# ihsanhadi57/Face-Detection-With-YOLOv11-SAHI-and-Real-ESRGAN

Measured on AMD Instinct MI355X. Metric: end-to-end 4K frames/sec (SAHI+YOLOv11s+ESRGAN×4), higher is better.
Workload: dtype f32x3(detect)+f16(sr)

## Files before the change

### face-detection-with-yolov11-sahi-and-real-esrgan_amd/_lib.py

```python
from __future__ import annotations

import ctypes as C
import os
import sys
from typing import List, Optional, Sequence, Tuple

import numpy as np

from . import weights_io

_HERE = os.path.dirname(os.path.abspath(__file__))
LIB_PATH = os.environ.get("FFP_LIB") or os.path.join(_HERE, "libffp.so")

PREC_F32, PREC_F16, PREC_F32X3 = 0, 1, 2
SR_ALPHA_REALESRGAN, SR_ALPHA_LINEAR = 0, 1
CHAN_AS_BGR, CHAN_AS_RGB = 0, 1
IQA_F32_CHW, IQA_U8_HWC = 0, 1
NIQE_FEATURES = 36
PP_NMS, PP_GREEDYNMM = 0, 1
METRIC_IOU, METRIC_IOS = 0, 1
PP_TYPES = {"NMS": PP_NMS, "GREEDYNMM": PP_GREEDYNMM}
METRICS = {"IOU": METRIC_IOU, "IOS": METRIC_IOS}

_lib = None


class FfpError(RuntimeError):
    def __init__(self, code: int, msg: str):
        super().__init__(f"libffp error {code}: {msg}")
        self.code = code


def _p(t):
    return C.POINTER(t)


_SIGS = {
    "ffp_last_error": (C.c_char_p, []),
    "ffp_version": (C.c_int, []),
    "ffp_device_count": (C.c_int, [_p(C.c_int)]),
    "ffp_slice_bboxes": (C.c_int, [C.c_int, C.c_int, C.c_int, C.c_int, C.c_float, C.c_float, _p(C.c_int32), C.c_int, _p(C.c_int32)]),
    "ffp_tile_chunks": (C.c_int, [C.c_int, C.c_int, _p(C.c_int32), C.c_int, _p(C.c_int32)]),
    "ffp_letterbox_geometry": (C.c_int, [C.c_int, C.c_int, C.c_int, _p(C.c_int32)]),
    "ffp_det_create": (C.c_int, [C.c_void_p, C.c_size_t, C.c_int, C.c_int, C.c_int, C.c_int, C.c_int, _p(C.c_void_p)]),
    "ffp_det_destroy": (None, [C.c_void_p]),
    "ffp_det_infer_tiles": (C.c_int, [C.c_void_p, C.c_void_p, C.c_int, C.c_int, C.c_int, _p(C.c_int32), C.c_int, C.c_int, C.c_float,
                                      C.c_float, C.c_int, C.c_int, _p(C.c_float), _p(C.c_int32)]),
    "ffp_det_infer_tiles_dev": (C.c_int, [C.c_void_p, C.c_void_p, C.c_int, C.c_int, C.c_int, _p(C.c_int32), C.c_int, C.c_int, C.c_float,
                                          C.c_float, C.c_int, C.c_int, C.c_void_p, C.c_void_p]),
    "ffp_det_truncate_shift_dev": (C.c_int, [C.c_void_p, C.c_void_p, C.c_void_p, C.c_int, C.c_int, C.c_int, C.c_int]),
    "ffp_det_forward_raw": (C.c_int, [C.c_void_p, C.c_void_p, C.c_int, C.c_int, C.c_int, _p(C.c_int32), C.c_int, C.c_int, _p(C.c_float),
                                      C.c_size_t, _p(C.c_int32)]),
    "ffp_merge": (C.c_int, [C.c_int, _p(C.c_float), C.c_int, C.c_int, C.c_int, C.c_int, C.c_double, C.c_int, _p(C.c_float), _p(C.c_int32),
                            _p(C.c_int32)]),
    "ffp_merge_dev": (C.c_int, [C.c_void_p, C.c_void_p, C.c_void_p, C.c_int, C.c_int, C.c_int, C.c_int, C.c_double, C.c_int, C.c_void_p,
                                C.c_int, C.c_void_p]),
    "ffp_sliced_predict": (C.c_int, [C.c_void_p, C.c_void_p, C.c_int, C.c_int, C.c_int, C.c_int, C.c_int, C.c_float, C.c_float, C.c_int,
                                     C.c_int, C.c_float, C.c_float, C.c_int, C.c_int, C.c_int, C.c_int, C.c_double, C.c_int, _p(C.c_float),
                                     C.c_int, _p(C.c_int32)]),
    "ffp_det_stage_dev": (C.c_int, [C.c_void_p, C.c_void_p, C.c_int, C.c_int, C.c_int, C.c_int, C.c_int, C.c_float, C.c_float, C.c_int,
                                    C.c_int, C.c_float, C.c_float, C.c_int, C.c_int, C.c_int, C.c_int, C.c_void_p, C.c_void_p,
                                    _p(C.c_int32), _p(C.c_int32)]),
    "ffp_det_last_ms": (C.c_int, [C.c_void_p, C.c_int, _p(C.c_float)]),
    "ffp_det_last_conv_stats": (C.c_int, [C.c_void_p, _p(C.c_double), _p(C.c_float), _p(C.c_int32)]),
    "ffp_det_set_profile": (C.c_int, [C.c_void_p, C.c_int]),
    "ffp_det_profile_count": (C.c_int, [C.c_void_p, _p(C.c_int32)]),
    "ffp_det_profile_get": (C.c_int, [C.c_void_p, C.c_int, C.c_char_p, C.c_int, _p(C.c_double), _p(C.c_float), _p(C.c_int32)]),
    "ffp_det_profile_detail": (C.c_int, [C.c_void_p, C.c_int, C.c_char_p, C.c_int, _p(C.c_double), _p(C.c_float)]),
    "ffp_sr_profile_detail": (C.c_int, [C.c_void_p, C.c_int, C.c_char_p, C.c_int, _p(C.c_double), _p(C.c_float)]),
    "ffp_sr_create": (C.c_int, [C.c_void_p, C.c_size_t, C.c_int, C.c_int, C.c_int, C.c_int, _p(C.c_void_p)]),
    "ffp_sr_destroy": (None, [C.c_void_p]),
    "ffp_sr_enhance": (C.c_int, [C.c_void_p, C.c_void_p, C.c_int, C.c_int, C.c_int, C.c_int, C.c_int, C.c_void_p]),
    "ffp_sr_enhance_ex": (C.c_int, [C.c_void_p, C.c_void_p, C.c_int, C.c_int, C.c_int, C.c_int, C.c_int, C.c_int, C.c_int, C.c_int, C.c_int,
                                    C.c_int, C.c_int, C.c_void_p]),
    "ffp_sr_enhance_dev": (C.c_int, [C.c_void_p, C.c_void_p, C.c_int, C.c_int, C.c_int, C.c_int, C.c_int, C.c_void_p]),
    "ffp_sr_enhance_batch": (C.c_int, [C.c_void_p, C.c_int, _p(C.c_void_p), _p(C.c_int32), _p(C.c_int32), C.c_int, C.c_int, C.c_int,
                                       _p(C.c_void_p)]),
    "ffp_sr_enhance_crops_dev": (C.c_int, [C.c_void_p, C.c_void_p, C.c_int, C.c_int, _p(C.c_int32), C.c_int, C.c_int, C.c_int, C.c_void_p,
                                           C.c_size_t, _p(C.c_int64)]),
    "ffp_sr_enhance_crops_dev_async": (C.c_int, [C.c_void_p, C.c_void_p, C.c_int, C.c_int, _p(C.c_int32), C.c_int, C.c_int, C.c_int,
                                                 C.c_void_p, C.c_size_t, _p(C.c_int64)]),
    "ffp_sr_wait": (C.c_int, [C.c_void_p]),
    "ffp_sr_enhance_crops_multi_dev_async": (C.c_int, [C.c_void_p, C.c_int, _p(C.c_void_p), _p(C.c_int32), C.c_int, C.c_int, _p(C.c_int32),
                                                       C.c_int, C.c_int, C.c_int, C.c_void_p, C.c_size_t, _p(C.c_int64)]),
    "ffp_sr_plan_state": (C.c_int, [C.c_void_p, _p(C.c_int32), _p(C.c_int32)]),
    "ffp_det_graph_status": (C.c_int, [C.c_void_p, _p(C.c_int32)]),
    "ffp_sr_set_fused_body": (C.c_int, [C.c_void_p, C.c_int]),
    "ffp_det_drop_plans": (C.c_int, [C.c_void_p]),
    "ffp_sr_drop_plans": (C.c_int, [C.c_void_p]),
    "ffp_det_profile_bytes": (C.c_int, [C.c_void_p, C.c_int, _p(C.c_double)]),
    "ffp_sr_profile_bytes": (C.c_int, [C.c_void_p, C.c_int, _p(C.c_double)]),
    "ffp_conv_totals_enable": (C.c_int, [C.c_int]),
    "ffp_conv_totals_count": (C.c_int, [_p(C.c_int32)]),
    "ffp_conv_totals_get": (C.c_int, [C.c_int, C.c_char_p, C.c_int, _p(C.c_double), _p(C.c_double), _p(C.c_int64)]),
    "ffp_sr_mem_bytes": (C.c_int, [C.c_void_p, _p(C.c_uint64), _p(C.c_uint64), _p(C.c_int32)]),
    "ffp_det_mem_bytes": (C.c_int, [C.c_void_p, _p(C.c_uint64), _p(C.c_uint64), _p(C.c_int32)]),
    "ffp_det_set_lanes": (C.c_int, [C.c_void_p, C.c_int]),
    "ffp_det_set_buffer_reuse": (C.c_int, [C.c_void_p, C.c_int]),
    "ffp_det_set_gate": (C.c_int, [C.c_void_p, C.c_int]),
    "ffp_det_last_active": (C.c_int, [C.c_void_p, C.POINTER(C.c_int32), C.POINTER(C.c_int32)]),
    "ffp_det_mem_detail": (C.c_int, [C.c_void_p, _p(C.c_uint64), _p(C.c_uint64), _p(C.c_uint64)]),
    "ffp_det_fill_steps": (C.c_int, [C.c_void_p, _p(C.c_int32), _p(C.c_int32)]),
    "ffp_det_stream_wait_event": (C.c_int, [C.c_void_p, C.c_void_p]),
    "ffp_sr_last_ms": (C.c_int, [C.c_void_p, _p(C.c_float)]),
    "ffp_sr_last_conv_stats": (C.c_int, [C.c_void_p, _p(C.c_double), _p(C.c_float), _p(C.c_int32)]),
    "ffp_sr_set_profile": (C.c_int, [C.c_void_p, C.c_int]),
    "ffp_sr_profile_count": (C.c_int, [C.c_void_p, _p(C.c_int32)]),
    "ffp_sr_profile_get": (C.c_int, [C.c_void_p, C.c_int, C.c_char_p, C.c_int, _p(C.c_double), _p(C.c_float), _p(C.c_int32)]),
    "ffp_eval_wider_pr": (C.c_int, [C.c_int, _p(C.c_double), _p(C.c_int64), _p(C.c_double), _p(C.c_int64), _p(C.c_uint8), C.c_int, C.c_double, C.c_int,
                                    _p(C.c_int64)]),
    "ffp_eval_dual_match": (C.c_int, [C.c_int, _p(C.c_double), _p(C.c_int64), _p(C.c_double), _p(C.c_int64), _p(C.c_uint8), C.c_int, C.c_double, _p(C.c_int32)]),
    "ffp_eval_coco_bbox": (C.c_int, [C.c_int, C.c_int, C.c_int, _p(C.c_double), _p(C.c_int64), _p(C.c_double), _p(C.c_int64), _p(C.c_double), C.c_int,
                                     _p(C.c_double), C.c_int, _p(C.c_double), C.c_int, _p(C.c_int32), C.c_int, _p(C.c_double), _p(C.c_double),
                                     _p(C.c_double), _p(C.c_double), _p(C.c_uint8), _p(C.c_double), _p(C.c_uint8)]),
    "ffp_jpeg_encode": (C.c_int, [C.c_int, _p(C.c_uint8), C.c_int, C.c_int, C.c_int, C.c_int, _p(C.c_uint8), C.c_int64, _p(C.c_int64)]),
    "ffp_jpeg_encode_dev": (C.c_int, [C.c_int, C.c_void_p, C.c_int, C.c_int, C.c_int64, C.c_int, C.c_int, _p(C.c_uint8), C.c_int64, _p(C.c_int64)]),
    "ffp_jpeg_encode_batch_dev": (C.c_int, [C.c_int, C.c_void_p, C.c_int, _p(C.c_int64), _p(C.c_int32), _p(C.c_int32), _p(C.c_int64), C.c_int, C.c_int, _p(C.c_uint8),
                                            C.c_int64, _p(C.c_int64)]),
    "ffp_png_bound": (C.c_int64, [C.c_int, C.c_int, C.c_int, C.c_int]),
    "ffp_png_segment_bytes": (C.c_int, []),
    "ffp_png_encode": (C.c_int, [C.c_int, C.c_void_p, C.c_int, C.c_int, C.c_int, C.c_int, C.c_int, C.c_int, _p(C.c_uint8), C.c_int64, _p(C.c_int64)]),
    "ffp_png_encode_dev": (C.c_int, [C.c_int, C.c_void_p, C.c_int, C.c_int, C.c_int, C.c_int, C.c_int64, C.c_int, C.c_int, _p(C.c_uint8), C.c_int64, _p(C.c_int64)]),
    "ffp_png_encode_batch_dev": (C.c_int, [C.c_int, C.c_void_p, C.c_int, _p(C.c_int64), _p(C.c_int32), _p(C.c_int32), _p(C.c_int64), C.c_int, C.c_int, C.c_int, C.c_int,
                                           _p(C.c_uint8), C.c_int64, _p(C.c_int64)]),
    "ffp_jpeg_info": (C.c_int, [_p(C.c_uint8), C.c_int64, _p(C.c_int32), _p(C.c_int32), _p(C.c_int32)]),
    "ffp_jpeg_decode": (C.c_int, [C.c_int, _p(C.c_uint8), C.c_int64, C.c_int, _p(C.c_uint8), C.c_int64]),
    "ffp_jpeg_decode_dev": (C.c_int, [C.c_int, _p(C.c_uint8), C.c_int64, C.c_int, C.c_void_p, C.c_int64, C.c_int64]),
    "ffp_jpeg_decode_stats": (C.c_int, [_p(C.c_int64), _p(C.c_int64), _p(C.c_int64)]),
    "ffp_op_conv2d_shape": (C.c_int, [C.c_int]),
    "ffp_op_conv2d_shape_name": (C.c_int, [C.c_int, C.c_char_p, C.c_int]),
    "ffp_op_conv2d_last_variant": (C.c_int, [C.c_char_p, C.c_int]),
    "ffp_op_conv2d_act_post": (C.c_int, [C.c_int]),
    "ffp_op_conv1x1_up2": (C.c_int, [C.c_int, C.c_int, _p(C.c_float), _p(C.c_float), C.c_int, C.c_int, C.c_int, C.c_int, C.c_int, _p(C.c_float),
                                     _p(C.c_float), C.c_int, C.c_int, _p(C.c_float)]),
    "ffp_op_conv2d_time": (C.c_int, [C.c_int, C.c_int, C.c_int, C.c_int, C.c_int, C.c_int, C.c_int, C.c_int, C.c_int, C.c_int, C.c_int, C.c_int,
                                     C.c_int, _p(C.c_float)]),
    "ffp_op_conv2d": (C.c_int, [C.c_int, C.c_int, _p(C.c_float), C.c_int, C.c_int, C.c_int, C.c_int, _p(C.c_float), _p(C.c_float), C.c_int,
                                C.c_int, C.c_int, C.c_int, C.c_int, C.c_int, _p(C.c_float), C.c_float, _p(C.c_float)]),
    "ffp_op_variant": (C.c_int, [C.c_int, C.c_int]),
    "ffp_op_cls_tower_variant": (C.c_int, [C.c_int, C.c_int]),
    "ffp_op_sppf_pool": (C.c_int, [C.c_int, C.c_int, C.c_int, _p(C.c_int32), _p(C.c_int32), C.c_int, C.c_int, _p(C.c_float), C.c_int, C.c_int,
                                   _p(C.c_float), C.c_int, C.c_int, C.c_int, C.c_int]),
    "ffp_op_upsample2x": (C.c_int, [C.c_int, C.c_int, C.c_int, _p(C.c_int32), _p(C.c_int32), C.c_int, C.c_int, _p(C.c_float), C.c_int, C.c_int,
                                    _p(C.c_float), C.c_int, C.c_int]),
    "ffp_op_psa_attention": (C.c_int, [C.c_int, C.c_int, C.c_int, _p(C.c_int32), _p(C.c_int32), C.c_int, C.c_int, _p(C.c_float), C.c_int, C.c_int,
                                       _p(C.c_float), C.c_int, C.c_int]),
    "ffp_op_dwconv3x3": (C.c_int, [C.c_int, C.c_int, C.c_int, _p(C.c_int32), _p(C.c_int32), C.c_int, C.c_int, _p(C.c_float), C.c_int, C.c_int,
                                   C.c_int, C.c_int, C.c_int, _p(C.c_float), _p(C.c_float), C.c_int, _p(C.c_float), C.c_int, C.c_int,
                                   _p(C.c_float), C.c_int, C.c_int]),
    "ffp_op_cls_tower": (C.c_int, [C.c_int, C.c_int, _p(C.c_int32), _p(C.c_int32), C.c_int, C.c_int, C.c_int] + [_p(C.c_float)] * 13 + [C.c_int, C.c_int, _p(C.c_int64)]),
    "ffp_op_conv2d_views": (C.c_int, [C.c_int, C.c_int, C.c_int, _p(C.c_int32), _p(C.c_int32), C.c_int, _p(C.c_float), C.c_int, C.c_int, C.c_int,
                                      _p(C.c_float), _p(C.c_float), C.c_int, C.c_int, C.c_int, C.c_int, C.c_int, C.c_int, _p(C.c_float), C.c_int,
                                      C.c_int, C.c_float, _p(C.c_float), C.c_int, C.c_int, C.c_float, _p(C.c_float), C.c_int, C.c_int, C.c_int,
                                      _p(C.c_uint32), _p(C.c_int32), _p(C.c_int32), _p(C.c_int64)]),
    "ffp_op_det_post": (C.c_int, [C.c_int, C.c_int, _p(C.c_int32), _p(C.c_int32), C.c_int, C.c_int, C.c_int, _p(C.c_float), _p(C.c_float),
                                  _p(C.c_float), _p(C.c_float), _p(C.c_int32), C.c_float, C.c_float, C.c_int, C.c_int, C.c_int, C.c_int, C.c_int,
                                  _p(C.c_float), _p(C.c_float), _p(C.c_int32)]),
    "ffp_op_rt_topk": (C.c_int, [C.c_int, C.c_int, C.c_int, C.c_int, _p(C.c_float), C.c_int, C.c_int, _p(C.c_int32)]),
    "ffp_op_rt_dwconv": (C.c_int, [C.c_int, C.c_int, C.c_int, C.c_int, C.c_int, C.c_int, C.c_int, C.c_int, _p(C.c_float), C.c_int, C.c_int, _p(C.c_float), _p(C.c_float), _p(C.c_float), C.c_int, C.c_int, _p(C.c_uint32)]),
    "ffp_op_rt_maxpool2": (C.c_int, [C.c_int, C.c_int, C.c_int, C.c_int, C.c_int, _p(C.c_float), C.c_int, C.c_int, _p(C.c_float), C.c_int, C.c_int, _p(C.c_uint32)]),
    "ffp_op_rt_add": (C.c_int, [C.c_int, C.c_longlong, C.c_int, _p(C.c_float), C.c_int, C.c_int, _p(C.c_float), C.c_int, C.c_int, C.c_longlong, _p(C.c_float), C.c_int, C.c_int, _p(C.c_uint32)]),
    "ffp_op_rt_layernorm": (C.c_int, [C.c_int, C.c_longlong, _p(C.c_float), C.c_int, C.c_int, _p(C.c_float), _p(C.c_float), _p(C.c_float), C.c_int, C.c_int, _p(C.c_uint32)]),
    "ffp_op_rt_gelu": (C.c_int, [C.c_int, C.c_longlong, C.c_int, _p(C.c_float), C.c_int, C.c_int, _p(C.c_uint32)]),
    "ffp_op_rt_attention": (C.c_int, [C.c_int, C.c_int, C.c_int, _p(C.c_float), C.c_int, C.c_int, _p(C.c_float), C.c_int, C.c_int, _p(C.c_float), C.c_int, C.c_int, _p(C.c_uint32)]),
    "ffp_op_rt_enc_prep": (C.c_int, [C.c_int, C.c_int, _p(C.c_int32), _p(C.c_int32), _p(C.c_float), _p(C.c_float), _p(C.c_float), _p(C.c_int32), _p(C.c_int32), _p(C.c_float), C.c_longlong, _p(C.c_float), _p(C.c_float), _p(C.c_uint32), _p(C.c_uint32)]),
    "ffp_op_rt_gather": (C.c_int, [C.c_int, C.c_int, C.c_int, _p(C.c_float), C.c_int, C.c_int, _p(C.c_int32), _p(C.c_float), _p(C.c_float), C.c_int, C.c_int, _p(C.c_float), _p(C.c_uint32)]),
    "ffp_op_rt_ref": (C.c_int, [C.c_int, C.c_longlong, _p(C.c_float), C.c_int, C.c_int, _p(C.c_float), _p(C.c_float), C.c_int, C.c_int, _p(C.c_uint32)]),
    "ffp_op_rt_deform": (C.c_int, [C.c_int, C.c_int, _p(C.c_int32), _p(C.c_int32), _p(C.c_float), C.c_int, C.c_int, _p(C.c_float), C.c_int, C.c_int, _p(C.c_float), C.c_int, C.c_int, _p(C.c_float), C.c_int, C.c_int, _p(C.c_uint32)]),
    "ffp_op_rt_decode": (C.c_int, [C.c_int, C.c_int, C.c_int, _p(C.c_float), C.c_int, C.c_int, _p(C.c_float), C.c_int, C.c_int, C.c_float, _p(C.c_float), _p(C.c_float), _p(C.c_float), _p(C.c_int32)]),
    "ffp_op_rt_post_tiles": (C.c_int, [C.c_int, C.c_int, C.c_int, _p(C.c_float), C.c_int, C.c_int, _p(C.c_float), C.c_int, C.c_int, C.c_float, _p(C.c_int32), C.c_int, C.c_int, C.c_int, _p(C.c_float), _p(C.c_int32)]),
    "ffp_op_scrfd_pool": (C.c_int, [C.c_int, C.c_int, _p(C.c_int32), _p(C.c_int32), C.c_int, C.c_int, C.c_int, C.c_int, _p(C.c_float), C.c_int, C.c_int, _p(C.c_float), C.c_int, C.c_int]),
    "ffp_op_scrfd_post": (C.c_int, [C.c_int, C.c_int, C.c_int, C.c_int, C.c_int, _p(C.c_int32), C.c_int, _p(_p(C.c_float)), _p(C.c_int32), _p(C.c_int32), _p(C.c_float), C.c_float, C.c_float, C.c_int, _p(C.c_float), _p(C.c_int32), _p(C.c_float)]),
    "ffp_op_resize_lanczos4": (C.c_int, [C.c_int, C.c_void_p, C.c_int, C.c_int, C.c_int, C.c_int, C.c_int, C.c_int, C.c_void_p]),
    "ffp_op_image_input": (C.c_int, [C.c_int, C.c_int, C.c_int, _p(C.c_uint8), C.c_int, C.c_int, C.c_int, C.c_int, _p(C.c_int32), C.c_int, C.c_int,
                                     _p(C.c_float), _p(C.c_int32), _p(C.c_int32)]),
    "ffp_op_stem": (C.c_int, [C.c_int, C.c_int, C.c_int, _p(C.c_uint8), C.c_int, C.c_int, C.c_int, C.c_int, _p(C.c_int32), C.c_int, _p(C.c_float),
                              _p(C.c_float), C.c_int, C.c_int, C.c_int, _p(C.c_float)]),
    "ffp_op_stem_conv": (C.c_int, [C.c_int, _p(C.c_uint8), C.c_int, C.c_int, C.c_int, C.c_int, _p(C.c_int32), C.c_int, _p(C.c_float), _p(C.c_float),
                                   C.c_int, _p(C.c_float), _p(C.c_float), _p(C.c_float)]),
    "ffp_scrfd_create": (C.c_int, [C.c_void_p, C.c_size_t, C.c_int, C.c_int, C.c_int, _p(C.c_void_p)]),
    "ffp_scrfd_destroy": (None, [C.c_void_p]),
    "ffp_scrfd_describe": (C.c_int, [C.c_void_p, C.c_size_t, C.c_int, C.c_int, C.c_int, C.c_char_p, C.c_size_t]),
    "ffp_scrfd_infer_tiles": (C.c_int, [C.c_void_p, C.c_void_p, C.c_int, C.c_int, C.c_int, _p(C.c_int32), C.c_int, C.c_int, C.c_int, C.c_float,
                                        C.c_float, _p(C.c_float), C.c_int, _p(C.c_int32)]),
    "ffp_scrfd_infer_tiles_ex": (C.c_int, [C.c_void_p, C.c_void_p, C.c_int, C.c_int, C.c_int, _p(C.c_int32), C.c_int, C.c_int, C.c_int, C.c_float,
                                           C.c_float, C.c_float, C.c_int, C.c_int, _p(C.c_float), C.c_int, _p(C.c_int32)]),
    "ffp_scrfd_infer_tiles_dev": (C.c_int, [C.c_void_p, C.c_void_p, C.c_int, C.c_int, C.c_int, _p(C.c_int32), C.c_int, C.c_int, C.c_int, C.c_float,
                                            C.c_float, C.c_float, C.c_int, C.c_int, C.c_void_p, C.c_int, C.c_void_p]),
    "ffp_scrfd_sliced_predict": (C.c_int, [C.c_void_p, C.c_void_p, C.c_int, C.c_int, C.c_int, C.c_int, C.c_int, C.c_float, C.c_float, C.c_int, C.c_int,
                                           C.c_int, C.c_float, C.c_float, C.c_float, C.c_int, C.c_int, C.c_int, C.c_int, C.c_double, C.c_int,
                                           _p(C.c_float), C.c_int, _p(C.c_int32)]),
    "ffp_scrfd_sliced_predict_dev": (C.c_int, [C.c_void_p, C.c_void_p, C.c_int, C.c_int, C.c_int, C.c_int, C.c_int, C.c_float, C.c_float, C.c_int,
                                               C.c_int, C.c_int, C.c_float, C.c_float, C.c_float, C.c_int, C.c_int, C.c_int, C.c_int, C.c_double,
                                               C.c_int, C.c_void_p, C.c_int, C.c_void_p]),
    "ffp_scrfd_mem_bytes": (C.c_int, [C.c_void_p, _p(C.c_uint64), _p(C.c_int32)]),
    "ffp_scrfd_drop_plans": (C.c_int, [C.c_void_p]),
    "ffp_op_scrfd_sahi_rows": (C.c_int, [C.c_int, C.c_int, C.c_int, _p(C.c_int32), C.c_int, C.c_int, C.c_float, _p(C.c_float), _p(C.c_int32),
                                         _p(C.c_int32)]),
    "ffp_scrfd_forward_raw": (C.c_int, [C.c_void_p, C.c_void_p, C.c_int, C.c_int, C.c_int, _p(C.c_int32), C.c_int, C.c_int, C.c_int, _p(C.c_float),
                                        C.c_size_t, _p(C.c_int64)]),
    "ffp_scrfd_info": (C.c_int, [C.c_void_p, _p(C.c_int32), _p(C.c_double)]),
    "ffp_scrfd_geometry": (C.c_int, [C.c_int, C.c_int, C.c_int, C.c_int, _p(C.c_int32), _p(C.c_float)]),
    "ffp_rtdetr_create": (C.c_int, [C.c_void_p, C.c_size_t, C.c_int, C.c_int, _p(C.c_void_p)]),
    "ffp_rtdetr_destroy": (None, [C.c_void_p]),
    "ffp_rtdetr_predict": (C.c_int, [C.c_void_p, _p(C.c_void_p), _p(C.c_int32), C.c_int, C.c_int, C.c_float, _p(C.c_float), _p(C.c_int32)]),
    "ffp_rtdetr_forward_raw": (C.c_int, [C.c_void_p, _p(C.c_void_p), _p(C.c_int32), C.c_int, C.c_int, _p(C.c_float), _p(C.c_int32)]),
    "ffp_rtdetr_infer_tiles": (C.c_int, [C.c_void_p, C.c_void_p, C.c_int, C.c_int, C.c_int, _p(C.c_int32), C.c_int, C.c_int, C.c_float, C.c_int, C.c_int,
                                         _p(C.c_float), _p(C.c_int32)]),
    "ffp_rtdetr_infer_tiles_dev": (C.c_int, [C.c_void_p, C.c_void_p, C.c_int, C.c_int, C.c_int, _p(C.c_int32), C.c_int, C.c_int, C.c_float, C.c_int,
                                             C.c_int, C.c_void_p, C.c_void_p]),
    "ffp_rtdetr_sliced_predict": (C.c_int, [C.c_void_p, C.c_void_p, C.c_int, C.c_int, C.c_int, C.c_int, C.c_int, C.c_float, C.c_float, C.c_int, C.c_int,
                                            C.c_float, C.c_int, C.c_int, C.c_int, C.c_double, C.c_int, _p(C.c_float), C.c_int, _p(C.c_int32)]),
    "ffp_rtdetr_mem_bytes": (C.c_int, [C.c_void_p, _p(C.c_uint64), _p(C.c_int32)]),
    "ffp_rtdetr_drop_plans": (C.c_int, [C.c_void_p]),
    "ffp_rtdetr_info": (C.c_int, [C.c_void_p, _p(C.c_int32), _p(C.c_double), _p(C.c_int32)]),
    "ffp_rtdetr_set_profile": (C.c_int, [C.c_void_p, C.c_int]),
    "ffp_rtdetr_profile_count": (C.c_int, [C.c_void_p, _p(C.c_int32)]),
    "ffp_rtdetr_profile_get": (C.c_int, [C.c_void_p, C.c_int, C.c_char_p, C.c_int, _p(C.c_float)]),
    "ffp_iqa_create": (C.c_int, [C.c_int, _p(C.c_void_p)]),
    "ffp_iqa_destroy": (None, [C.c_void_p]),
    "ffp_iqa_niqe_blocks": (C.c_int, [C.c_int, C.c_int, _p(C.c_int64)]),
    "ffp_iqa_niqe_features": (C.c_int, [C.c_void_p, C.c_int, _p(C.c_void_p), _p(C.c_int32), _p(C.c_int32), _p(C.c_int32), C.c_int, C.c_int, C.c_int,
                                        _p(C.c_double), _p(C.c_double), C.c_int64, _p(C.c_int64)]),
    "ffp_iqa_niqe_luma": (C.c_int, [C.c_void_p, C.c_void_p, C.c_int, C.c_int, C.c_int, C.c_int, C.c_int, _p(C.c_float)]),
    "ffp_iqa_niqe_score": (C.c_int, [_p(C.c_double), _p(C.c_int64), C.c_int, _p(C.c_double), _p(C.c_double), _p(C.c_double)]),
}

EXPORTED_SYMBOLS = tuple(_SIGS)


def lib() -> C.CDLL:
    global _lib
    if _lib is None:
        if not os.path.exists(LIB_PATH):
            raise RuntimeError(f"{LIB_PATH} is missing: build it with `python -m ffp_amd.build` "
                               "(hipcc --offload-arch=gfx950). There is no CPU/PyTorch fallback.")
        if "torch" not in sys.modules:
            try:
                import importlib.util
                spec = importlib.util.find_spec("torch")
                cand = os.path.join(os.path.dirname(spec.origin), "lib", "libamdhip64.so") if spec and spec.origin else None
                if cand and os.path.exists(cand):
                    C.CDLL(cand, mode=C.RTLD_GLOBAL)
            except Exception:
                pass
        l = C.CDLL(LIB_PATH)
        for name, (res, args) in _SIGS.items():
            f = getattr(l, name)
            f.restype = res
            f.argtypes = args
        _lib = l
    return _lib


def _check(rc: int):
    if rc != 0:
        raise FfpError(rc, lib().ffp_last_error().decode("utf-8", "replace"))


def device_count() -> int:
    n = C.c_int(0)
    _check(lib().ffp_device_count(C.byref(n)))
    return n.value


def _fp(a: np.ndarray):
    return a.ctypes.data_as(_p(C.c_float))


def _ip(a: np.ndarray):
    return a.ctypes.data_as(_p(C.c_int32))


def slice_bboxes(H: int, W: int, slice_h: int, slice_w: int, overlap_h: float = 0.2, overlap_w: float = 0.2) -> np.ndarray:
    n = C.c_int32(0)
    _check(lib().ffp_slice_bboxes(H, W, slice_h, slice_w, overlap_h, overlap_w, None, 0, C.byref(n)))
    out = np.zeros((n.value, 4), np.int32)
    _check(lib().ffp_slice_bboxes(H, W, slice_h, slice_w, overlap_h, overlap_w, _ip(out), n.value, C.byref(n)))
    return out


def tile_chunks(n: int, max_batch: int) -> List[int]:
# ... 1108 lines not shown
    if rc != 0:
        e = FfpError(rc, lib().ffp_last_error().decode("utf-8", "replace"))
        e.needed = n.value
        raise e
    return out[:n.value].tobytes()


def png_encode_dev(d_ptr: int, h: int, w: int, channels: int = 3, bit_depth: int = 8, row_stride: int = None, level: int = 1, bgr: bool = True,
                   device: int = 0) -> bytes:
    if row_stride is None:
        row_stride = w * channels * (bit_depth // 8)
    cap = png_bound(h, w, channels, bit_depth)
    out = np.empty(cap, np.uint8)
    n = C.c_int64(0)
    _check(lib().ffp_png_encode_dev(device, C.c_void_p(d_ptr), h, w, channels, bit_depth, row_stride, int(bgr), level, out.ctypes.data_as(_p(C.c_uint8)), cap,
                                    C.byref(n)))
    return out[:n.value].tobytes()


def png_encode_batch_dev(d_base: int, offsets, hs, ws, channels: int = 3, bit_depth: int = 8, strides=None, level: int = 1, bgr: bool = True, device: int = 0):
    offsets = np.ascontiguousarray(offsets, np.int64)
    hs, ws = np.ascontiguousarray(hs, np.int32), np.ascontiguousarray(ws, np.int32)
    n = len(offsets)
    st = None if strides is None else np.ascontiguousarray(strides, np.int64)
    cap = sum(png_bound(int(h), int(w), channels, bit_depth) for h, w in zip(hs, ws))
    out = np.empty(max(cap, 1), np.uint8)
    oo = np.zeros(n + 1, np.int64)
    _check(lib().ffp_png_encode_batch_dev(device, C.c_void_p(d_base), n, offsets.ctypes.data_as(_p(C.c_int64)), hs.ctypes.data_as(_p(C.c_int32)),
                                          ws.ctypes.data_as(_p(C.c_int32)), None if st is None else st.ctypes.data_as(_p(C.c_int64)), channels, bit_depth,
                                          int(bgr), level, out.ctypes.data_as(_p(C.c_uint8)), cap, oo.ctypes.data_as(_p(C.c_int64))))
    return [out[oo[i]:oo[i + 1]].tobytes() for i in range(n)]


def jpeg_info(data: bytes):
    buf = np.frombuffer(data, np.uint8)
    h, w, nc = C.c_int32(0), C.c_int32(0), C.c_int32(0)
    _check(lib().ffp_jpeg_info(buf.ctypes.data_as(_p(C.c_uint8)), len(buf), C.byref(h), C.byref(w), C.byref(nc)))
    return h.value, w.value, nc.value


def jpeg_decode(data: bytes, bgr: bool = False, device: int = 0) -> np.ndarray:
    h, w, _ = jpeg_info(data)
    buf = np.frombuffer(data, np.uint8)
    out = np.empty((h, w, 3), np.uint8)
    _check(lib().ffp_jpeg_decode(device, buf.ctypes.data_as(_p(C.c_uint8)), len(buf), int(bgr), out.ctypes.data_as(_p(C.c_uint8)), out.size))
    return out


def jpeg_decode_dev(data: bytes, d_ptr: int, row_stride: int, cap: int, bgr: bool = True, device: int = 0):
    h, w, _ = jpeg_info(data)
    buf = np.frombuffer(data, np.uint8)
    _check(lib().ffp_jpeg_decode_dev(device, buf.ctypes.data_as(_p(C.c_uint8)), len(buf), int(bgr), C.c_void_p(d_ptr), row_stride, cap))
    return h, w


def jpeg_decode_stats():
    a, b, c = C.c_int64(0), C.c_int64(0), C.c_int64(0)
    _check(lib().ffp_jpeg_decode_stats(C.byref(a), C.byref(b), C.byref(c)))
    return a.value, b.value, c.value


def _ragged(rows, width, dtype):
    rows = [np.asarray(r, dtype).reshape(-1, width) for r in rows]
    off = np.zeros(len(rows) + 1, np.int64)
    np.cumsum([len(r) for r in rows], out=off[1:])
    flat = np.ascontiguousarray(np.concatenate(rows + [np.zeros((0, width), dtype)], 0))
    return flat, off


def eval_wider_pr(preds, gts, evaluate, iou_thr: float = 0.5, thresh_num: int = 1000, device: int = 0) -> np.ndarray:
    p, po = _ragged(preds, 5, np.float64)
    g, go = _ragged(gts, 4, np.float64)
    e, eo = _ragged([np.asarray(x, np.uint8).reshape(-1, 1) for x in evaluate], 1, np.uint8)
    if len(po) != len(go) or not np.array_equal(go, eo):
        raise ValueError("preds / gts / evaluate must describe the same images and faces")
    out = np.zeros((thresh_num, 2), np.int64)
    _check(lib().ffp_eval_wider_pr(device, p.ctypes.data_as(_p(C.c_double)), po.ctypes.data_as(_p(C.c_int64)), g.ctypes.data_as(_p(C.c_double)),
                                   go.ctypes.data_as(_p(C.c_int64)), e.ctypes.data_as(_p(C.c_uint8)), len(po) - 1, iou_thr, thresh_num,
                                   out.ctypes.data_as(_p(C.c_int64))))
    return out


def eval_dual_match(preds, faces, valid, iou_thr: float = 0.5, device: int = 0):
    p, po = _ragged(preds, 5, np.float64)
    f, fo = _ragged(faces, 4, np.float64)
    v, vo = _ragged([np.asarray(x, np.uint8).reshape(-1, 1) for x in valid], 1, np.uint8)
    if len(po) != len(fo) or not np.array_equal(fo, vo):
        raise ValueError("preds / faces / valid must describe the same images and faces")
    flags = np.zeros(max(int(po[-1]), 1), np.int32)
    _check(lib().ffp_eval_dual_match(device, p.ctypes.data_as(_p(C.c_double)), po.ctypes.data_as(_p(C.c_int64)), f.ctypes.data_as(_p(C.c_double)),
                                     fo.ctypes.data_as(_p(C.c_int64)), v.ctypes.data_as(_p(C.c_uint8)), len(po) - 1, iou_thr, flags.ctypes.data_as(_p(C.c_int32))))
    return [flags[po[i]:po[i + 1]] for i in range(len(po) - 1)]


def eval_coco_bbox(dets, det_off, gts, gt_off, n_img: int, n_cat: int, iou_thrs, rec_thrs, area_rng, max_dets, matches: bool = False,
                   device: int = 0) -> dict:
    d = np.ascontiguousarray(np.asarray(dets, np.float64).reshape(-1, 7))
    g = np.ascontiguousarray(np.asarray(gts, np.float64).reshape(-1, 8))
    do = np.ascontiguousarray(det_off, np.int64)
    go = np.ascontiguousarray(gt_off, np.int64)
    it = np.ascontiguousarray(iou_thrs, np.float64).reshape(-1)
    rt = np.ascontiguousarray(rec_thrs, np.float64).reshape(-1)
    ar = np.ascontiguousarray(area_rng, np.float64).reshape(-1, 2)
    md = np.ascontiguousarray(max_dets, np.int32).reshape(-1)
    U = int(n_img) * int(n_cat)
    if len(do) != U + 1 or len(go) != U + 1:
        raise ValueError(f"offsets must have n_cat * n_img + 1 = {U + 1} entries")
    T, R, K, A, M = len(it), len(rt), int(n_cat), len(ar), len(md)
    prec, sc = np.zeros((T, R, K, A, M)), np.zeros((T, R, K, A, M))
    rec = np.zeros((T, K, A, M))
    out = {"precision": prec, "recall": rec, "scores": sc}
    ptrs = [None] * 4
    if matches:
        cut = np.zeros(U + 1, np.int64)
        if U and len(md):
            np.cumsum(np.minimum(np.diff(do), int(md[-1])), out=cut[1:])
        ndc, ng = int(cut[-1]), int(go[-1]) if U else 0
        out.update(cut_off=cut, dt_matches=np.zeros((A, T, ndc)), dt_ignore=np.zeros((A, T, ndc), np.uint8), gt_matches=np.zeros((A, T, ng)),
                   gt_ignore=np.zeros((A, ng), np.uint8))
        ptrs = [out["dt_matches"].ctypes.data_as(_p(C.c_double)), out["dt_ignore"].ctypes.data_as(_p(C.c_uint8)),
                out["gt_matches"].ctypes.data_as(_p(C.c_double)), out["gt_ignore"].ctypes.data_as(_p(C.c_uint8))]
    dp = lambda a: a.ctypes.data_as(_p(C.c_double))
    _check(lib().ffp_eval_coco_bbox(device, int(n_img), int(n_cat), dp(d), do.ctypes.data_as(_p(C.c_int64)), dp(g), go.ctypes.data_as(_p(C.c_int64)),
                                    dp(it), T, dp(rt), R, dp(ar), A, md.ctypes.data_as(_p(C.c_int32)), M, dp(prec), dp(rec), dp(sc), *ptrs))
    return out


def op_conv1x1_up2(coarse: np.ndarray, fine: np.ndarray, w: np.ndarray, b: np.ndarray, act: int = 0, precision: int = PREC_F32X3, device: int = 0) -> np.ndarray:
    coarse = np.ascontiguousarray(coarse, np.float32)
    fine = np.ascontiguousarray(fine, np.float32)
    w = np.ascontiguousarray(w, np.float32).reshape(w.shape[0], -1)
    b = np.ascontiguousarray(b, np.float32)
    n, h, wd, cf = fine.shape
    y = np.zeros((n, h, wd, w.shape[0]), np.float32)
    _check(lib().ffp_op_conv1x1_up2(device, precision, _fp(coarse), _fp(fine), n, h, wd, coarse.shape[3], cf, _fp(w), _fp(b), w.shape[0], act, _fp(y)))
    return y


def op_resize_lanczos4(img: np.ndarray, out_h: int, out_w: int, device: int = 0) -> np.ndarray:
    a = np.ascontiguousarray(img)
    if a.dtype not in (np.uint8, np.uint16) or a.ndim not in (2, 3):
        raise ValueError(f"expected an HxW or HxWxC uint8 / uint16 array, got {a.dtype} {a.shape}")
    h, w = a.shape[:2]
    out = np.zeros((int(out_h), int(out_w)) + a.shape[2:], a.dtype)
    _check(lib().ffp_op_resize_lanczos4(device, a.ctypes.data, h, w, 1 if a.ndim == 2 else a.shape[2], 8 * a.itemsize, int(out_h), int(out_w),
                                        out.ctypes.data))
    return out


def op_conv2d_shape(shape: int = -1) -> None:
    _check(lib().ffp_op_conv2d_shape(int(shape)))


def op_conv2d_shape_name(shape: int) -> str:
    out = C.create_string_buffer(64)
    _check(lib().ffp_op_conv2d_shape_name(int(shape), out, len(out)))
    return out.value.decode()


def op_conv2d_last_variant() -> str:
    out = C.create_string_buffer(64)
    _check(lib().ffp_op_conv2d_last_variant(out, len(out)))
    return out.value.decode()


def op_conv2d_act_post(act: int = 0) -> None:
    _check(lib().ffp_op_conv2d_act_post(int(act)))


def op_conv2d_time(n, h, w, cin, cout, k=3, stride=1, up=False, precision=PREC_F16, iters=50, dbg=0, shape=-1, device=0) -> float:
    us = C.c_float(0)
    _check(lib().ffp_op_conv2d_time(device, precision, n, h, w, cin, cout, k, stride, int(up), iters, dbg, shape, C.byref(us)))
    return us.value


def niqe_blocks(h: int, w: int) -> int:
    n = C.c_int64(0)
    _check(lib().ffp_iqa_niqe_blocks(int(h), int(w), C.byref(n)))
    return n.value


def niqe_score(feat: np.ndarray, block_off: np.ndarray, mu: np.ndarray, cov: np.ndarray) -> np.ndarray:
    f = np.ascontiguousarray(feat, np.float64).reshape(-1, NIQE_FEATURES)
    off = np.ascontiguousarray(block_off, np.int64)
    m = np.ascontiguousarray(np.asarray(mu, np.float64).reshape(-1))
    c = np.ascontiguousarray(cov, np.float64)
    if m.shape != (NIQE_FEATURES,) or c.shape != (NIQE_FEATURES, NIQE_FEATURES):
        raise ValueError(f"the NIQE model is a 36-vector and a 36x36 matrix, got {m.shape} and {c.shape}")
    if off.ndim != 1 or off.size < 1 or off[-1] != f.shape[0]:
        raise ValueError("block offsets do not match the feature rows")
    out = np.zeros(off.size - 1, np.float64)
    dp = _p(C.c_double)
    _check(lib().ffp_iqa_niqe_score(f.ctypes.data_as(dp), off.ctypes.data_as(_p(C.c_int64)), off.size - 1, m.ctypes.data_as(dp), c.ctypes.data_as(dp),
                                    out.ctypes.data_as(dp)))
    return out


class IQA:

    def __init__(self, device: int = 0):
        self._h = C.c_void_p()
        self.device = device
        _check(lib().ffp_iqa_create(device, C.byref(self._h)))

    def close(self):
        if getattr(self, "_h", None) is not None and self._h.value:
            lib().ffp_iqa_destroy(self._h)
            self._h = C.c_void_p()

    def __del__(self):
        try:
            self.close()
        except Exception:
            pass

    def niqe_features(self, images: Sequence[np.ndarray], chan_order: int = CHAN_AS_RGB) -> Tuple[np.ndarray, np.ndarray, np.ndarray]:
        ims = [np.ascontiguousarray(i) for i in images]
        if not ims:
            raise ValueError("no images")
        kinds = {i.dtype == np.uint8 for i in ims}
        if len(kinds) != 1 or any(i.dtype not in (np.uint8, np.float32) for i in ims):
            raise ValueError("images must be all uint8 (H, W, C) or all float32 (C, H, W)")
        u8 = ims[0].dtype == np.uint8
        shp = []
        for i in ims:
            if i.ndim == 2:
                shp.append((i.shape[0], i.shape[1], 1))
            elif i.ndim == 3:
                shp.append((i.shape[0], i.shape[1], i.shape[2]) if u8 else (i.shape[1], i.shape[2], i.shape[0]))
            else:
                raise ValueError(f"expected a 2-d or 3-d image, got shape {i.shape}")
        return self._features([i.ctypes.data for i in ims], shp, IQA_U8_HWC if u8 else IQA_F32_CHW, chan_order, False)

    def luma(self, image: np.ndarray, chan_order: int = CHAN_AS_RGB) -> np.ndarray:
        a = np.ascontiguousarray(image)
        u8 = a.dtype == np.uint8
        if a.dtype not in (np.uint8, np.float32) or a.ndim not in (2, 3):
            raise ValueError(f"expected a uint8 (H, W, C) or float32 (C, H, W) image, got {a.dtype} {a.shape}")
        h, w, c = (a.shape[0], a.shape[1], 1) if a.ndim == 2 else ((a.shape[0], a.shape[1], a.shape[2]) if u8 else (a.shape[1], a.shape[2], a.shape[0]))
        out = np.zeros((max(h // 96 * 96, 1), max(w // 96 * 96, 1)), np.float32)
        _check(lib().ffp_iqa_niqe_luma(self._h, a.ctypes.data, h, w, c, IQA_U8_HWC if u8 else IQA_F32_CHW, int(chan_order), _fp(out)))
        return out

    def niqe_features_dev(self, ptrs: Sequence[int], shapes: Sequence[Tuple[int, int, int]]) -> Tuple[np.ndarray, np.ndarray, np.ndarray]:
        return self._features(list(ptrs), [(h, w, c) for c, h, w in shapes], IQA_F32_CHW, CHAN_AS_RGB, True)

    def _features(self, ptrs, shp, layout, chan_order, on_device):
        n = len(ptrs)
        hs = np.asarray([s[0] for s in shp], np.int32)
        ws = np.asarray([s[1] for s in shp], np.int32)
        cs = np.asarray([s[2] for s in shp], np.int32)
        nb = max(1, sum((int(h) // 96) * (int(w) // 96) for h, w in zip(hs, ws)))
        feat = np.zeros((nb, NIQE_FEATURES), np.float64)
        sharp = np.zeros(nb, np.float64)
        off = np.zeros(n + 1, np.int64)
        ip = (C.c_void_p * n)(*ptrs)
        _check(lib().ffp_iqa_niqe_features(self._h, n, ip, _ip(hs), _ip(ws), _ip(cs), layout, int(chan_order), int(on_device),
                                           feat.ctypes.data_as(_p(C.c_double)), sharp.ctypes.data_as(_p(C.c_double)), nb, off.ctypes.data_as(_p(C.c_int64))))
        return feat[:off[-1]], sharp[:off[-1]], off

    def niqe(self, images: Sequence[np.ndarray], mu: np.ndarray, cov: np.ndarray, chan_order: int = CHAN_AS_RGB) -> np.ndarray:
        feat, _, off = self.niqe_features(images, chan_order)
        return niqe_score(feat, off, mu, cov)
```

### face-detection-with-yolov11-sahi-and-real-esrgan_amd/csrc/api_ops.cpp

```cpp
#include <climits>
#include <cmath>

#include "api_util.hpp"
#include "conv_route.hpp"
#include "rtdetr.hpp"
#include "scrfd.hpp"
#include "sr_ops.hpp"
#include "yolo11.hpp"

using namespace ffp;

extern "C" {

static int g_op_conv_shape = SHAPE_AUTO;
int ffp_op_conv2d_shape(int force_shape) {
  FFP_API_BEGIN
  FFP_CHECK(force_shape == SHAPE_AUTO || conv_shape_info(force_shape), FFP_ERR_ARG, "conv2d_shape: %d is not a shape number", force_shape);
  g_op_conv_shape = force_shape;
  FFP_API_END
}

int ffp_op_conv2d_shape_name(int shape, char* out, int cap) {
  FFP_API_BEGIN
  const ConvShapeInfo* s = conv_shape_info(shape);
  FFP_CHECK(s && out && cap > 0, FFP_ERR_ARG, "conv2d_shape_name: %d is not a shape number, or no output buffer", shape);
  std::snprintf(out, cap, "%s %s", s->family_name, s->suffix);
  FFP_API_END
}

static thread_local std::string tl_op_conv_variant;
int ffp_op_conv2d_last_variant(char* out, int cap) {
  FFP_API_BEGIN
  FFP_CHECK(out && cap > 0, FFP_ERR_ARG, "conv2d_last_variant: no output buffer");
  std::snprintf(out, cap, "%s", tl_op_conv_variant.c_str());
  FFP_API_END
}

static int g_op_conv_act_post = ACT_NONE;
int ffp_op_conv2d_act_post(int act) {
  FFP_API_BEGIN
  FFP_CHECK(act >= ACT_NONE && act <= ACT_RELU, FFP_ERR_ARG, "conv2d_act_post: activation code %d (0..3)", act);
  g_op_conv_act_post = act;
  FFP_API_END
}

int ffp_op_conv2d(int device, int precision, const float* x, int n, int h, int w, int cin, const float* wt, const float* bias, int cout,
                  int k, int stride, int groups, int act, int up, const float* res, float res_scale, float* y) {
  FFP_API_BEGIN
  FFP_CHECK(x && wt && y && n > 0 && h > 0 && w > 0 && cin > 0 && cout > 0, FFP_ERR_ARG, "conv2d: bad arguments");
  FFP_CHECK((k == 1 || k == 3) && (stride == 1 || stride == 2), FFP_ERR_ARG, "conv2d: k in {1,3}, stride in {1,2}");
  ScopedStream cx(device, "conv2d");
  conv_kernels_init();
  tl_op_conv_variant.clear();
  const DType T = precision == FFP_PREC_F16 ? F16 : F32;
  const bool split = precision == FFP_PREC_F32X3;
  PackedConv pc;
  pack_conv(pc, "op", wt, bias, cout, cin, k, groups, T, cx.st, split);
  const int hi = up ? h * 2 : h, wi = up ? w * 2 : w;
  const int ho = (hi + 2 * (k / 2) - k) / stride + 1, wo = (wi + 2 * (k / 2) - k) / stride + 1;
  Level lin, lout;
  lin.build(std::vector<int>(n, h), std::vector<int>(n, w), cx.st);
  lout.build(std::vector<int>(n, ho), std::vector<int>(n, wo), cx.st);
  const int cin_s = pc.depthwise() ? cin : pc.cin;
  const size_t npx_in = (size_t)lin.total_px, npx_out = (size_t)lout.total_px;
  auto to_dev = [&](const float* src, size_t px, int c, int c_store) {
    DevBuf b(px * c_store * dsize(T) + 256);
    if (T == F32) {
      std::vector<float> t(px * c_store, 0.f);
      for (size_t p = 0; p < px; ++p) std::memcpy(&t[p * c_store], src + p * c, sizeof(float) * c);
      FFP_HIP(hipMemcpy(b.p, t.data(), t.size() * 4, hipMemcpyHostToDevice));
    } else {
      std::vector<_Float16> t(px * c_store, (_Float16)0.f);
      for (size_t p = 0; p < px; ++p) for (int q = 0; q < c; ++q) t[p * c_store + q] = (_Float16)src[p * c + q];
      FFP_HIP(hipMemcpy(b.p, t.data(), t.size() * 2, hipMemcpyHostToDevice));
    }
    return b;
  };
  DevBuf din = to_dev(x, npx_in, cin, cin_s);
  DevBuf dres;
  if (res) dres = to_dev(res, npx_out, cout, cout);
  DevBuf dout(npx_out * cout * dsize(T) + 256);
  TView vin{din.p, T, cin_s, 0, cin_s, &lin}, vout{dout.p, T, cout, 0, cout, &lout}, vres{dres.p, T, cout, 0, cout, &lout};
  DevBuf slots(2 * sizeof(unsigned));
  {
    float m = 0.f;
    for (size_t i = 0; i < npx_in * (size_t)cin; ++i) m = std::max(m, std::fabs(x[i]));
    unsigned hb[2] = {0u, 0u};
    std::memcpy(&hb[0], &m, 4);
    FFP_HIP(hipMemcpy(slots.p, hb, sizeof(hb), hipMemcpyHostToDevice));
    vin.amax = slots.as<unsigned>(); vout.amax = slots.as<unsigned>() + 1;
  }
  if (pc.depthwise()) {
    FFP_CHECK(k == 3 && stride == 1 && !up, FFP_ERR_ARG, "conv2d: depthwise is 3x3 stride 1");
    FFP_CHECK(g_op_conv_act_post == ACT_NONE, FFP_ERR_ARG, "conv2d: depthwise convs have no post-activation");
    DwConvOp o;
    o.pc = &pc; o.in = vin; o.out = vout; o.out.lvl = &lin; o.act = act;
    if (res) { o.has_res = true; o.res = vres; o.res.lvl = &lin; FFP_CHECK(res_scale == 1.f, FFP_ERR_ARG, "conv2d: depthwise residual has no scale"); }
    launch_dwconv(o, cx.st);
  } else {
    ConvOp o;
    o.pc = &pc; o.in = vin; o.out = vout; o.stride = stride; o.act = act; o.up = up;
    if (res) { o.has_res1 = true; o.res1 = vres; o.s1 = res_scale; }
    o.force_shape = g_op_conv_shape;
    o.act_post = g_op_conv_act_post;
    launch_conv(o, cx.st);
    tl_op_conv_variant = conv_variant(o);
  }
  FFP_HIP(hipStreamSynchronize(cx.st));
  if (T == F32) {
    FFP_HIP(hipMemcpy(y, dout.p, npx_out * cout * 4, hipMemcpyDeviceToHost));
  } else {
    std::vector<_Float16> t(npx_out * cout);
    FFP_HIP(hipMemcpy(t.data(), dout.p, t.size() * 2, hipMemcpyDeviceToHost));
    for (size_t i = 0; i < t.size(); ++i) y[i] = (float)t[i];
  }
  FFP_API_END
}

int ffp_op_conv1x1_up2(int device, int precision, const float* coarse, const float* fine, int n, int h, int w, int c_up, int c_fine,
                       const float* wt, const float* bias, int cout, int act, float* y) {
  FFP_API_BEGIN
  FFP_CHECK(coarse && fine && wt && y && n > 0 && h > 0 && w > 0 && h % 2 == 0 && w % 2 == 0 && c_up > 0 && c_fine > 0 && cout > 0, FFP_ERR_ARG, "conv1x1_up2: bad arguments");
  FFP_CHECK(precision == FFP_PREC_F32 || precision == FFP_PREC_F32X3, FFP_ERR_ARG, "conv1x1_up2: fp32 precisions only");
  ScopedStream cx(device, "conv1x1_up2");
  conv_kernels_init();
  tl_op_conv_variant.clear();
  const int cin = c_up + c_fine;
  PackedConv pc;
  pack_conv(pc, "op", wt, bias, cout, cin, 1, 1, F32, cx.st, precision == FFP_PREC_F32X3);
  FFP_CHECK(pc.cin == cin, FFP_ERR_ARG, "conv1x1_up2: channel count %d needs padding", cin);
  Level lf, lc;
  lf.build(std::vector<int>(n, h), std::vector<int>(n, w), cx.st);
  lc.build(std::vector<int>(n, h / 2), std::vector<int>(n, w / 2), cx.st);
  const size_t pf = (size_t)lf.total_px, pcs = (size_t)lc.total_px;
  std::vector<float> cat(pf * cin, std::nanf(""));
  for (size_t p = 0; p < pf; ++p) std::memcpy(&cat[p * cin + c_up], fine + p * c_fine, sizeof(float) * c_fine);
  DevBuf dcat(cat.size() * 4 + 256), dco(pcs * c_up * 4 + 256), dout(pf * cout * 4 + 256), slots(3 * sizeof(unsigned));
  FFP_HIP(hipMemcpy(dcat.p, cat.data(), cat.size() * 4, hipMemcpyHostToDevice));
  FFP_HIP(hipMemcpy(dco.p, coarse, pcs * c_up * 4, hipMemcpyHostToDevice));
  float mf = 0.f, mc = 0.f;
  for (size_t i = 0; i < pf * (size_t)c_fine; ++i) mf = std::max(mf, std::fabs(fine[i]));
  for (size_t i = 0; i < pcs * (size_t)c_up; ++i) mc = std::max(mc, std::fabs(coarse[i]));
  unsigned hb[3] = {0u, 0u, 0u};
  std::memcpy(&hb[0], &mf, 4);
  std::memcpy(&hb[1], &mc, 4);
  FFP_HIP(hipMemcpy(slots.p, hb, sizeof(hb), hipMemcpyHostToDevice));
  TView vin{dcat.p, F32, cin, 0, cin, &lf}, vco{dco.p, F32, c_up, 0, c_up, &lc}, vout{dout.p, F32, cout, 0, cout, &lf};
  vin.amax = slots.as<unsigned>(); vco.amax = slots.as<unsigned>() + 1; vout.amax = slots.as<unsigned>() + 2;
  ConvOp o;
  o.pc = &pc; o.in = vin; o.out = vout; o.stride = 1; o.act = act;
  o.has_up2 = true; o.up2 = vco; o.up2_c = c_up; o.up2_map = lf.up2_map(&lc, cx.st);
  o.force_shape = g_op_conv_shape;
  launch_conv(o, cx.st);
  tl_op_conv_variant = conv_variant(o);
  FFP_HIP(hipStreamSynchronize(cx.st));
  FFP_HIP(hipMemcpy(y, dout.p, pf * cout * 4, hipMemcpyDeviceToHost));
  FFP_API_END
}

static int g_op_variant[3] = {0, 0, 0};
int ffp_op_variant(int family, int variant) {
  FFP_API_BEGIN
  FFP_CHECK(family >= 0 && family < 3 && variant >= 0 && variant <= 2, FFP_ERR_ARG, "op_variant: family %d / variant %d unknown", family, variant);
  g_op_variant[family] = variant;
  FFP_API_END
}
static int g_op_cls_tower_force = 0;
int ffp_op_cls_tower_variant(int rows, int wg_cap) {
  FFP_API_BEGIN
  FFP_CHECK((rows == 0 || rows == 8 || rows == 16) && wg_cap >= 0 && wg_cap <= 65535, FFP_ERR_ARG, "op_cls_tower_variant: rows %d (0, 8, 16) / workgroup cap %d", rows, wg_cap);
  g_op_cls_tower_force = (rows == 16 ? 1 : rows == 8 ? 2 : 0) | wg_cap << 2;
  FFP_API_END
}

namespace {

void op_check_batch(const char* what, int n, const int32_t* hs, const int32_t* ws, int px_align) {
  FFP_CHECK(n > 0 && n <= 4096 && hs && ws && px_align >= 1 && px_align <= 4096, FFP_ERR_ARG, "%s: bad batch description", what);
  for (int i = 0; i < n; ++i) FFP_CHECK(hs[i] > 0 && ws[i] > 0 && hs[i] <= 8192 && ws[i] <= 8192, FFP_ERR_ARG, "%s: image %d is %dx%d", what, i, ws[i], hs[i]);
}
void op_check_view(const char* what, int cs, int coff, int C) {
  FFP_CHECK(C > 0 && coff >= 0 && cs > 0 && coff + C <= cs, FFP_ERR_ARG, "%s: channels [%d, %d) do not fit records of %d", what, coff, coff + C, cs);
}
DType op_dtype(const char* what, int precision) {
  FFP_CHECK(precision == FFP_PREC_F32 || precision == FFP_PREC_F16, FFP_ERR_ARG, "%s: precision must be FFP_PREC_F32 or FFP_PREC_F16", what);
  return precision == FFP_PREC_F16 ? F16 : F32;
}

DevBuf op_upload(const Level& L, DType T, const float* src, int cs) {
  const size_t tot = (size_t)L.total_px * cs;
  DevBuf b(tot * dsize(T) + 256);
  std::vector<float> t(tot, std::nanf(""));
  size_t sp = 0;
  for (int i = 0; i < L.n; ++i) {
    const size_t np = (size_t)L.h[i] * L.w[i];
    std::memcpy(&t[(size_t)L.off[i] * cs], src + sp * cs, np * cs * sizeof(float));
    sp += np;
  }
  if (T == F32) {
    FFP_HIP(hipMemcpy(b.p, t.data(), tot * 4, hipMemcpyHostToDevice));
  } else {
    std::vector<_Float16> h(tot);
    for (size_t i = 0; i < tot; ++i) h[i] = (_Float16)t[i];
    FFP_HIP(hipMemcpy(b.p, h.data(), tot * 2, hipMemcpyHostToDevice));
  }
  return b;
}

void op_download(const Level& L, DType T, const DevBuf& b, int cs, float* dst) {
  const size_t tot = (size_t)L.total_px * cs;
  std::vector<float> t(tot);
  if (T == F32) {
    FFP_HIP(hipMemcpy(t.data(), b.p, tot * 4, hipMemcpyDeviceToHost));
  } else {
    std::vector<_Float16> h(tot);
    FFP_HIP(hipMemcpy(h.data(), b.p, tot * 2, hipMemcpyDeviceToHost));
    for (size_t i = 0; i < tot; ++i) t[i] = (float)h[i];
  }
  size_t sp = 0;
  for (int i = 0; i < L.n; ++i) {
    const size_t np = (size_t)L.h[i] * L.w[i];
    std::memcpy(dst + sp * cs, &t[(size_t)L.off[i] * cs], np * cs * sizeof(float));
    sp += np;
  }
}

}

int ffp_op_sppf_pool(int device, int precision, int n, const int32_t* hs, const int32_t* ws, int px_align, int c, const float* x, int x_cs,
                     int x_coff, float* y, int y_cs, int y1_coff, int y2_coff, int y3_coff) {
  FFP_API_BEGIN
  FFP_CHECK(x && y, FFP_ERR_ARG, "sppf_pool: null argument");
  op_check_batch("sppf_pool", n, hs, ws, px_align);
  op_check_view("sppf_pool input", x_cs, x_coff, c);
  const int yo[3] = {y1_coff, y2_coff, y3_coff};
  for (int i = 0; i < 3; ++i) {
    op_check_view("sppf_pool output", y_cs, yo[i], c);
    for (int j = 0; j < i; ++j) FFP_CHECK(yo[i] >= yo[j] + c || yo[j] >= yo[i] + c, FFP_ERR_ARG, "sppf_pool: output slices %d and %d overlap", j + 1, i + 1);
  }
  const DType T = op_dtype("sppf_pool", precision);
  ScopedStream cx(device, "sppf_pool");
  Level L;
  L.build(std::vector<int>(hs, hs + n), std::vector<int>(ws, ws + n), cx.st, px_align);
  DevBuf din = op_upload(L, T, x, x_cs), dout = op_upload(L, T, y, y_cs);
  const TView vin{din.p, T, x_cs, x_coff, c, &L};
  const TView v1{dout.p, T, y_cs, y1_coff, c, &L}, v2{dout.p, T, y_cs, y2_coff, c, &L}, v3{dout.p, T, y_cs, y3_coff, c, &L};
  launch_sppf_pool(vin, v1, v2, v3, cx.st, g_op_variant[0]);
  FFP_HIP(hipStreamSynchronize(cx.st));
  op_download(L, T, dout, y_cs, y);
  FFP_API_END
}

int ffp_op_upsample2x(int device, int precision, int n, const int32_t* hs, const int32_t* ws, int px_align, int c, const float* x, int x_cs,
                      int x_coff, float* y, int y_cs, int y_coff) {
  FFP_API_BEGIN
  FFP_CHECK(x && y, FFP_ERR_ARG, "upsample2x: null argument");
// ... 88 lines not shown
  pack_conv(dw1, "cv3.1.0", dw1_w, dw1_b, C3, C3, 3, C3, F32, cx.st, false);
  pack_conv(pw1, "cv3.1.1", pw1_w, pw1_b, C3, C3, 1, 1, F32, cx.st, true);
  pack_conv(fin, "cv3.2", fin_w, fin_b, nc, C3, 1, 1, F32, cx.st, true);
  DenseF32 dense;
  dense.w.alloc(sizeof(float) * nc * C3);
  dense.b.alloc(sizeof(float) * nc);
  FFP_HIP(hipMemcpy(dense.w.p, fin_w, sizeof(float) * nc * C3, hipMemcpyHostToDevice));
  FFP_HIP(hipMemcpy(dense.b.p, fin_b, sizeof(float) * nc, hipMemcpyHostToDevice));
  Level L;
  L.build(std::vector<int>(hs, hs + n), std::vector<int>(ws, ws + n), cx.st, px_align);
  DevBuf dx = op_upload(L, F32, x, cin), dhead = op_upload(L, F32, head, head_cs);
  FFP_HIP(hipMemset(static_cast<char*>(dhead.p) + (size_t)L.total_px * head_cs * 4, 0xFF, 256));
  DevBuf de1((size_t)L.total_px * C3 * 4 + 256), de2((size_t)L.total_px * C3 * 4 + 256);
  FFP_HIP(hipMemset(de1.p, 0xFF, de1.n));
  FFP_HIP(hipMemset(de2.p, 0xFF, de2.n));
  std::vector<unsigned> slots(3 * (size_t)n, 0u);
  {
    size_t sp = 0;
    for (int i = 0; i < n; ++i) {
      const size_t np = (size_t)hs[i] * ws[i] * cin;
      float m = 0.f;
      for (size_t k = 0; k < np; ++k) m = std::max(m, std::fabs(x[sp + k]));
      std::memcpy(&slots[i], &m, 4);
      sp += np;
    }
  }
  DevBuf dslots(slots.size() * 4);
  FFP_HIP(hipMemcpy(dslots.p, slots.data(), slots.size() * 4, hipMemcpyHostToDevice));
  auto view = [&](void* p, int cs, int coff, int c, int slot) {
    TView v{p, F32, cs, coff, c, &L};
    if (slot >= 0) { v.amax = dslots.as<unsigned>() + (size_t)slot * n; v.amax_n = n; }
    return v;
  };
  const bool fuse_fin = nc <= 4;
  ConvOp t1, t2;
  t1.pc = &pw0; t1.dw = &dw0; t1.dw_act = ACT_SILU; t1.act = ACT_SILU;
  t1.in = view(dx.p, cin, 0, cin, 0); t1.out = view(de1.p, C3, 0, C3, 1);
  t2.pc = &pw1; t2.dw = &dw1; t2.dw_act = ACT_SILU; t2.act = ACT_SILU;
  t2.in = t1.out; t2.out = view(fuse_fin ? nullptr : de2.p, C3, 0, C3, 2);
  const TView logits = view(dhead.p, head_cs, head_coff, nc, -1);
  if (fuse_fin) { t2.fin = &fin; t2.fin_w = &dense; t2.fin_out = logits; }
  t1.dwpw_force = t2.dwpw_force = g_op_cls_tower_force;
  launch_conv(t1, cx.st);
  launch_conv(t2, cx.st);
  if (!fuse_fin) {
    ConvOp t3;
    t3.pc = &fin; t3.in = t2.out; t3.out = logits; t3.act = ACT_NONE;
    launch_conv(t3, cx.st);
  }
  FFP_HIP(hipStreamSynchronize(cx.st));
  op_download(L, F32, dhead, head_cs, head);
  if (e1) op_download(L, F32, de1, C3, e1);
  if (stray) {
    const float nanv = std::nanf("");
    unsigned nan_bits;
    std::memcpy(&nan_bits, &nanv, 4);
    auto changed = [&](const DevBuf& b, int cs, unsigned want, unsigned want_slack) {
      std::vector<unsigned> h(b.n / 4);
      FFP_HIP(hipMemcpy(h.data(), b.p, h.size() * 4, hipMemcpyDeviceToHost));
      int64_t bad = 0;
      for (int i = 0; i < n; ++i) {
        const size_t p0 = (size_t)(L.off[i] + (int64_t)hs[i] * ws[i]) * cs, p1 = (size_t)(i + 1 < n ? L.off[i + 1] : L.total_px) * cs;
        for (size_t k = p0; k < p1; ++k) bad += h[k] != want;
      }
      for (size_t k = (size_t)L.total_px * cs; k < h.size(); ++k) bad += h[k] != want_slack;
      return bad;
    };
    *stray = changed(de1, C3, 0xFFFFFFFFu, 0xFFFFFFFFu) + changed(de2, C3, 0xFFFFFFFFu, 0xFFFFFFFFu);
    if (fuse_fin) *stray += changed(dhead, head_cs, nan_bits, 0xFFFFFFFFu);
  }
  FFP_API_END
}

int ffp_op_conv2d_views(int device, int precision, int n, const int32_t* hs, const int32_t* ws, int px_align, const float* x, int x_cs, int x_coff,
                        int cin, const float* wt, const float* bias, int cout, int k, int stride, int act, int act_post, int up, const float* res1,
                        int r1_cs, int r1_coff, float s1, const float* res2, int r2_cs, int r2_coff, float s2, float* y, int y_cs, int y_coff,
                        int per_image_amax, uint32_t* amax_out, const int32_t* gate, const int32_t* gate_prev, int64_t* stray) {
  FFP_API_BEGIN
  FFP_CHECK(x && wt && y && amax_out && cin > 0 && cout > 0, FFP_ERR_ARG, "conv2d_views: null argument or no channels");
  FFP_CHECK(precision == FFP_PREC_F32 || precision == FFP_PREC_F16 || precision == FFP_PREC_F32X3, FFP_ERR_ARG, "conv2d_views: precision %d", precision);
  FFP_CHECK((k == 1 || k == 3) && (stride == 1 || stride == 2) && (up == 0 || up == 1) && (per_image_amax == 0 || per_image_amax == 1), FFP_ERR_ARG,
            "conv2d_views: k in {1,3}, stride in {1,2}, up and per_image_amax in {0,1}");
  FFP_CHECK(act >= ACT_NONE && act <= ACT_RELU && act_post >= ACT_NONE && act_post <= ACT_RELU, FFP_ERR_ARG, "conv2d_views: activation codes %d / %d (0..3)", act, act_post);
  FFP_CHECK(!gate_prev || gate, FFP_ERR_ARG, "conv2d_views: gate_prev without gate");
  op_check_batch("conv2d_views", n, hs, ws, px_align);
  const DType T = precision == FFP_PREC_F16 ? F16 : F32;
  const int epv = 16 / (int)dsize(T);
  const int cin_s = (cin + epv - 1) / epv * epv;
  op_check_view("conv2d_views input", x_cs, x_coff, cin_s);
  FFP_CHECK(x_cs % epv == 0 && x_coff % epv == 0, FFP_ERR_ARG, "conv2d_views: input view not 16-byte aligned (cs=%d coff=%d)", x_cs, x_coff);
  op_check_view("conv2d_views output", y_cs, y_coff, cout);
  if (res1) op_check_view("conv2d_views res1", r1_cs, r1_coff, cout);
  if (res2) op_check_view("conv2d_views res2", r2_cs, r2_coff, cout);
  std::vector<int> hi(hs, hs + n), wi(ws, ws + n), ho(n), wo(n);
  for (int i = 0; i < n; ++i) {
    const int hv = up ? hi[i] * 2 : hi[i], wv = up ? wi[i] * 2 : wi[i];
    ho[i] = (hv + 2 * (k / 2) - k) / stride + 1;
    wo[i] = (wv + 2 * (k / 2) - k) / stride + 1;
  }
  ScopedStream cx(device, "conv2d_views");
  conv_kernels_init();
  tl_op_conv_variant.clear();
  PackedConv pc;
  pack_conv(pc, "op", wt, bias, cout, cin, k, 1, T, cx.st, precision == FFP_PREC_F32X3);
  FFP_CHECK(pc.cin == cin_s, FFP_ERR_STATE, "conv2d_views: packed conv reads %d channels, expected %d", pc.cin, cin_s);
  Level lin, lout;
  lin.build(hi, wi, cx.st, px_align);
  lout.build(ho, wo, cx.st, px_align);
  lout.gate_compact = &launch_gate_compact;
  const size_t esz = dsize(T), ybytes = (size_t)lout.total_px * y_cs * esz;
  DevBuf din = op_upload(lin, T, x, x_cs), dout, dr1, dr2;
  if (res1) dr1 = op_upload(lout, T, res1, r1_cs);
  if (res2) dr2 = op_upload(lout, T, res2, r2_cs);
  const int ns = per_image_amax ? n : 1;
  std::vector<unsigned> slots(2 * (size_t)ns, 0u);
  {
    size_t sp = 0;
    for (int i = 0; i < n; ++i) {
      const size_t np = (size_t)hi[i] * wi[i];
      float m = 0.f;
      for (size_t p = 0; p < np; ++p)
        for (int c = 0; c < cin; ++c) m = std::max(m, std::fabs(x[(sp + p) * x_cs + x_coff + c]));
      unsigned b;
      std::memcpy(&b, &m, 4);
      slots[per_image_amax ? i : 0] = std::max(slots[per_image_amax ? i : 0], b);
      sp += np;
    }
  }
  DevBuf dslots(slots.size() * 4), dgate;
  auto upload_outputs = [&]() {
    dout = op_upload(lout, T, y, y_cs);
    FFP_HIP(hipMemset(static_cast<char*>(dout.p) + ybytes, 0xFF, 256));
    std::copy(amax_out, amax_out + ns, slots.begin() + ns);
    FFP_HIP(hipMemcpy(dslots.p, slots.data(), slots.size() * 4, hipMemcpyHostToDevice));
  };
  upload_outputs();
  if (gate) dgate = upload(gate_prev ? gate_prev : gate, (size_t)n);
  auto view = [&](void* p, int cs, int coff, int c, Level* L, int slot) {
    TView v{p, T, cs, coff, c, L};
    if (slot >= 0) { v.amax = dslots.as<unsigned>() + (size_t)slot * ns; v.amax_n = ns; }
    return v;
  };
  ConvOp o;
  o.pc = &pc; o.stride = stride; o.act = act; o.act_post = act_post; o.up = up;
  o.in = view(din.p, x_cs, x_coff, cin_s, &lin, 0);
  auto bind_out = [&]() {
    o.out = view(dout.p, y_cs, y_coff, cout, &lout, 1);
  };
  bind_out();
  if (res1) { o.has_res1 = true; o.res1 = view(dr1.p, r1_cs, r1_coff, cout, &lout, -1); o.s1 = s1; }
  if (res2) { o.has_res2 = true; o.res2 = view(dr2.p, r2_cs, r2_coff, cout, &lout, -1); o.s2 = s2; }
  if (gate) o.gate = dgate.as<int>();
  o.force_shape = g_op_conv_shape;
  launch_conv(o, cx.st);
  tl_op_conv_variant = conv_variant(o);
  FFP_HIP(hipStreamSynchronize(cx.st));
  if (gate_prev) {
    upload_outputs();
    bind_out();
    FFP_HIP(hipMemcpy(dgate.p, gate, sizeof(int32_t) * (size_t)n, hipMemcpyHostToDevice));
    lout.compact_gated(cx.st);
    launch_conv(o, cx.st);
    FFP_HIP(hipStreamSynchronize(cx.st));
  }
  std::vector<unsigned char> now(ybytes + 256);
  FFP_HIP(hipMemcpy(now.data(), dout.p, now.size(), hipMemcpyDeviceToHost));
  {
    size_t sp = 0;
    for (int i = 0; i < n; ++i) {
      const size_t ne = (size_t)ho[i] * wo[i] * y_cs, e0 = (size_t)lout.off[i] * y_cs;
      if (T == F32) std::memcpy(y + sp, &now[e0 * 4], ne * 4);
      else for (size_t e = 0; e < ne; ++e) y[sp + e] = (float)reinterpret_cast<const _Float16*>(now.data())[e0 + e];
      sp += ne;
    }
  }
  FFP_HIP(hipMemcpy(slots.data(), dslots.p, slots.size() * 4, hipMemcpyDeviceToHost));
  std::copy(slots.begin() + ns, slots.end(), amax_out);
  if (stray) {
    volatile float nanv = std::nanf("");
    const float nanf32 = nanv;
    const _Float16 nanf16 = (_Float16)nanf32;
    const void* want_pad = T == F32 ? static_cast<const void*>(&nanf32) : static_cast<const void*>(&nanf16);
    int64_t bad = 0;
    for (int i = 0; i < n; ++i) {
      const size_t p0 = (size_t)(lout.off[i] + (int64_t)ho[i] * wo[i]), p1 = (size_t)(i + 1 < n ? lout.off[i + 1] : lout.total_px);
      for (size_t p = p0; p < p1; ++p)
        for (int c = 0; c < y_cs; ++c) {
          if (k == 1 && c >= y_coff && c < y_coff + cout && (!gate || gate[i])) continue;
          bad += std::memcmp(&now[(p * y_cs + c) * esz], want_pad, esz) != 0;
        }
    }
    for (size_t e = ybytes; e < now.size(); ++e) bad += now[e] != 0xFF;
    *stray = bad;
  }
  FFP_API_END
}

int ffp_op_det_post(int device, int n, const int32_t* hs, const int32_t* ws, int px_align, int nc, int nkpt, const float* head8, const float* head16,
                    const float* head32, const float* gain_pad, const int32_t* rects, float conf, float iou, int max_det, int round_boxes,
                    int shift, int full_h, int full_w, float* out_raw, float* out_dets, int32_t* out_counts) {
  FFP_API_BEGIN
  FFP_CHECK(head8 && head16 && head32 && gain_pad && rects && nc >= 1 && nc <= 1024 && nkpt >= 0 && nkpt <= 64, FFP_ERR_ARG, "det_post: bad arguments");
  FFP_CHECK((out_dets != nullptr) == (out_counts != nullptr) && (out_raw || out_dets), FFP_ERR_ARG, "det_post: dets and counts come together, and something must be asked for");
  op_check_batch("det_post", n, hs, ws, px_align);
  for (int i = 0; i < n; ++i) {
    FFP_CHECK(hs[i] % 32 == 0 && ws[i] % 32 == 0, FFP_ERR_ARG, "det_post: net input %dx%d of image %d is not a multiple of 32", ws[i], hs[i], i);
    FFP_CHECK(gain_pad[3 * i] > 0.f && rects[4 * i] > 0 && rects[4 * i + 1] > 0, FFP_ERR_ARG, "det_post: image %d has no gain or no size", i);
  }
  if (out_dets) FFP_CHECK(max_det >= 1 && max_det <= 1024 && conf >= 0.f, FFP_ERR_ARG, "det_post: max_det %d outside [1,1024] or negative conf", max_det);
  ScopedStream cx(device, "det_post");
  const int cs = 64 + nc + 3 * nkpt, no = 4 + nc + 3 * nkpt, stride = 6 + 3 * nkpt;
  Level L[3];
  DevBuf dh[3];
  const float* heads[3] = {head8, head16, head32};
  for (int l = 0; l < 3; ++l) {
    std::vector<int> h(n), w(n);
    for (int i = 0; i < n; ++i) { h[i] = hs[i] / (8 << l); w[i] = ws[i] / (8 << l); }
    L[l].build(h, w, cx.st, px_align);
    dh[l] = op_upload(L[l], F32, heads[l], cs);
  }
  std::vector<int> aoff(n + 1, 0);
  std::vector<long long> roff(n);
  long long rtot = 0;
  for (int i = 0; i < n; ++i) {
    int a = 0;
    for (int l = 0; l < 3; ++l) a += L[l].h[i] * L[l].w[i];
    aoff[i + 1] = aoff[i] + a;
    roff[i] = rtot;
    rtot += (long long)no * a;
  }
  const int total = aoff[n];
  std::vector<DetImg> di(n);
  for (int i = 0; i < n; ++i) {
    di[i].gain = gain_pad[3 * i]; di[i].pad_x = gain_pad[3 * i + 1]; di[i].pad_y = gain_pad[3 * i + 2];
    di[i].sw = rects[4 * i]; di[i].sh = rects[4 * i + 1]; di[i].x0 = rects[4 * i + 2]; di[i].y0 = rects[4 * i + 3];
  }
  DevBuf d_aoff = upload(aoff.data(), aoff.size()), d_roff = upload(roff.data(), roff.size()), d_imgs = upload(di.data(), di.size());
  DecodeArgs a{};
  for (int l = 0; l < 3; ++l) { a.head[l] = dh[l].as<float>(); a.tab[l] = L[l].d_tab.as<int4>(); }
  a.head_cs = cs; a.nc = nc; a.nkpt = nkpt; a.n_img = n; a.anchor_off = d_aoff.as<int>(); a.total_anchors = total;
  if (out_raw) {
    DevBuf d_raw(sizeof(float) * (size_t)rtot);
    launch_decode_raw(a, d_raw.as<float>(), d_roff.as<long long>(), cx.st);
    FFP_HIP(hipStreamSynchronize(cx.st));
    FFP_HIP(hipMemcpy(out_raw, d_raw.p, sizeof(float) * (size_t)rtot, hipMemcpyDeviceToHost));
  }
  if (out_dets) {
    DevBuf d_boxes(sizeof(float4) * (size_t)total), d_scores(sizeof(float) * (size_t)total), d_classes(sizeof(int) * (size_t)total),
        d_cand(sizeof(int) * (size_t)total), d_cscore(sizeof(float) * (size_t)total);
    const size_t nd = (size_t)n * max_det * stride;
    DevBuf d_dets(sizeof(float) * nd), d_counts(sizeof(int) * (size_t)n);
    FFP_HIP(hipMemsetAsync(d_dets.p, 0, sizeof(float) * nd, cx.st));
    launch_decode(a, conf, d_boxes.as<float4>(), d_scores.as<float>(), d_classes.as<int>(), cx.st);
    launch_nms(a, d_boxes.as<float4>(), d_scores.as<float>(), d_classes.as<int>(), d_cand.as<int>(), d_cscore.as<float>(), d_imgs.as<DetImg>(), iou,
               max_det, round_boxes, stride, d_dets.as<float>(), d_counts.as<int>(), cx.st);
    if (shift) launch_truncate_shift(d_dets.as<float>(), d_counts.as<int>(), d_imgs.as<DetImg>(), n, max_det, stride, nkpt, full_h, full_w, cx.st);
    FFP_HIP(hipStreamSynchronize(cx.st));
    FFP_HIP(hipMemcpy(out_dets, d_dets.p, sizeof(float) * nd, hipMemcpyDeviceToHost));
    FFP_HIP(hipMemcpy(out_counts, d_counts.p, sizeof(int) * (size_t)n, hipMemcpyDeviceToHost));
  }
  FFP_API_END
}

int ffp_op_rt_topk(int device, int n, int nt, int nc, const float* scores, int s_cs, int s_coff, int32_t* out_idx) {
  FFP_API_BEGIN
  FFP_CHECK(scores && out_idx && n > 0 && n <= 4096 && nt >= RT_NQ && nt <= (1 << 22), FFP_ERR_ARG, "rt_topk: needs n in [1,4096] images of [%d, 2^22] tokens", RT_NQ);
  op_check_view("rt_topk scores", s_cs, s_coff, nc);
  ScopedStream cx(device, "rt_topk");
  const size_t tok = (size_t)n * nt;
  DevBuf ds = upload(scores, tok * s_cs), keys(sizeof(unsigned) * tok), idx(sizeof(int) * (size_t)n * RT_NQ);
  Level L;
  L.build(std::vector<int>(n, 1), std::vector<int>(n, nt), cx.st);
  launch_rt_topk(TView{ds.p, F32, s_cs, s_coff, nc, &L}, nc, nt, n, keys.as<unsigned>(), idx.as<int>(), cx.st);
  FFP_HIP(hipStreamSynchronize(cx.st));
  FFP_HIP(hipMemcpy(out_idx, idx.p, sizeof(int) * (size_t)n * RT_NQ, hipMemcpyDeviceToHost));
  FFP_API_END
}

namespace {

struct OpSlot {
  DevBuf d;
  uint32_t* host;
  explicit OpSlot(uint32_t* h) : host(h) { if (h) d = upload(h, 1); }
  unsigned* ptr() const { return host ? d.as<unsigned>() : nullptr; }
  void fetch() { if (host) FFP_HIP(hipMemcpy(host, d.p, sizeof(uint32_t), hipMemcpyDeviceToHost)); }
};

void op_check_view4(const char* what, int cs, int coff, int C) {
  op_check_view(what, cs, coff, C);
  FFP_CHECK(C % 4 == 0 && cs % 4 == 0 && coff % 4 == 0, FFP_ERR_ARG, "%s: channels, offset and record size must be multiples of 4 (%d at %d of %d)", what, C, coff, cs);
}

void op_flat_level(Level& L, int n, long long per_image, hipStream_t st) {
  FFP_CHECK(per_image >= 1 && per_image <= INT_MAX && n >= 1 && n <= 4096 && (long long)n * per_image <= (1ll << 28), FFP_ERR_ARG,
            "op: %d images of %lld records", n, per_image);
  L.build(std::vector<int>(n, 1), std::vector<int>(n, (int)per_image), st);
}

struct OpView : TView {
  OpView(const DevBuf& b, int cs_, int coff_, int C_, Level* L, unsigned* slot = nullptr) : TView{b.p, F32, cs_, coff_, C_, L} { amax = slot; }
};

void op_fetch(const DevBuf& b, float* dst, size_t n) { FFP_HIP(hipMemcpy(dst, b.p, n * sizeof(float), hipMemcpyDeviceToHost)); }

void op_rt_levels(const char* what, const int32_t* hs, const int32_t* ws, RtLevels& lv) {
// ... 428 lines not shown
  std::vector<LetterboxImg> lb;
  std::vector<float> scale;
  if (kind == 0) {
    lb = op_det_records(H, W, boxes_xyxy, n, size_a);
  } else if (kind == 1) {
    FFP_CHECK(size_a >= 32 && size_a % 32 == 0 && size_a <= 4096, FFP_ERR_ARG, "image_input: imgsz %d must be a multiple of 32 in [32, 4096]", size_a);
    rtdetr_tile_records(H, W, boxes_xyxy, n, size_a, lb);
  } else {
    FFP_CHECK(size_a % 32 == 0 && size_b % 32 == 0 && size_a >= 32 && size_b >= 32 && size_a <= 4096 && size_b <= 4096, FFP_ERR_ARG,
              "image_input: det size %dx%d must be multiples of 32 in [32, 4096]", size_a, size_b);
    scrfd_tile_records(size_a, size_b, H, W, boxes_xyxy, n, lb, scale);
  }
  std::vector<int> hs(n), ws(n);
  for (int i = 0; i < n; ++i) { hs[i] = lb[i].net_h; ws[i] = lb[i].net_w; }
  ScopedStream cx(device, "image_input");
  const int cs = T == F16 ? 8 : 4;
  Level L;
  L.build(hs, ws, cx.st);
  DevBuf d_frame = op_upload_frame(frame, H, W), d_imgs = upload(lb.data(), lb.size()), dout = op_nan_buffer((size_t)L.total_px * cs * dsize(T));
  const TView vout{dout.p, T, cs, 0, cs, &L};
  const int flip = chan_order == FFP_CHAN_AS_BGR ? 1 : 0;
  if (kind == 2) launch_scrfd_preproc(d_frame.as<uint8_t>(), W, flip, d_imgs.as<LetterboxImg>(), vout, cx.st);
  else launch_letterbox(d_frame.as<uint8_t>(), H, W, flip, d_imgs, vout, cx.st);
  FFP_HIP(hipStreamSynchronize(cx.st));
  op_download(L, T, dout, cs, out);
  std::copy(hs.begin(), hs.end(), out_hs);
  std::copy(ws.begin(), ws.end(), out_ws);
  FFP_API_END
}

int ffp_op_stem(int device, int precision, int fused, const uint8_t* frame, int H, int W, int chan_order, int n, const int32_t* boxes_xyxy, int imgsz,
                const float* w, const float* bias, int cout, int stride, int act, float* out) {
  FFP_API_BEGIN
  FFP_CHECK(w && bias && out, FFP_ERR_ARG, "stem: null argument");
  op_check_frame("stem", frame, H, W, chan_order, n, boxes_xyxy);
  FFP_CHECK((fused == 0 || fused == 1) && (cout == 16 || cout == 32 || cout == 64) && (stride == 1 || stride == 2) && act >= ACT_NONE && act <= ACT_RELU,
            FFP_ERR_ARG, "stem: fused %d (0, 1), cout %d (16, 32, 64), stride %d (1, 2), activation code %d (0..3)", fused, cout, stride, act);
  const DType T = op_dtype("stem", precision);
  const std::vector<LetterboxImg> lb = op_det_records(H, W, boxes_xyxy, n, imgsz);
  std::vector<int> hi(n), wi(n), ho(n), wo(n);
  for (int i = 0; i < n; ++i) {
    hi[i] = lb[i].net_h; wi[i] = lb[i].net_w;
    ho[i] = (hi[i] - 1) / stride + 1; wo[i] = (wi[i] - 1) / stride + 1;
  }
  ScopedStream cx(device, "stem");
  PackedConv pc;
  pack_conv(pc, "op_stem", w, bias, cout, 3, 3, 1, T, cx.st, false);
  Level lin, lout;
  lin.build(hi, wi, cx.st);
  lout.build(ho, wo, cx.st);
  const int cin0 = T == F16 ? 8 : 4;
  DevBuf d_frame = op_upload_frame(frame, H, W), d_imgs = upload(lb.data(), lb.size()), din,
         dout = op_nan_buffer((size_t)lout.total_px * cout * dsize(T));
  if (!fused) din = op_nan_buffer((size_t)lin.total_px * cin0 * dsize(T));
  ConvOp o;
  o.pc = &pc; o.stride = stride; o.act = act;
  o.in = TView{din.p, T, cin0, 0, cin0, &lin};
  o.out = TView{dout.p, T, cout, 0, cout, &lout};
  const int flip = chan_order == FFP_CHAN_AS_BGR ? 1 : 0;
  if (fused) {
    launch_stem_from_frame(d_frame.as<uint8_t>(), H, W, flip, d_imgs, o, cx.st);
  } else {
    launch_letterbox(d_frame.as<uint8_t>(), H, W, flip, d_imgs, o.in, cx.st);
    launch_conv_direct(o, cx.st);
  }
  FFP_HIP(hipStreamSynchronize(cx.st));
  op_download(lout, T, dout, cout, out);
  FFP_API_END
}

int ffp_op_stem_conv(int device, const uint8_t* frame, int H, int W, int chan_order, int n, const int32_t* boxes_xyxy, int imgsz, const float* stem_w,
                     const float* stem_b, int stem_cout, const float* conv_w, const float* conv_b, float* out) {
  FFP_API_BEGIN
  FFP_CHECK(stem_w && stem_b && conv_w && conv_b && out, FFP_ERR_ARG, "stem_conv: null argument");
  op_check_frame("stem_conv", frame, H, W, chan_order, n, boxes_xyxy);
  FFP_CHECK(stem_cout == 16 || stem_cout == 32, FFP_ERR_ARG, "stem_conv: %d stem channels (16 or 32: the loader holds one or two 16-channel chunks)", stem_cout);
  const std::vector<LetterboxImg> lb = op_det_records(H, W, boxes_xyxy, n, imgsz);
  std::vector<int> h0(n), w0(n), h1(n), w1(n), h2(n), w2(n);
  for (int i = 0; i < n; ++i) {
    h0[i] = lb[i].net_h; w0[i] = lb[i].net_w;
    h1[i] = (h0[i] - 1) / 2 + 1; w1[i] = (w0[i] - 1) / 2 + 1;
    h2[i] = (h1[i] - 1) / 2 + 1; w2[i] = (w1[i] - 1) / 2 + 1;
  }
  ScopedStream cx(device, "stem_conv");
  conv_kernels_init();
  const int cc = 2 * stem_cout;
  PackedConv ps, pc;
  pack_conv(ps, "model.0.conv", stem_w, stem_b, stem_cout, 3, 3, 1, F32, cx.st, true);
  pack_conv(pc, "model.1.conv", conv_w, conv_b, cc, stem_cout, 3, 1, F32, cx.st, true);
  Level L0, L1, L2;
  L0.build(h0, w0, cx.st, 32);
  L1.build(h1, w1, cx.st, 32);
  L2.build(h2, w2, cx.st, 32);
  std::vector<unsigned> slots(2 * (size_t)n, 0u);
  {
    const float bound = std::max(ps.out_bound, 0.3f);
    unsigned b;
    std::memcpy(&b, &bound, 4);
    std::fill(slots.begin(), slots.begin() + n, b);
  }
  DevBuf d_frame = op_upload_frame(frame, H, W), d_imgs = upload(lb.data(), lb.size()), dslots = upload(slots.data(), slots.size()),
         dout = op_nan_buffer((size_t)L2.total_px * cc * 4), d_stem_w;
  ConvOp stem, conv;
  stem.pc = &ps; stem.stride = 2; stem.act = ACT_SILU;
  stem.in = TView{nullptr, F32, 4, 0, 4, &L0};
  stem.out = TView{nullptr, F32, stem_cout, 0, stem_cout, &L1};
  stem.out.amax = dslots.as<unsigned>(); stem.out.amax_n = n;
  conv.pc = &pc; conv.stride = 2; conv.act = ACT_SILU;
  conv.in = stem.out;
  conv.out = TView{dout.p, F32, cc, 0, cc, &L2};
  conv.out.amax = dslots.as<unsigned>() + n; conv.out.amax_n = n;
  FFP_CHECK(stem_conv_eligible(stem, conv), FFP_ERR_ARG, "stem_conv: the stem-fused loader refuses this pair of convs");
  const int flip = chan_order == FFP_CHAN_AS_BGR ? 1 : 0;
  stem_conv_pack(stem, flip, d_stem_w, cx.st);
  launch_stem_conv(d_frame.as<uint8_t>(), H, W, d_imgs, d_stem_w, stem, conv, cx.st);
  FFP_HIP(hipStreamSynchronize(cx.st));
  op_download(L2, F32, dout, cc, out);
  FFP_API_END
}

int ffp_op_conv2d_time(int device, int precision, int n, int h, int w, int cin, int cout, int k, int stride, int up, int iters,
                       int dbg_mask, int force_shape, float* out_us) {
  FFP_API_BEGIN
  FFP_CHECK(out_us && n > 0 && iters > 0, FFP_ERR_ARG, "bad arguments");
  ScopedStream cx(device, "conv2d_time");
  conv_kernels_init();
  const DType T = precision == FFP_PREC_F16 ? F16 : F32;
  std::vector<float> wt((size_t)cout * cin * k * k), bias(cout, 0.1f);
  unsigned s = 12345u;
  auto rnd = [&]() { s = s * 1664525u + 1013904223u; return ((s >> 8) & 0xFFFF) / 65536.0f - 0.5f; };
  for (auto& v : wt) v = rnd() * 0.1f;
  PackedConv pc;
  pack_conv(pc, "bench", wt.data(), bias.data(), cout, cin, k, 1, T, cx.st, precision == FFP_PREC_F32X3);
  const int hi = up ? h * 2 : h, wi = up ? w * 2 : w;
  const int ho = (hi + 2 * (k / 2) - k) / stride + 1, wo = (wi + 2 * (k / 2) - k) / stride + 1;
  Level lin, lout;
  lin.build(std::vector<int>(n, h), std::vector<int>(n, w), cx.st);
  lout.build(std::vector<int>(n, ho), std::vector<int>(n, wo), cx.st);
  const size_t nin = (size_t)lin.total_px * pc.cin, nout = (size_t)lout.total_px * cout;
  DevBuf din(nin * dsize(T) + 256), dout(nout * dsize(T) + 256);
  {
    std::vector<float> hx(std::min(nin, (size_t)1 << 22));
    for (auto& v : hx) v = rnd();
    if (T == F32) {
      for (size_t o = 0; o < nin; o += hx.size()) FFP_HIP(hipMemcpy((float*)din.p + o, hx.data(), std::min(hx.size(), nin - o) * 4, hipMemcpyHostToDevice));
    } else {
      std::vector<_Float16> hh(hx.size());
      for (size_t i = 0; i < hx.size(); ++i) hh[i] = (_Float16)hx[i];
      for (size_t o = 0; o < nin; o += hh.size()) FFP_HIP(hipMemcpy((_Float16*)din.p + o, hh.data(), std::min(hh.size(), nin - o) * 2, hipMemcpyHostToDevice));
    }
  }
  ConvOp o;
  o.pc = &pc; o.stride = stride; o.act = precision == FFP_PREC_F16 ? ACT_LRELU : ACT_SILU; o.up = up; o.dbg = dbg_mask; o.force_shape = force_shape;
  o.in = TView{din.p, T, pc.cin, 0, pc.cin, &lin};
  o.out = TView{dout.p, T, cout, 0, cout, &lout};
  std::unique_ptr<TrunkPlan> tp;
  if (force_shape == SHAPE_TRUNK) tp.reset(new TrunkPlan(std::vector<ConvOp>{o}));
  auto once = [&]() { if (tp) tp->launch(cx.st, dbg_mask); else launch_conv(o, cx.st); };
  for (int i = 0; i < 3; ++i) once();
  ScopedEvent e0, e1;
  FFP_HIP(hipEventRecord(e0, cx.st));
  for (int i = 0; i < iters; ++i) once();
  FFP_HIP(hipEventRecord(e1, cx.st));
  FFP_HIP(hipStreamSynchronize(cx.st));
  float ms = 0.f;
  FFP_HIP(hipEventElapsedTime(&ms, e0, e1));
  *out_us = ms * 1e3f / iters;
  FFP_API_END
}

int ffp_op_resize_lanczos4(int device, const void* src, int h, int w, int channels, int bits, int out_h, int out_w, void* dst) {
  FFP_API_BEGIN
  FFP_CHECK(src && dst, FFP_ERR_ARG, "resize_lanczos4: null argument");
  FFP_CHECK(h >= 1 && w >= 1 && out_h >= 1 && out_w >= 1, FFP_ERR_ARG, "resize_lanczos4: empty image (%dx%d -> %dx%d)", h, w, out_h, out_w);
  FFP_CHECK(channels == 1 || channels == 3 || channels == 4, FFP_ERR_ARG, "resize_lanczos4: channels %d (1, 3 or 4)", channels);
  FFP_CHECK(bits == 8 || bits == 16, FFP_ERR_ARG, "resize_lanczos4: bits %d (8 or 16)", bits);
  const int wide = bits == 16;
  const size_t in_bytes = ((size_t)h * w * channels) << wide, out_bytes = ((size_t)out_h * out_w * channels) << wide;
  if (out_h == h && out_w == w) {
    std::memcpy(dst, src, out_bytes);
    return FFP_OK;
  }
  std::vector<uint8_t> host_tab;
  ScopedStream cx(device, "resize_lanczos4");
  DevBuf din(in_bytes), dout(out_bytes), tab;
  FFP_HIP(hipMemcpyAsync(din.p, src, in_bytes, hipMemcpyHostToDevice, cx.st));
  resize_lanczos4_dev(din.p, h, w, channels, wide, out_h, out_w, dout.p, tab, host_tab, cx.st);
  FFP_HIP(hipStreamSynchronize(cx.st));
  FFP_HIP(hipMemcpy(dst, dout.p, out_bytes, hipMemcpyDeviceToHost));
  FFP_API_END
}

}
```

### face-detection-with-yolov11-sahi-and-real-esrgan_amd/csrc/conv_args.hpp

```cpp
#pragma once
#include "conv_route.hpp"
#include "dw_bound.hpp"
#include "ops.hpp"

namespace ffp {

typedef float f32x16 __attribute__((ext_vector_type(16)));
typedef _Float16 f16x8 __attribute__((ext_vector_type(8)));

struct ConvArgs {
  const void* in;
  const void* wpk;
  const float* bias;
  void* out;
  const void* res1;
  const void* res2;
  const int4* in_tab;
  const int4* out_tab;
  const int4* tiles;
  long long total_px;
  int in_cs, in_coff, cin, cin_pad;
  int out_cs, out_coff, cout;
  int r1_cs, r1_coff, r2_cs, r2_coff;
  float s1, s2;
  int act_post;
  int act, out_f32, up, n_nblk, ncg, ntiles32, vec_ok, fast_out;
  int force_shape;
  int dbg;
  const void* up_src;
  const int* up_map;
  int up_c, up_cs;
  const void* zeros;
  const unsigned* amax_in;
  const unsigned* amax_in2;
  unsigned* amax_out;
  const float* oscale;
  int amax_img;
  const int* frag_img;
  int ntiles_host;
  const int* n_tiles_dev;
  const unsigned char* st_frame;
  const LetterboxImg* st_imgs;
  const int4* st_tab;
  const void* st_w;
  const float* st_bias;
  int st_W;
  long long st_bytes;
  float st_scale;
  const int* gate;
};

__device__ __forceinline__ int live_workgroups(const ConvArgs& a) {
  return a.n_tiles_dev ? __builtin_amdgcn_readfirstlane(*a.n_tiles_dev) * a.n_nblk : (int)gridDim.x;
}

__device__ __forceinline__ int xcd_remap(int b, int nwg) {
  const int xcd = b & 7, q = nwg >> 3, r = nwg & 7;
  return (xcd < r ? xcd * (q + 1) : r * (q + 1) + (xcd - r) * q) + (b >> 3);
}

__device__ __forceinline__ int sload(const void* p, int idx) {
  typedef const __attribute__((address_space(4))) int* cptr;
  return reinterpret_cast<cptr>(reinterpret_cast<unsigned long long>(p))[idx];
}

__device__ __forceinline__ unsigned wave_max_bits(float mx) {
  int v = __float_as_int(mx);
  v = max(v, __builtin_amdgcn_update_dpp(0, v, 0xB1, 0xF, 0xF, true));
  v = max(v, __builtin_amdgcn_update_dpp(0, v, 0x4E, 0xF, 0xF, true));
  v = max(v, __builtin_amdgcn_update_dpp(0, v, 0x141, 0xF, 0xF, true));
  v = max(v, __builtin_amdgcn_update_dpp(0, v, 0x140, 0xF, 0xF, true));
  const int a = max(__builtin_amdgcn_readlane(v, 0), __builtin_amdgcn_readlane(v, 16));
  const int b = max(__builtin_amdgcn_readlane(v, 32), __builtin_amdgcn_readlane(v, 48));
  return (unsigned)max(a, b);
}

__device__ __forceinline__ unsigned slot_peek(const unsigned* slot) {
  return __hip_atomic_load(slot, __ATOMIC_RELAXED, __HIP_MEMORY_SCOPE_AGENT);
}
__device__ __forceinline__ void raise_amax(unsigned* slot, float mx, unsigned old) {
  const unsigned b = wave_max_bits(mx);
  if ((threadIdx.x & 63) == 0 && b > old) atomicMax(slot, b);
}
__device__ __forceinline__ void raise_amax(unsigned* slot, float mx) {
  const unsigned b = wave_max_bits(mx);
  if ((threadIdx.x & 63) == 0 && b > slot_peek(slot)) atomicMax(slot, b);
}

__device__ __forceinline__ unsigned amax_in_bits(const ConvArgs& a, int img) {
  if (!a.amax_in) return 0u;
  const int i = a.amax_img ? img : 0;
  unsigned m = a.amax_in[i];
  if (a.amax_in2) m = max(m, a.amax_in2[i]);
  return m;
}
__device__ __forceinline__ unsigned amax_in_bits_s(const ConvArgs& a, int img) {
  if (!a.amax_in) return 0u;
  const int i = a.amax_img ? img : 0;
  unsigned m = (unsigned)sload(a.amax_in, i);
  if (a.amax_in2) m = max(m, (unsigned)sload(a.amax_in2, i));
  return m;
}

__device__ __forceinline__ void split_scales(unsigned amax_bits, float* t, float* tinv) {
  split_scales_hd(amax_bits, t, tinv);
}

__device__ __forceinline__ void split_pair(float x0, float x1, float t, unsigned& hi, unsigned& lo) {
  unsigned h, l;
  asm("v_fma_mixlo_f16 %0, %1, %2, 0" : "=v"(h) : "v"(x0), "v"(t));
  asm("v_fma_mixhi_f16 %0, %1, %2, 0" : "+v"(h) : "v"(x1), "v"(t));
  asm("v_fma_mixlo_f16 %0, %1, %2, -%3 op_sel:[0,0,0] op_sel_hi:[0,0,1]" : "=v"(l) : "v"(x0), "v"(t), "v"(h));
  asm("v_fma_mixhi_f16 %0, %1, %2, -%3 op_sel:[0,0,1] op_sel_hi:[0,0,1]" : "+v"(l) : "v"(x1), "v"(t), "v"(h));
  hi = h;
  lo = l;
}

__device__ __forceinline__ float act_fn(float v, int act) {
  if (act == ACT_SILU) return v / (1.0f + expf(-v));
  if (act == ACT_LRELU) return v >= 0.f ? v : v * 0.2f;
  if (act == ACT_RELU) return fmaxf(v, 0.f);
  return v;
}

__device__ __forceinline__ float apply_act(float v, int act) {
  if (act == ACT_SILU) return v * __builtin_amdgcn_rcpf(1.0f + __expf(-v));
  if (act == ACT_LRELU) return v >= 0.f ? v : v * 0.2f;
  if (act == ACT_RELU) return fmaxf(v, 0.f);
  return v;
}

constexpr unsigned BUF_OOB = 0xFFFFFFFFu;
__device__ __forceinline__ auto buf_rsrc(const unsigned char* p, unsigned bytes = 0x7FFFFFF0) {
  const unsigned long long u = reinterpret_cast<unsigned long long>(p);
  const unsigned lo = __builtin_amdgcn_readfirstlane((unsigned)u), hi = __builtin_amdgcn_readfirstlane((unsigned)(u >> 32));
  return __builtin_amdgcn_make_buffer_rsrc(reinterpret_cast<unsigned char*>(((unsigned long long)hi << 32) | lo), 0, bytes, 0x00020000);
}
typedef decltype(buf_rsrc(nullptr)) buf_rsrc_t;
__device__ __forceinline__ uint4 buf_load16(buf_rsrc_t rs, unsigned off, int soff = 0) {
  const auto v = __builtin_amdgcn_raw_buffer_load_b128(rs, off, soff, 0);
  return make_uint4(v[0], v[1], v[2], v[3]);
}
struct EpiCaps { unsigned acts; bool res, act_post, out_f16, out_f32; };
constexpr unsigned EPI_ALL_ACTS = 1u << ACT_NONE | 1u << ACT_SILU | 1u << ACT_LRELU | 1u << ACT_RELU;
inline bool epilogue_fits(int act, bool res, int act_post, DType out, const EpiCaps& caps) {
  return act >= 0 && act < 32 && (caps.acts >> act & 1u) && (!res || caps.res) && (!act_post || caps.act_post) && (out == F16 ? caps.out_f16 : caps.out_f32);
}
inline bool epilogue_fits(const ConvOp& op, const EpiCaps& caps) { return epilogue_fits(op.act, op.has_res1 || op.has_res2, op.act_post, op.out.dt, caps); }

ConvArgs make_conv_args(const ConvOp& op);
unsigned conv_generic_mask(const ConvOp& op, const ConvArgs& a);
int conv_generic_choose(const ConvOp& op, const ConvArgs& a);
void launch_conv_generic(ConvArgs& a, int shape, const ConvOp& op, hipStream_t st);
bool conv_rows_eligible(const ConvOp& op, const ConvArgs& a, int shape);
void launch_conv_rows(ConvArgs& a, int shape, Level* out_lvl, hipStream_t st);
void conv_rows_init();
bool conv_rows16_eligible(const ConvOp& op, const ConvArgs& a, int shape);
void launch_conv_rows16(ConvArgs& a, int shape, const PackedConv& pc, Level* out_lvl, hipStream_t st);
void conv_rows16_init();
unsigned rows16_grid(int n_tiles, int n_nblk, int min_ws, int tcap, const char* what);
void launch_conv_rows16pc(ConvArgs& a, const PackedConv& pc, Level* out_lvl, hipStream_t st);
void conv_rows16pc_init();
unsigned conv_pw_mask(const ConvOp& op, const ConvArgs& a);
void launch_conv_pw(ConvArgs& a, int shape, hipStream_t st);
void conv_pw_init();

bool conv_dwpw_eligible(const ConvOp& op, bool need_storage = true);
void launch_conv_dwpw(const ConvOp& op, hipStream_t st);
void conv_dwpw_init();

unsigned conv_k3d_mask(const ConvOp& op, const ConvArgs& a);
void launch_conv_k3d(ConvArgs& a, int shape, int stride, Level* out_lvl, hipStream_t st);
void conv_k3d_init();

}
```

### face-detection-with-yolov11-sahi-and-real-esrgan_amd/csrc/conv_k3d.hip

```cpp
#include <algorithm>
#include <cstdlib>
#include <type_traits>

#include "conv_args.hpp"

#ifndef FFP_K3D_DBG
#define FFP_K3D_DBG 0
#endif

namespace ffp {

namespace {

typedef unsigned u32x4 __attribute__((ext_vector_type(4)));

template <int S, int WM, int WN, int MI, int NIW> struct K3Geo {
  static_assert(WM * WN == 4 && (S == 1 || S == 2), "geometry");
  static constexpr int TH = 2 * WM * MI;
  static constexpr int HH = (TH - 1) * S + 3, HWD = 15 * S + 3;
  static constexpr int RP = HWD;
  static constexpr int PP = 17;
  static constexpr int NPX = HH * HWD;
  static constexpr int NPIECE = ((NPX * 4 + 63) / 64 + 3) / 4 * 4;
  static constexpr int NPW = NPIECE / 4;
  static constexpr int STAGE = NPIECE * 16 * 64;
  static constexpr int EROW = 144;
  static constexpr int SCR = 4 * 32 * EROW;
  static constexpr bool SCR_IN_STAGE = STAGE >= SCR;
  static constexpr int TCAP = 32;
  static constexpr int DESC = 2 * STAGE + (SCR_IN_STAGE ? 0 : SCR);
  static constexpr int LDS = DESC + TCAP * 48;
  static constexpr int NTB = WN * NIW;
  static constexpr int OCC = (MI * NIW * 16 > 64 || LDS > 80 * 1024) ? 1 : 2;
  static constexpr int NSET = ((OCC == 2 && MI * NIW * 16 + 2 * NPW * 4 > 120) || NPW > 9) ? 1 : 2;
  static constexpr int MPS = 3 * NIW * MI;
  static constexpr int AD = MPS >= 12 ? 2 : MPS >= 6 ? 5 : 8;
};

template <int S, int WM, int WN, int MI, int NIW>
__global__ void __launch_bounds__(256, (K3Geo<S, WM, WN, MI, NIW>::OCC)) conv_k3d_kernel(const ConvArgs a) {
  using G = K3Geo<S, WM, WN, MI, NIW>;
  constexpr int NPW = G::NPW, RP = G::RP, HWD = G::HWD, NPX = G::NPX;
  extern __shared__ __attribute__((aligned(16))) unsigned char smem[];

  const int tid = threadIdx.x, lane = tid & 63;
  const int wave = __builtin_amdgcn_readfirstlane(tid >> 6);
  const int DBG = FFP_K3D_DBG ? a.dbg : 0;
  const int wm = wave % WM, wn = wave / WM;
  const int p = lane & 31, hh = lane >> 5;

  const int n_items = (a.n_tiles_dev ? __builtin_amdgcn_readfirstlane(*a.n_tiles_dev) : a.ntiles_host) * a.n_nblk;
  const int Ws = (int)gridDim.x >> 3;
  const int xcd = blockIdx.x & 7, slot = blockIdx.x >> 3;
  int per_xcd = (n_items + 7) >> 3;
  per_xcd = (per_xcd + a.n_nblk - 1) / a.n_nblk * a.n_nblk;
  const int first = xcd * per_xcd + slot;
  const int last = min(n_items, (xcd + 1) * per_xcd);
  const int J = first < last ? min((last - first + Ws - 1) / Ws, G::TCAP) : 0;
  if (J == 0) return;
  const int nb0 = first % a.n_nblk;

  int4* desc = reinterpret_cast<int4*>(smem + G::DESC);
  if (tid < J) {
    const int4 t = a.tiles[(first + tid * Ws) / a.n_nblk];
    desc[tid * 3] = t;
    desc[tid * 3 + 1] = a.in_tab[t.x];
    desc[tid * 3 + 2] = a.out_tab[t.x];
  }
  __syncthreads();

  constexpr unsigned OOB = 0xFFFFFFFFu;
  auto uniform_ptr = [](const unsigned char* q) {
    const unsigned long long u = reinterpret_cast<unsigned long long>(q);
    const unsigned lo = __builtin_amdgcn_readfirstlane((unsigned)u), hi = __builtin_amdgcn_readfirstlane((unsigned)(u >> 32));
    return reinterpret_cast<unsigned char*>(((unsigned long long)hi << 32) | lo);
  };
  auto sgpr = [](int v) { return __builtin_amdgcn_readfirstlane(v); };
  const int NC = a.cin >> 4;
  const unsigned char* wb = reinterpret_cast<const unsigned char*>(a.wpk);
  const auto rs_w = __builtin_amdgcn_make_buffer_rsrc(uniform_ptr(wb), 0, 0x7FFFFFF0, 0x00020000);
  auto rs_in = rs_w;
  auto bload = [](decltype(rs_w) rs, unsigned off, int soff = 0) {
    const auto v = __builtin_amdgcn_raw_buffer_load_b128(rs, off, soff, 0);
    return make_uint4(v[0], v[1], v[2], v[3]);
  };

  float pf_ts = 1.f;
  auto item_scales = [&](int img, float* ts, float* ti) {
    *ts = 1.f; *ti = 1.f;
    if (a.amax_in) split_scales(amax_in_bits_s(a, img), ts, ti);
  };

  auto rec_of = [](int hy, int hx) { return S == 1 ? hy * RP + hx : hy * RP + (hx & 1) * G::PP + (hx >> 1); };
  auto swz_of = [](int hy, int hx) { return S == 1 ? (((hx >> 1) & 2) ^ (hy & 1)) : ((((hx >> 1) >> 1) & 2) ^ ((hy >> 1) & 1)); };

  unsigned isrc[NPW];
  unsigned idst[NPW];
  unsigned hyx[NPW];
#pragma unroll
  for (int i = 0; i < NPW; ++i) {
    const int idx = (wave + 4 * i) * 64 + lane;
    const int px = idx >> 2, q = idx & 3;
    const int hy = px / HWD, hx = px - hy * HWD;
    const int rec = px < NPX ? rec_of(hy, hx) : px;
    const int x = px < NPX ? swz_of(hy, hx) : 0;
    idst[i] = (unsigned)(rec * 64 + (((q >> 1) ^ x) << 4) + ((q & 1) << 3));
    hyx[i] = px < NPX ? (unsigned)((q << 16) | (hy << 8) | hx) : 0xFFFFu;
  }
  int pf_item = 0, pf_c = 0;
  auto setup_pf = [&](int j) {
    const int4 t = desc[j * 3], it = desc[j * 3 + 1];
    const int oy0 = sgpr(t.y), ox0 = sgpr(t.z), Hi = sgpr(it.y), Wi = sgpr(it.z);
    float ti_unused;
    item_scales(sgpr(t.x), &pf_ts, &ti_unused);
    const unsigned char* inb = reinterpret_cast<const unsigned char*>(a.in) + ((long long)sgpr(it.x) * a.in_cs + a.in_coff) * 4;
    rs_in = __builtin_amdgcn_make_buffer_rsrc(uniform_ptr(inb), 0, 0x7FFFFFF0, 0x00020000);
#pragma unroll
    for (int i = 0; i < NPW; ++i) {
      const int hy = (int)(hyx[i] >> 8) & 0xFF, hx = (int)hyx[i] & 0xFF, q = (int)(hyx[i] >> 16);
      const int iy = oy0 * S - 1 + hy, ix = ox0 * S - 1 + hx;
      const bool ok = (hyx[i] & 0xFFFFu) != 0xFFFFu && (unsigned)iy < (unsigned)Hi && (unsigned)ix < (unsigned)Wi;
      isrc[i] = ok ? (unsigned)((iy * Wi + ix) * a.in_cs * 4 + q * 16) : OOB;
    }
  };
  constexpr int NSET = G::NSET;
  uint4 set[NSET][NPW];
  float set_ts[NSET];
  auto piece_fetch = [&](int k, int i, unsigned after = 0u) {
    unsigned off = isrc[i] != OOB ? isrc[i] + (unsigned)(pf_c * 64) : OOB;
    asm("" : "+v"(off) : "v"(after));
    if (!(DBG & 4)) set[k][i] = bload(rs_in, off);
  };
  auto piece_stash = [&](unsigned char* sb, int k, int i) {
    uint2 hi, lo;
    split_pair(__uint_as_float(set[k][i].x), __uint_as_float(set[k][i].y), set_ts[k], hi.x, lo.x);
    split_pair(__uint_as_float(set[k][i].z), __uint_as_float(set[k][i].w), set_ts[k], hi.y, lo.y);
    unsigned d = idst[i];
    asm volatile("" : "+v"(d));
    *reinterpret_cast<uint2*>(sb + idst[i]) = hi;
    *reinterpret_cast<uint2*>(sb + (d ^ 32u)) = lo;
    return lo.x ^ lo.y;
  };
  auto advance_pf = [&]() {
    if (pf_item >= J) return;
    if (++pf_c == NC) {
      pf_c = 0;
      if (++pf_item < J) setup_pf(pf_item);
      else rs_in = __builtin_amdgcn_make_buffer_rsrc(uniform_ptr(wb), 0, 0, 0x00020000);
    }
  };

  int wbase[NIW];
#pragma unroll
  for (int ni = 0; ni < NIW; ++ni) wbase[ni] = min(nb0 * G::NTB + wn * NIW + ni, a.ntiles32 - 1) * 9 * a.ncg * 2048;
  const unsigned wlane = (unsigned)lane * 16u;
  constexpr int AD = G::AD, AR = AD + 1;
  static_assert(18 % AR == 0 && AD < 9, "A ring");
  uint4 aq[AR][2 * NIW];
  auto ldA = [&](int tap, int cg, int r) {
#pragma unroll
    for (int ni = 0; ni < NIW; ++ni) {
      const int so = __builtin_amdgcn_readfirstlane(wbase[ni] + (tap * a.ncg + cg) * 2048);
      if (DBG & 16) continue;
      aq[r][ni] = bload(rs_w, wlane, so);
      aq[r][NIW + ni] = bload(rs_w, wlane, so + 1024);
    }
  };

  unsigned boff[3][2];
  {
    const int r0 = p >> 4, c0 = p & 15;
#pragma unroll
    for (int kx = 0; kx < 3; ++kx)
#pragma unroll
      for (int cls = 0; cls < 2; ++cls) {
        const int hy = S == 1 ? 2 * wm * MI + r0 + cls : 2 * (2 * wm * MI + r0) + 2 * cls;
        const int hx = c0 * S + kx;
        boff[kx][cls] = (unsigned)(rec_of(hy, hx) * 64 + ((hh ^ swz_of(hy, hx)) << 4));
      }
  }

  f32x16 acc[NIW][MI];
  auto zero_acc = [&]() {
#pragma unroll
    for (int ni = 0; ni < NIW; ++ni)
#pragma unroll
      for (int mi = 0; mi < MI; ++mi)
#pragma unroll
        for (int r = 0; r < 16; ++r) acc[ni][mi][r] = 0.f;
  };
  zero_acc();

  float amax_run = 0.f;

  auto chunk = [&](auto phase_tag, const unsigned char* sb, unsigned char* sbn, int cg, int cg_next) __attribute__((always_inline)) {
    constexpr int PH = decltype(phase_tag)::value * 9;
    constexpr int KS = NSET == 2 ? decltype(phase_tag)::value : 0;
    uint4 bq[2][2 * MI];
    unsigned tok[NPW];
    auto ldB = [&](int s, int r) {
      const int ky = s / 3, kx = s - 3 * ky;
      const int cls = S == 1 ? (ky & 1) : (ky >> 1);
      const int kyo = S == 1 ? ky - cls : ky - 2 * cls;
      unsigned ol = boff[kx][cls];
      asm volatile("" : "+v"(ol));
      ol ^= 32u;
#pragma unroll
      for (int mi = 0; mi < MI; ++mi) {
        if (DBG & 32) continue;
        const unsigned ro = (unsigned)(((S == 1 ? 2 * mi : 4 * mi) + kyo) * RP * 64);
        bq[r][mi] = *reinterpret_cast<const uint4*>(sb + boff[kx][cls] + ro);
        bq[r][MI + mi] = *reinterpret_cast<const uint4*>(sb + ol + ro);
      }
    };
    ldB(0, 0);
    __builtin_amdgcn_sched_barrier(0);
#pragma unroll
    for (int s = 0; s < 9; ++s) {
      if (s + 1 < 9) ldB(s + 1, (s + 1) & 1);
      if (s + AD < 9) ldA(s + AD, cg, (PH + s + AD) % AR);
      else ldA(s + AD - 9, cg_next, (PH + s + AD) % AR);
      if (s >= 2) {
#pragma unroll
        for (int i = (s - 2) * NPW / 7; i < (s - 1) * NPW / 7; ++i) tok[i] = (DBG & 8) ? 0u : piece_stash(sbn, KS, i);
      }
      if (s == 8) {
#pragma unroll
        for (int i = 0; i < NPW; ++i) piece_fetch(KS, i, tok[i]);
        set_ts[KS] = pf_ts;
      }
#pragma unroll
      for (int ni = 0; ni < NIW; ++ni)
#pragma unroll
        for (int mi = 0; mi < MI; ++mi) {
          union { uint4 u; f16x8 h; } ah, al, bh, bl;
          if (DBG & 2) continue;
          ah.u = aq[(PH + s) % AR][ni]; al.u = aq[(PH + s) % AR][NIW + ni]; bh.u = bq[s & 1][mi]; bl.u = bq[s & 1][MI + mi];
          acc[ni][mi] = __builtin_amdgcn_mfma_f32_32x32x16_f16(al.h, bh.h, acc[ni][mi], 0, 0, 0);
          acc[ni][mi] = __builtin_amdgcn_mfma_f32_32x32x16_f16(ah.h, bl.h, acc[ni][mi], 0, 0, 0);
          acc[ni][mi] = __builtin_amdgcn_mfma_f32_32x32x16_f16(ah.h, bh.h, acc[ni][mi], 0, 0, 0);
        }
#pragma unroll
      for (int r = 0; r < 3 * NIW * MI; ++r) {
        __builtin_amdgcn_sched_group_barrier(0x008, 1, 0);
        __builtin_amdgcn_sched_group_barrier(0x7F6, 3, 0);
      }
      __builtin_amdgcn_sched_barrier(0);
    }
    advance_pf();
  };

  auto epilogue = [&](int j, unsigned char* scr) __attribute__((always_inline)) {
    const int4 t = desc[j * 3], ot = desc[j * 3 + 2];
    const int oy0 = sgpr(t.y), ox0 = sgpr(t.z), Ho = sgpr(ot.y), Wo = sgpr(ot.z);
    const int img = sgpr(t.x);
    float ts_unused, tinv;
    item_scales(img, &ts_unused, &tinv);
    float am = 0.f;
    unsigned slot_now = 0u;
    if (a.amax_img && a.amax_out) slot_now = slot_peek(a.amax_out + img);
    const long long out_base = sgpr(ot.x);
    const unsigned char* r1b = a.res1 ? reinterpret_cast<const unsigned char*>(a.res1) + (out_base * a.r1_cs + a.r1_coff) * 4 : wb;
    const unsigned char* r2b = a.res2 ? reinterpret_cast<const unsigned char*>(a.res2) + (out_base * a.r2_cs + a.r2_coff) * 4 : wb;
    unsigned char* ob = reinterpret_cast<unsigned char*>(a.out) + (out_base * a.out_cs + a.out_coff) * 4;
    const auto rs_r1 = __builtin_amdgcn_make_buffer_rsrc(uniform_ptr(r1b), 0, 0x7FFFFFF0, 0x00020000);
    const auto rs_r2 = __builtin_amdgcn_make_buffer_rsrc(uniform_ptr(r2b), 0, 0x7FFFFFF0, 0x00020000);
    const auto rs_o = __builtin_amdgcn_make_buffer_rsrc(uniform_ptr(ob), 0, 0x7FFFFFF0, 0x00020000);
    unsigned char* et = scr + wave * (32 * G::EROW);
    const int ch0 = (lane & 7) * 4;
#pragma unroll
    for (int mi = 0; mi < MI; ++mi) {
      const int f = wm * MI + mi;
#pragma unroll
      for (int ni = 0; ni < NIW; ++ni) {
        const int nt = nb0 * G::NTB + wn * NIW + ni;
        if (nt >= a.ntiles32) continue;
        const int chb = nt * 32 + ch0;
        const float4 bv = *reinterpret_cast<const float4*>(a.bias + chb);
        const float4 sv = a.oscale ? *reinterpret_cast<const float4*>(a.oscale + chb) : make_float4(1.f, 1.f, 1.f, 1.f);
        const float bias_t[4] = {bv.x, bv.y, bv.z, bv.w};
        const float osc_t[4] = {sv.x * tinv, sv.y * tinv, sv.z * tinv, sv.w * tinv};
        unsigned rel[4];
        bool oks[4];
        uint4 r1v[4], r2v[4];
#pragma unroll
        for (int it = 0; it < 4; ++it) {
          const int pp = it * 8 + (lane >> 3);
          const int oy = oy0 + 2 * f + (pp >> 4), ox = ox0 + (pp & 15);
          oks[it] = oy < Ho && ox < Wo && nt * 32 + ch0 < a.cout;
          rel[it] = (unsigned)(oy * Wo + ox);
          r1v[it] = make_uint4(0u, 0u, 0u, 0u); r2v[it] = r1v[it];
          if (a.res1) r1v[it] = bload(rs_r1, oks[it] ? (rel[it] * a.r1_cs + nt * 32 + ch0) * 4 : OOB);
          if (a.res2) r2v[it] = bload(rs_r2, oks[it] ? (rel[it] * a.r2_cs + nt * 32 + ch0) * 4 : OOB);
        }
        asm volatile("s_waitcnt lgkmcnt(0)" ::: "memory");
#pragma unroll
        for (int g = 0; g < 4; ++g)
          *reinterpret_cast<float4*>(et + p * G::EROW + (8 * g + 4 * hh) * 4) =
              make_float4(acc[ni][mi][4 * g + 0], acc[ni][mi][4 * g + 1], acc[ni][mi][4 * g + 2], acc[ni][mi][4 * g + 3]);
        asm volatile("s_waitcnt lgkmcnt(0)" ::: "memory");
#pragma unroll
        for (int it = 0; it < 4; ++it) {
          const int pp = it * 8 + (lane >> 3);
          const float4 t4 = *reinterpret_cast<const float4*>(et + pp * G::EROW + ch0 * 4);
          float v[4] = {t4.x, t4.y, t4.z, t4.w};
#pragma unroll
          for (int q = 0; q < 4; ++q) v[q] = apply_act(fmaf(v[q], osc_t[q], bias_t[q]), a.act);
          if (a.res1) {
            const float* r = reinterpret_cast<const float*>(&r1v[it]);
#pragma unroll
            for (int q = 0; q < 4; ++q) v[q] = v[q] * a.s1 + r[q];
          }
          if (a.res2) {
            const float* r = reinterpret_cast<const float*>(&r2v[it]);
#pragma unroll
            for (int q = 0; q < 4; ++q) v[q] = v[q] * a.s2 + r[q];
          }
          if (a.act_post) {
#pragma unroll
            for (int q = 0; q < 4; ++q) v[q] = apply_act(v[q], a.act_post);
          }
          if (oks[it]) {
#pragma unroll
            for (int q = 0; q < 4; ++q) am = fmaxf(am, fabsf(v[q]));
          }
          u32x4 ov = {__float_as_uint(v[0]), __float_as_uint(v[1]), __float_as_uint(v[2]), __float_as_uint(v[3])};
          __builtin_amdgcn_raw_buffer_store_b128(ov, rs_o, oks[it] ? (rel[it] * a.out_cs + nt * 32 + ch0) * 4 : OOB, 0, 0);
        }
      }
    }
    asm volatile("s_waitcnt lgkmcnt(0)" ::: "memory");
    if (a.amax_img) { if (a.amax_out) raise_amax(a.amax_out + img, am, slot_now); }
    else amax_run = fmaxf(amax_run, am);
  };

  const int Q = J * NC;
  int cj = 0, cc = 0;
  setup_pf(0);
#pragma unroll
  for (int i = 0; i < NPW; ++i) piece_fetch(0, i);
  set_ts[0] = pf_ts;
  advance_pf();
#pragma unroll
  for (int t = 0; t < AD; ++t) ldA(t, 0, t);
#pragma unroll
  for (int i = 0; i < NPW; ++i) piece_fetch(0, i, piece_stash(smem, 0, i));
  set_ts[0] = pf_ts;
  advance_pf();
  if constexpr (NSET == 2) {
#pragma unroll
    for (int i = 0; i < NPW; ++i) piece_fetch(1, i);
    set_ts[1] = pf_ts;
    advance_pf();
  }
  __syncthreads();
  auto step_chunk = [&](auto phase_tag, unsigned char* sb, unsigned char* sbn) __attribute__((always_inline)) {
    const int cn = cc + 1 == NC ? 0 : cc + 1;
    chunk(phase_tag, sb, sbn, cc, cn);
    if (++cc == NC) {
      if constexpr (G::SCR_IN_STAGE) __syncthreads();
      if (!(DBG & 1)) epilogue(cj, G::SCR_IN_STAGE ? sb : smem + 2 * G::STAGE);
      zero_acc();
      cc = 0; ++cj;
    }
    if (!(DBG & 64)) __syncthreads();
  };
  for (int q = 0; q < Q; q += 2) {
    step_chunk(std::integral_constant<int, 0>{}, smem, smem + G::STAGE);
    if (q + 1 >= Q) break;
    step_chunk(std::integral_constant<int, 1>{}, smem + G::STAGE, smem);
  }
  if (a.amax_out && !a.amax_img) raise_amax(a.amax_out, amax_run);
}

template <int S, int WM, int WN, int MI, int NIW> struct K3Cfg {
  using G = K3Geo<S, WM, WN, MI, NIW>;
  static_assert(G::LDS <= 160 * 1024, "conv_k3d: LDS");
  static void init() {
    FFP_HIP(hipFuncSetAttribute(reinterpret_cast<const void*>(&conv_k3d_kernel<S, WM, WN, MI, NIW>), hipFuncAttributeMaxDynamicSharedMemorySize, G::LDS));
  }
  static void launch(ConvArgs& a, Level* out_lvl, hipStream_t st) {
    int n_tiles = 0;
    a.tiles = out_lvl->tile_table(G::TH, &n_tiles, &a.n_tiles_dev, st, a.gate);
    if (n_tiles == 0) return;
    a.ntiles_host = n_tiles;
    a.n_nblk = (a.ntiles32 + G::NTB - 1) / G::NTB;
    const long long items = (long long)n_tiles * a.n_nblk;
    long long per_xcd = (items + 7) / 8;
    per_xcd = (per_xcd + a.n_nblk - 1) / a.n_nblk * a.n_nblk;
    static const int ws_env = [] { const char* e = getenv("FFP_K3D_WS"); return e ? atoi(e) : 0; }();
    long long ws = std::max<long long>(ws_env > 0 ? ws_env : 32 * G::OCC, (per_xcd + G::TCAP - 1) / G::TCAP);
    ws = (ws + a.n_nblk - 1) / a.n_nblk * a.n_nblk;
    FFP_CHECK(8 * ws < (1ll << 31) && (per_xcd + ws - 1) / ws <= G::TCAP, FFP_ERR_STATE, "conv_k3d: launch geometry");
    hipLaunchKernelGGL((conv_k3d_kernel<S, WM, WN, MI, NIW>), dim3((unsigned)(8 * ws)), dim3(256), G::LDS, st, a);
  }
};

template <int S> struct K3Family {
  using V0 = K3Cfg<S, 2, 2, 2, 2>;
  using V1 = K3Cfg<S, 2, 2, 2, 1>;
  using V2 = K3Cfg<S, 4, 1, 1, 1>;
  using V3 = K3Cfg<S, 2, 2, 4, 2>;
  using V4 = K3Cfg<S, 2, 2, 4, 1>;
  static void init() { V0::init(); V1::init(); V2::init(); V3::init(); V4::init(); }
  static void launch(ConvArgs& a, int shape, Level* out_lvl, hipStream_t st) {
    switch (shape) {
      case SHAPE_K3D_128: V0::launch(a, out_lvl, st); break;
      case SHAPE_K3D_64: V1::launch(a, out_lvl, st); break;
      case SHAPE_K3D_32: V2::launch(a, out_lvl, st); break;
      case SHAPE_K3D_128X256: V3::launch(a, out_lvl, st); break;
      case SHAPE_K3D_64X256: V4::launch(a, out_lvl, st); break;
      default: fail(FFP_ERR_ARG, "conv_k3d: shape %d", shape);
    }
  }
};

}

void conv_k3d_init() { K3Family<1>::init(); K3Family<2>::init(); }

static constexpr EpiCaps kEpiK3d{EPI_ALL_ACTS, true, true, false, true};
unsigned conv_k3d_mask(const ConvOp& op, const ConvArgs& a) {
  const PackedConv& pc = *op.pc;
  if (!(epilogue_fits(op, kEpiK3d) && pc.split && pc.dt == F32 && pc.k == 3 && (op.stride == 1 || op.stride == 2) && !op.up && !op.has_up2 && a.fast_out &&
        pc.cin % 16 == 0 && pc.cin_pad == pc.cin && op.in.lvl->n > 0))
    return 0;
  long long max_px = 0;
  for (int i = 0; i < op.in.lvl->n; ++i) max_px = std::max(max_px, (long long)op.in.lvl->h[i] * op.in.lvl->w[i]);
  long long max_opx = 0;
  for (int i = 0; i < op.out.lvl->n; ++i) max_opx = std::max(max_opx, (long long)op.out.lvl->h[i] * op.out.lvl->w[i]);
  const long long cs_max = std::max<long long>(op.out.cs, std::max(op.has_res1 ? op.res1.cs : 0, op.has_res2 ? op.res2.cs : 0));
  if (max_px * op.in.cs * 4 >= 0x7FFFFFF0ll || max_opx * cs_max * 4 >= 0x7FFFFFF0ll) return 0;
  unsigned m = shape_bit(SHAPE_K3D_32);
  if (a.ntiles32 >= 2) m |= shape_bit(SHAPE_K3D_64) | shape_bit(SHAPE_K3D_64X256);
  if (a.ntiles32 >= 3) m |= shape_bit(SHAPE_K3D_128) | shape_bit(SHAPE_K3D_128X256);
  return m;
}

void launch_conv_k3d(ConvArgs& a, int shape, int stride, Level* out_lvl, hipStream_t st) {
  if (stride == 1) K3Family<1>::launch(a, shape, out_lvl, st);
  else K3Family<2>::launch(a, shape, out_lvl, st);
}

}
```

### face-detection-with-yolov11-sahi-and-real-esrgan_amd/csrc/conv_route.cpp

```cpp
#include "conv_route.hpp"

#include <algorithm>

#include "api_util.hpp"
#include "conv_args.hpp"
#include "engine.hpp"
#include "trunk.hpp"

namespace ffp {

namespace {

using F = ConvFamily;
constexpr ConvShapeInfo kShapes[SHAPE_COUNT] = {
    {SHAPE_WIDE, F::GENERIC, "generic", "wide"},         {SHAPE_WIDE_H, F::GENERIC, "generic", "wideH"},
    {SHAPE_NARROW2, F::GENERIC, "generic", "narrow2"},   {SHAPE_NARROW2_H, F::GENERIC, "generic", "narrow2H"},
    {SHAPE_NARROW1, F::GENERIC, "generic", "narrow1"},   {SHAPE_NARROW1_H, F::GENERIC, "generic", "narrow1H"},
    {SHAPE_ROWS, F::ROWS, "rows", "rows"},               {SHAPE_ROWS_3STAGE, F::ROWS, "rows", "rows"},
    {SHAPE_ROWS_2TILE, F::ROWS, "rows", "rows"},         {SHAPE_ROWS16, F::ROWS16, "rows16", "rows16"},
    {SHAPE_PW_1X4, F::PW, "pw", "pw1x4"},                {SHAPE_PW_2X2, F::PW, "pw", "pw2x2"},
    {SHAPE_PW_2X1, F::PW, "pw", "pw2x1"},                {SHAPE_PW_1X4W, F::PW, "pw", "pw1x4w"},
    {SHAPE_PW_2X2W, F::PW, "pw", "pw2x2w"},              {SHAPE_PW_2X1W, F::PW, "pw", "pw2x1w"},
    {SHAPE_PW_1X4S, F::PW, "pw", "pw1x4s"},              {SHAPE_K3D_128, F::K3D, "k3d", "d128"},
    {SHAPE_K3D_64, F::K3D, "k3d", "d64"},                {SHAPE_K3D_32, F::K3D, "k3d", "d32"},
    {SHAPE_K3D_128X256, F::K3D, "k3d", "d128x256"},      {SHAPE_K3D_64X256, F::K3D, "k3d", "d64x256"},
    {SHAPE_PW_2X2S, F::PW, "pw", "pw2x2s"},              {SHAPE_ROWS16_RES, F::ROWS16, "rows16", "rows16"},
    {SHAPE_ROWS16PC, F::ROWS16PC, "rows16pc", "rows16pc"}, {SHAPE_TRUNK, F::TRUNK, "trunk", "trunk"},
};
constexpr ConvShapeInfo kDwPw{SHAPE_DWPW, F::DWPW, "dwpw", "dw3"};
constexpr bool table_in_order() {
  for (int i = 0; i < SHAPE_COUNT; ++i) if (kShapes[i].shape != i) return false;
  return true;
}
static_assert(table_in_order(), "conv shape table: row i holds shape i");
static_assert(SHAPE_COUNT <= 32 && SHAPE_DWPW >= 32, "forceable shapes fit a 32-bit candidate mask; route-only numbers lie above them");

bool env_is(const char* name, char c) {
  const char* e = getenv(name);
  return e && e[0] == c;
}
struct Switches { bool rows16, rows16_res, rows16_pc, pw, k3d; };
const Switches& switches() {
  static const Switches s{!env_is("FFP_ROWS16", '0'), env_is("FFP_ROWS16_RES", '1'), env_is("FFP_ROWS16_PC", '1'), !env_is("FFP_PW", '0'), !env_is("FFP_K3D", '0')};
  return s;
}

bool family_runs(ConvFamily family, int shape, const ConvOp& op, const ConvArgs& a) {
  switch (family) {
    case F::GENERIC: return true;
    case F::ROWS: return conv_rows_eligible(op, a, shape);
    case F::ROWS16:
    case F::ROWS16PC: return conv_rows16_eligible(op, a, shape);
    case F::PW: return conv_pw_mask(op, a) & shape_bit(shape);
    case F::K3D: return conv_k3d_mask(op, a) & shape_bit(shape);
    case F::TRUNK: return conv_trunk_layer_ok(op);
    case F::DWPW: return conv_dwpw_eligible(op);
    case F::DIRECT: break;
  }
  return false;
}

}

const ConvShapeInfo* conv_shape_info(int shape) {
  if (shape < 0 || shape >= SHAPE_COUNT) return nullptr;
  return &kShapes[shape];
}

const ConvShapeInfo* conv_route_info(int shape) { return shape == SHAPE_DWPW ? &kDwPw : conv_shape_info(shape); }

ConvArgs conv_route_args(const ConvOp& op) { return op.dw || conv_direct_eligible(op) ? ConvArgs{} : make_conv_args(op); }

ConvRoute conv_route(const ConvOp& op, const ConvArgs& a) {
  if (op.dw) {
    FFP_CHECK((op.force_shape < 0 || op.force_shape == SHAPE_DWPW) && conv_dwpw_eligible(op), FFP_ERR_ARG, "conv %s: the depthwise-fused kernel cannot run this op", op.pc->name.c_str());
    return {F::DWPW, SHAPE_DWPW};
  }
  if (conv_direct_eligible(op)) {
    FFP_CHECK(!op.gate, FFP_ERR_ARG, "conv %s: the image-input kernel cannot honour a gate", op.pc->name.c_str());
    return {F::DIRECT, SHAPE_AUTO};
  }
  if (op.force_shape >= 0) {
    const ConvShapeInfo* s = conv_shape_info(op.force_shape);
    FFP_CHECK(s, FFP_ERR_ARG, "conv %s: %d is not a shape number", op.pc->name.c_str(), op.force_shape);
    FFP_CHECK(family_runs(s->family, s->shape, op, a), FFP_ERR_ARG, "conv %s: %s shape %d cannot run this op", op.pc->name.c_str(), s->family_name, s->shape);
    return {s->family, s->shape};
  }
  const Switches& sw = switches();
  if (sw.rows16 && conv_rows16_eligible(op, a, SHAPE_ROWS16)) {
    if (sw.rows16_pc && a.dbg == 0) return {F::ROWS16PC, SHAPE_ROWS16PC};
    if (sw.rows16_res && conv_rows16_eligible(op, a, SHAPE_ROWS16_RES)) return {F::ROWS16, SHAPE_ROWS16_RES};
    return {F::ROWS16, SHAPE_ROWS16};
  }
  if (conv_rows_eligible(op, a, SHAPE_ROWS)) return {F::ROWS, SHAPE_ROWS};
  return {F::GENERIC, conv_generic_choose(op, a)};
}

unsigned conv_candidates(const ConvOp& op, const ConvArgs& a) {
  const Switches& sw = switches();
  return conv_generic_mask(op, a) | (sw.pw ? conv_pw_mask(op, a) : 0u) | (sw.k3d ? conv_k3d_mask(op, a) : 0u);
}

void launch_conv(const ConvOp& op, hipStream_t st) {
  ConvArgs a = conv_route_args(op);
  const ConvRoute r = conv_route(op, a);
  switch (r.family) {
    case F::DIRECT: launch_conv_direct(op, st); return;
    case F::GENERIC: launch_conv_generic(a, r.shape, op, st); break;
    case F::ROWS: launch_conv_rows(a, r.shape, op.out.lvl, st); break;
    case F::ROWS16: launch_conv_rows16(a, r.shape, *op.pc, op.out.lvl, st); break;
    case F::ROWS16PC: launch_conv_rows16pc(a, *op.pc, op.out.lvl, st); break;
    case F::PW: launch_conv_pw(a, r.shape, st); break;
    case F::K3D: launch_conv_k3d(a, r.shape, op.stride, op.out.lvl, st); break;
    case F::DWPW: launch_conv_dwpw(op, st); break;
    case F::TRUNK: {
      TrunkPlan tp(std::vector<ConvOp>{op});
      tp.launch(st, op.dbg);
      FFP_HIP(hipStreamSynchronize(st));
      return;
    }
  }
  FFP_HIP(hipGetLastError());
}

std::string conv_variant(const ConvOp& op) {
  const PackedConv& pc = *op.pc;
  const ConvRoute r = conv_route(op, conv_route_args(op));
  if (r.family == F::DIRECT) return std::string(pc.dt == F32 ? "f32" : "f16") + "_k3_direct";
  char buf[64];
  snprintf(buf, sizeof(buf), "%s_k%ds%d_%s", pc.dt == F16 ? "f16" : pc.split ? "f32x3" : "f32", pc.k, op.stride, conv_route_info(r.shape)->suffix);
  return buf;
}

int conv_tune(const ConvOp& op, hipStream_t st) {
  const PackedConv& pc = *op.pc;
  const ConvArgs a = conv_route_args(op);
  const ConvRoute r = conv_route(op, a);
  if (op.force_shape >= 0 || r.family != F::GENERIC) return -1;
  const unsigned mask = conv_candidates(op, a);
  if (__builtin_popcount(mask) < 2) return -1;
  const int heur = r.shape;
  ScopedEvent e0, e1;
  auto time_shape = [&](int shape, int iters) {
    ConvOp o = op;
    o.force_shape = shape;
    o.gate = nullptr;
    FFP_HIP(hipEventRecord(e0, st));
    for (int i = 0; i < iters; ++i) launch_conv(o, st);
    FFP_HIP(hipEventRecord(e1, st));
    FFP_HIP(hipEventSynchronize(e1));
    float ms = 0.f;
    FFP_HIP(hipEventElapsedTime(&ms, e0, e1));
    return ms * 1e3f / iters;
  };
  float best_t = 0.f, heur_t = 0.f;
  int best = -1;
  for (int shape = 0; shape < SHAPE_COUNT; ++shape) {
    if (!(mask & shape_bit(shape))) continue;
    const float t1 = time_shape(shape, 2);
    const int iters = std::min(24, std::max(3, (int)(300.f / std::max(t1, 1.f))));
    const float t = time_shape(shape, iters);
    if (shape == heur) heur_t = t;
    if (best < 0 || t < best_t) { best = shape; best_t = t; }
    static const bool log = [] { const char* e = getenv("FFP_TUNE_LOG"); return e && e[0] == '1'; }();
    if (log) {
      ConvOp o = op;
      o.force_shape = shape;
      fprintf(stderr, "[tune] %-28s %4d->%4d k%d s%d px %9lld  shape %2d %-22s %9.1f us%s\n", pc.name.c_str(), pc.cin_real, pc.cout, pc.k, op.stride,
              (long long)op.out.lvl->actual_px(), shape, conv_variant(o).c_str(), t, shape == heur ? "  (heuristic)" : "");
    }
  }
  if (heur_t > 0.f && best_t > 0.97f * heur_t) return heur;
  return best;
}

}
```

### face-detection-with-yolov11-sahi-and-real-esrgan_amd/csrc/conv_route.hpp

```cpp
#pragma once
#include "ops.hpp"

namespace ffp {

struct ConvArgs;

enum ConvShape : int {
  SHAPE_AUTO = -1,
  SHAPE_WIDE = 0, SHAPE_WIDE_H, SHAPE_NARROW2, SHAPE_NARROW2_H, SHAPE_NARROW1, SHAPE_NARROW1_H,
  SHAPE_ROWS = 6, SHAPE_ROWS_3STAGE, SHAPE_ROWS_2TILE,
  SHAPE_ROWS16 = 9,
  SHAPE_PW_1X4 = 10, SHAPE_PW_2X2, SHAPE_PW_2X1, SHAPE_PW_1X4W, SHAPE_PW_2X2W, SHAPE_PW_2X1W,
  SHAPE_PW_1X4S = 16,
  SHAPE_K3D_128 = 17, SHAPE_K3D_64, SHAPE_K3D_32, SHAPE_K3D_128X256, SHAPE_K3D_64X256,
  SHAPE_PW_2X2S = 22,
  SHAPE_ROWS16_RES = 23,
  SHAPE_ROWS16PC = 24,
  SHAPE_TRUNK = 25,
  SHAPE_COUNT,
  SHAPE_DWPW = 64
};
constexpr unsigned shape_bit(int shape) { return 1u << shape; }

enum class ConvFamily { DIRECT, GENERIC, ROWS, ROWS16, ROWS16PC, PW, K3D, TRUNK, DWPW };

struct ConvShapeInfo { int shape; ConvFamily family; const char* family_name; const char* suffix; };
const ConvShapeInfo* conv_shape_info(int shape);
const ConvShapeInfo* conv_route_info(int shape);

struct ConvRoute { ConvFamily family; int shape; };
ConvRoute conv_route(const ConvOp& op, const ConvArgs& a);
ConvArgs conv_route_args(const ConvOp& op);
unsigned conv_candidates(const ConvOp& op, const ConvArgs& a);

}
```

### face-detection-with-yolov11-sahi-and-real-esrgan_amd/csrc/engine.cpp

```cpp
#include "engine.hpp"
#include "conv_route.hpp"

#include <mutex>

#include <shared_mutex>

#include <cstdlib>

namespace ffp {

ConvProfile::~ConvProfile() {
  for (auto& e : ev) { (void)hipEventDestroy(e.first); (void)hipEventDestroy(e.second); }
}

void ConvProfile::begin() {
  table.clear();
  pending.clear();
  detail.clear();
}

int ConvProfile::open(hipStream_t st) {
  const int slot = (int)pending.size();
  if (slot >= (int)ev.size()) {
    hipEvent_t a, b;
// ... 175 lines not shown
  FFP_CHECK(amax_init.size() + ns <= amax_cap_slots, FFP_ERR_STATE, "plan: more than %d buffers", AMAX_CAP);
  FFP_CHECK(!per_image_amax || l->px_align % 32 == 0, FFP_ERR_STATE, "plan: per-image exponent slots need levels aligned to 32 pixels");
  v.amax = amax_slots.as<unsigned>() + amax_init.size();
  v.amax_n = ns;
  amax_init.insert(amax_init.end(), ns, 0u);
  return v;
}

void Plan::set_amax_bound(const TView& v, float bound) {
  FFP_CHECK(v.amax && amax_slots.p, FFP_ERR_STATE, "plan: view has no max-|value| slot");
  unsigned b;
  std::memcpy(&b, &bound, 4);
  for (int i = 0; i < v.amax_n; ++i) amax_init[(v.amax - amax_slots.as<unsigned>()) + i] = b;
}

void Plan::add_amax_reset(hipStream_t st) {
  if (amax_init.empty()) return;
  amax_init_dev.alloc(sizeof(unsigned) * amax_init.size());
  FFP_HIP(hipMemcpyAsync(amax_init_dev.p, amax_init.data(), sizeof(unsigned) * amax_init.size(), hipMemcpyHostToDevice, st));
  FFP_HIP(hipStreamSynchronize(st));
  unsigned* slots = amax_slots.as<unsigned>();
  const unsigned* init = amax_init_dev.as<unsigned>();
  const int n = (int)amax_init.size();
  if (reset_outside) {
    reset_fn = [slots, init, n](hipStream_t q) { launch_amax_init(slots, init, n, q); };
    return;
  }
  Step s;
  s.run = [slots, init, n](hipStream_t q) { launch_amax_init(slots, init, n, q); };
  steps.insert(steps.begin(), std::move(s));
}

void Plan::add_conv(const ConvOp& op) {
  Step s;
  ConvOp o = op;
  o.flops = conv_flops_of(*op.pc, op.out.lvl->actual_px()) + (op.fin ? conv_flops_of(*op.fin, op.out.lvl->actual_px()) : 0.0);
  s.is_conv = true;
  s.variant = conv_variant(o);
  s.name = op.label.empty() ? op.pc->name : op.label;
  s.flops = o.flops;
  s.conv = std::make_shared<ConvOp>(o);
  std::shared_ptr<ConvOp> cp = s.conv;
  s.lane = cur_lane;
  s.run = [cp](hipStream_t st) { launch_conv(*cp, st); };
  conv_flops += o.flops;
  conv_launches += 1;
  steps.push_back(std::move(s));
}

void Plan::add_trunk(const std::vector<ConvOp>& ops) {
  Step s;
  s.is_conv = true;
  s.trunk = std::make_shared<TrunkPlan>(ops);
  for (const ConvOp& op : ops) {
    ConvOp o = op;
    o.flops = conv_flops_of(*op.pc, op.out.lvl->actual_px());
    o.force_shape = SHAPE_TRUNK;
    s.fused.push_back(std::make_shared<ConvOp>(o));
    s.flops += o.flops;
  }
  s.conv = s.fused.front();
  s.variant = conv_variant(*s.conv);
  s.name = ops.front().pc->name + ".." + ops.back().pc->name;
  s.lane = cur_lane;
  std::shared_ptr<TrunkPlan> tp = s.trunk;
  s.run = [tp](hipStream_t st) { tp->launch(st); };
  conv_flops += s.flops;
  conv_launches += 1;
  steps.push_back(std::move(s));
}

namespace {
std::shared_mutex g_gate;
thread_local int tl_shared_depth = 0;
}

ApiShared::ApiShared() {
  if (tl_shared_depth++ == 0) g_gate.lock_shared();
}
ApiShared::~ApiShared() {
  if (--tl_shared_depth == 0) g_gate.unlock_shared();
}
CaptureExclusive::CaptureExclusive() {
  if (tl_shared_depth > 0) g_gate.unlock_shared();
  g_gate.lock();
}
CaptureExclusive::~CaptureExclusive() {
  g_gate.unlock();
  if (tl_shared_depth > 0) g_gate.lock_shared();
}

Plan::~Plan() {
  if (gexec) (void)hipGraphExecDestroy(gexec);
  if (graph) (void)hipGraphDestroy(graph);
  for (Step& s : steps) if (s.ev) (void)hipEventDestroy(s.ev);
  for (hipStream_t q : lane_streams) (void)hipStreamDestroy(q);
}

int Plan::lanes_env() {
  static const int m = [] { const char* e = getenv("FFP_LANES"); return e ? atoi(e) : -1; }();
  return m;
}

void Plan::fork(int lane) {
  if (!lanes_enabled() || lane <= 0) return;
  while ((int)lane_streams.size() < lane) {
    hipStream_t q;
    FFP_HIP(hipStreamCreateWithFlags(&q, hipStreamNonBlocking));
    lane_streams.push_back(q);
  }
  Step s;
  s.kind = 1; s.lane = lane;
  FFP_HIP(hipEventCreateWithFlags(&s.ev, hipEventDisableTiming));
  steps.push_back(std::move(s));
  pool().fork();
}

void Plan::join(int lane) {
  if (!lanes_enabled() || lane <= 0) return;
  Step s;
  s.kind = 2; s.lane = lane;
  FFP_HIP(hipEventCreateWithFlags(&s.ev, hipEventDisableTiming));
  steps.push_back(std::move(s));
  std::vector<int> flushed;
  FFP_CHECK(pool().join(&flushed), FFP_ERR_STATE, "plan: join without an open fork");
  ranges_freed += (int)flushed.size();
  if (reuse == 2) for (int id : flushed) add_fill(id);
}

void Plan::run_steps(hipStream_t st, bool use_lanes) {
  for (Step& s : steps) {
    hipStream_t q = (use_lanes && s.lane > 0) ? lane_streams[s.lane - 1] : st;
    if (s.kind == 1) {
      if (use_lanes) { FFP_HIP(hipEventRecord(s.ev, st)); FFP_HIP(hipStreamWaitEvent(q, s.ev, 0)); }
    } else if (s.kind == 2) {
      if (use_lanes) { FFP_HIP(hipEventRecord(s.ev, q)); FFP_HIP(hipStreamWaitEvent(st, s.ev, 0)); }
    } else {
      s.run(q);
    }
  }
}

static bool graphs_enabled() {
  static const bool on = [] { const char* e = getenv("FFP_NO_GRAPH"); return !(e && e[0] == '1'); }();
  return on;
}

void Plan::tune(hipStream_t st) {
  tuned = true;
  static const bool off = [] { const char* e = getenv("FFP_NO_TUNE"); return e && e[0] == '1'; }();
  if (off) return;
  for (Step& s : steps) {
    if (!s.is_conv || s.trunk || s.conv->force_shape >= 0) continue;
    const int best = conv_tune(*s.conv, st);
    if (best >= 0) {
      s.conv->force_shape = best;
      s.variant = conv_variant(*s.conv);
    }
  }
}

void Plan::execute(hipStream_t st, ConvProfile* prof) {
  if (!tuned) tune(st);
  if (g_totals_on) totals_add(steps);
  const bool p = prof && prof->enabled;
  if (p) {
    for (Step& s : steps) {
      if (s.kind != 0) continue;
      if (s.is_conv) {
        const int slot = prof->open(st);
        s.run(st);
        prof->close(slot, st, s.variant, s.actual_flops(), s.name, s.actual_bytes(), s.share);
      } else {
        s.run(st);
      }
    }
    return;
  }
  if (runs > 0 && graph_ok && graphs_enabled()) {
    if (!gexec) {
      CaptureExclusive only_me;
      if (hipStreamBeginCapture(st, hipStreamCaptureModeThreadLocal) == hipSuccess) {
        bool ok = true;
        try {
          run_steps(st, true);
        } catch (...) {
          ok = false;
        }
        hipGraph_t g = nullptr;
        if (hipStreamEndCapture(st, &g) != hipSuccess || !ok || !g) {
          graph_ok = ++capture_failures < 3;
          if (!graph_ok) fprintf(stderr, "libffp: hipGraph capture failed %d times, this plan keeps launching eagerly (ffp_*_graph_status reports -1)\n", capture_failures);
          if (g) (void)hipGraphDestroy(g);
          hipStreamCaptureStatus cs = hipStreamCaptureStatusNone;
          if (hipStreamIsCapturing(st, &cs) == hipSuccess && cs != hipStreamCaptureStatusNone) { g = nullptr; (void)hipStreamEndCapture(st, &g); if (g) (void)hipGraphDestroy(g); }
          (void)hipGetLastError();
        } else if (hipGraphInstantiate(&gexec, g, nullptr, nullptr, 0) != hipSuccess) {
          graph_ok = false;
          gexec = nullptr;
          fprintf(stderr, "libffp: hipGraphInstantiate failed, this plan keeps launching eagerly (ffp_*_graph_status reports -1)\n");
          (void)hipGraphDestroy(g);
          (void)hipGetLastError();
        } else {
          graph = g;
        }
      } else {
        graph_ok = false;
        (void)hipGetLastError();
      }
    }
    if (gexec) {
      FFP_HIP(hipGraphLaunch(gexec, st));
      ++runs;
      return;
    }
  }
  run_steps(st, runs > 0);
  ++runs;
}

}
```

### face-detection-with-yolov11-sahi-and-real-esrgan_amd/csrc/ops.hpp

```cpp
#pragma once
#include "common.hpp"
#include "weights.hpp"

namespace ffp {

struct DenseF32 { DevBuf w, b; };

struct ConvOp {
  const PackedConv* pc = nullptr;
  TView in, out;
  int stride = 1;
  int act = ACT_NONE;
  int act_post = ACT_NONE;
  int up = 0;
  bool has_res1 = false, has_res2 = false;
  TView res1, res2;
  float s1 = 1.f, s2 = 1.f;
  bool has_up2 = false;
  TView up2;
  int up2_c = 0;
  const int* up2_map = nullptr;
  double flops = 0;
  int dbg = 0;
  const int* gate = nullptr;
  const PackedConv* dw = nullptr;
  int dw_act = ACT_NONE;
  const PackedConv* fin = nullptr;
  const DenseF32* fin_w = nullptr;
  TView fin_out;
  std::string label;
  int dwpw_force = 0;
  int force_shape = -1;
};
void launch_conv(const ConvOp& op, hipStream_t st);
bool conv_direct_eligible(const ConvOp& op);
void launch_conv_direct(const ConvOp& op, hipStream_t st);
void conv_kernels_init();
int conv_tune(const ConvOp& op, hipStream_t st);
bool stem_conv_eligible(const ConvOp& stem, const ConvOp& conv);
void stem_conv_pack(const ConvOp& stem, int flip, DevBuf& out, hipStream_t st);
void launch_stem_conv(const uint8_t* d_frame, int H, int W, const DevBuf& d_imgs, const DevBuf& stem_w, const ConvOp& stem, const ConvOp& conv, hipStream_t st);

struct DwConvOp {
  const PackedConv* pc = nullptr;
  TView in, out;
  int act = ACT_NONE;
  int grp = 0, grp_stride = 0, grp_off = 0;
  bool has_res = false;
  TView res;
  int force = 0;
};
void launch_dwconv(const DwConvOp& op, hipStream_t st);
void launch_amax_init(unsigned* slots, const unsigned* init, int n, hipStream_t st);
void launch_amax_max(unsigned* dst, const unsigned* src, hipStream_t st, int n = 1);

void launch_sppf_pool(const TView& in, const TView& y1, const TView& y2, const TView& y3, hipStream_t st, int force = 0);

void launch_upsample2x(const TView& in, const TView& out, hipStream_t st);

void launch_psa_attention(const TView& qkv, const TView& out, int nh, int kd, int hd, hipStream_t st, int force = 0);

struct LetterboxImg {
  int x0, y0, sw, sh;
  int new_w, new_h;
  int top, left;
  int net_h, net_w;
};
void launch_letterbox(const uint8_t* d_frame, int H, int W, int flip, const DevBuf& d_imgs ,
                      const TView& out, hipStream_t st);

void launch_stem_from_frame(const uint8_t* d_frame, int H, int W, int flip, const DevBuf& d_imgs, const ConvOp& op, hipStream_t st);

}
```

### include/ffp.h

```cpp
#ifndef FFP_H
#define FFP_H

#include <stddef.h>
#include <stdint.h>

#ifdef __cplusplus
extern "C" {
#endif

#define FFP_OK 0
#define FFP_ERR_ARG 1
#define FFP_ERR_HIP 2
#define FFP_ERR_WEIGHTS 3
#define FFP_ERR_NOMEM 4
#define FFP_ERR_STATE 5

#define FFP_PREC_F32 0
#define FFP_PREC_F16 1
#define FFP_PREC_F32X3 2

#define FFP_CHAN_AS_BGR 0
#define FFP_CHAN_AS_RGB 1

#define FFP_PP_NMS 0
#define FFP_PP_GREEDYNMM 1
#define FFP_METRIC_IOU 0
#define FFP_METRIC_IOS 1

#define FFP_DET_STRIDE(nkpt) (6 + 3 * (nkpt))

typedef struct ffp_det ffp_det;
typedef struct ffp_sr ffp_sr;

const char* ffp_last_error(void);
int ffp_version(void);
int ffp_device_count(int* out_n);


int ffp_slice_bboxes(int image_h, int image_w, int slice_h, int slice_w, float overlap_h_ratio, float overlap_w_ratio,
                     int32_t* out_xyxy, int cap, int32_t* out_n);

int ffp_tile_chunks(int n, int max_batch, int32_t* out, int cap, int32_t* out_n);

int ffp_letterbox_geometry(int h, int w, int imgsz, int32_t* out6);


int ffp_det_create(const void* weights, size_t nbytes, int arch, int nc, int nkpt, int device, int precision,
                   ffp_det** out);
void ffp_det_destroy(ffp_det* d);

int ffp_det_infer_tiles(ffp_det* d, const uint8_t* frame_hwc, int H, int W, int chan_order,
                        const int32_t* tiles_xyxy, int n_tiles, int imgsz, float conf, float iou, int max_det,
                        int round_boxes, float* out_dets, int32_t* out_counts);

int ffp_det_infer_tiles_dev(ffp_det* d, const uint8_t* d_frame_hwc, int H, int W, int chan_order,
                            const int32_t* tiles_xyxy_host, int n_tiles, int imgsz, float conf, float iou,
                            int max_det, int round_boxes, float* d_out_dets, int32_t* d_out_counts);

int ffp_det_truncate_shift_dev(ffp_det* d, float* d_dets, const int32_t* d_counts, int n_tiles, int max_det, int full_h,
                               int full_w);

int ffp_det_forward_raw(ffp_det* d, const uint8_t* frame_hwc, int H, int W, int chan_order,
                        const int32_t* tiles_xyxy, int n_tiles, int imgsz, float* out_raw, size_t out_cap,
                        int32_t* out_anchor_counts);


int ffp_merge(int device, const float* dets, int n, int stride, int type, int metric, double thr, int class_agnostic,
              float* out, int32_t* out_src_index, int32_t* out_n);

int ffp_sliced_predict(ffp_det* d, const uint8_t* frame_hwc, int H, int W, int chan_order, int slice_h, int slice_w,
                       float overlap_h_ratio, float overlap_w_ratio, int perform_standard_pred, int imgsz,
                       float conf, float iou, int max_det, int round_boxes, int pp_type, int pp_metric, double pp_thr,
                       int class_agnostic, float* out, int cap, int32_t* out_n);

int ffp_det_stage_dev(ffp_det* d, const uint8_t* d_frame_hwc, int H, int W, int chan_order, int slice_h, int slice_w,
                      float overlap_h_ratio, float overlap_w_ratio, int perform_standard_pred, int imgsz, float conf,
                      float iou, int max_det, int round_boxes, int rank, int world, float* d_local_dets,
                      int32_t* d_local_counts, int32_t* out_n_local, int32_t* out_n_total);

int ffp_merge_dev(ffp_det* d, const float* d_dets, const int32_t* d_counts, int n_slices, int max_det, int type,
                  int metric, double thr, int class_agnostic, float* d_out, int cap, int32_t* d_out_n);


int ffp_sr_create(const void* weights, size_t nbytes, int scale, int num_block, int device, int half, ffp_sr** out);
void ffp_sr_destroy(ffp_sr* s);

int ffp_sr_enhance(ffp_sr* s, const uint8_t* bgr_hwc, int h, int w, int tile, int tile_pad, int pre_pad,
                   uint8_t* out_bgr);

int ffp_sr_enhance_dev(ffp_sr* s, const uint8_t* d_bgr_hwc, int h, int w, int tile, int tile_pad, int pre_pad, uint8_t* d_out_bgr);

#define FFP_SR_ALPHA_REALESRGAN 0
#define FFP_SR_ALPHA_LINEAR 1
int ffp_sr_enhance_ex(ffp_sr* s, const void* img, int h, int w, int channels, int bits, int max_range, int alpha_mode, int out_h,
                      int out_w, int tile, int tile_pad, int pre_pad, void* out);

int ffp_sr_enhance_batch(ffp_sr* s, int n, const uint8_t* const* imgs, const int32_t* hs, const int32_t* ws, int tile,
                         int tile_pad, int pre_pad, uint8_t* const* outs);

int ffp_sr_enhance_crops_dev(ffp_sr* s, const uint8_t* d_frame_bgr, int H, int W, const int32_t* boxes_xyxy, int n, int tile,
                             int tile_pad, uint8_t* d_out, size_t out_cap, int64_t* out_offsets);

int ffp_sr_enhance_crops_dev_async(ffp_sr* s, const uint8_t* d_frame_bgr, int H, int W, const int32_t* boxes_xyxy, int n, int tile,
                                   int tile_pad, uint8_t* d_out, size_t out_cap, int64_t* out_offsets);
int ffp_sr_wait(ffp_sr* s);
int ffp_sr_enhance_crops_multi_dev_async(ffp_sr* s, int n_frames, const uint8_t* const* d_frames, const int32_t* frame_of_box,
                                         int H, int W, const int32_t* boxes_xyxy, int n, int tile, int tile_pad, uint8_t* d_out,
                                         size_t out_cap, int64_t* out_offsets);

int ffp_sr_plan_state(ffp_sr* s, int32_t* out_plans_built, int32_t* out_last_graph);
int ffp_sr_set_fused_body(ffp_sr* s, int on);
int ffp_sr_mem_bytes(ffp_sr* s, uint64_t* out_weight_bytes, uint64_t* out_plan_bytes, int32_t* out_plans_resident);
int ffp_det_drop_plans(ffp_det* d);
int ffp_sr_drop_plans(ffp_sr* s);
int ffp_det_mem_bytes(ffp_det* d, uint64_t* out_weight_bytes, uint64_t* out_plan_bytes, int32_t* out_plans_resident);
int ffp_det_set_buffer_reuse(ffp_det* d, int mode);
int ffp_det_mem_detail(ffp_det* d, uint64_t* out_activation_bytes, uint64_t* out_no_reuse_bytes, uint64_t* out_peak_live_bytes);
int ffp_det_fill_steps(ffp_det* d, int32_t* out_fill_steps, int32_t* out_ranges_freed);
int ffp_det_graph_status(ffp_det* d, int32_t* out_state);
int ffp_det_set_lanes(ffp_det* d, int mode);
int ffp_det_set_gate(ffp_det* d, int on);
int ffp_det_last_active(ffp_det* d, int32_t* out_active, int32_t* out_items);
int ffp_det_stream_wait_event(ffp_det* d, void* hip_event);


int ffp_op_resize_lanczos4(int device, const void* src, int h, int w, int channels, int bits, int out_h, int out_w, void* dst);

int ffp_op_conv2d(int device, int precision, const float* x, int n, int h, int w, int cin, const float* wt,
                  const float* bias, int cout, int k, int stride, int groups, int act, int up, const float* res,
                  float res_scale, float* y);


int ffp_eval_wider_pr(int device, const double* preds, const int64_t* pred_off, const double* gts, const int64_t* gt_off, const uint8_t* evaluate,
                      int n_img, double iou_thr, int thresh_num, int64_t* out_counts);

int ffp_eval_dual_match(int device, const double* preds, const int64_t* pred_off, const double* faces, const int64_t* face_off, const uint8_t* valid,
                        int n_img, double iou_thr, int32_t* out_flags);

int ffp_eval_coco_bbox(int device, int n_img, int n_cat, const double* dets, const int64_t* det_off, const double* gts, const int64_t* gt_off,
                       const double* iou_thrs, int n_iou, const double* rec_thrs, int n_rec, const double* area_rng, int n_area,
                       const int32_t* max_dets, int n_max_dets, double* precision, double* recall, double* scores, double* dt_matches,
                       uint8_t* dt_ignore, double* gt_matches, uint8_t* gt_ignore);


int ffp_jpeg_encode(int device, const uint8_t* img, int h, int w, int bgr, int quality, uint8_t* out, int64_t cap, int64_t* out_size);
int ffp_jpeg_encode_dev(int device, const uint8_t* d_img, int h, int w, int64_t row_stride, int bgr, int quality, uint8_t* out, int64_t cap,
                        int64_t* out_size);
int ffp_jpeg_encode_batch_dev(int device, const uint8_t* d_base, int n, const int64_t* offsets, const int32_t* hs, const int32_t* ws, const int64_t* strides,
                              int bgr, int quality, uint8_t* out, int64_t cap, int64_t* out_offsets);

int ffp_jpeg_info(const uint8_t* data, int64_t n, int32_t* out_h, int32_t* out_w, int32_t* out_ncomp);
int ffp_jpeg_decode(int device, const uint8_t* data, int64_t n, int bgr, uint8_t* out, int64_t cap);
int ffp_jpeg_decode_dev(int device, const uint8_t* data, int64_t n, int bgr, uint8_t* d_out, int64_t row_stride, int64_t cap);
int ffp_jpeg_decode_stats(int64_t* device_decodes, int64_t* host_fallbacks, int64_t* extra_sync_rounds);


int64_t ffp_png_bound(int h, int w, int channels, int bit_depth);
int ffp_png_segment_bytes(void);
int ffp_png_encode(int device, const void* img, int h, int w, int channels, int bit_depth, int bgr, int level, uint8_t* out, int64_t cap, int64_t* out_size);
int ffp_png_encode_dev(int device, const void* d_img, int h, int w, int channels, int bit_depth, int64_t row_stride, int bgr, int level, uint8_t* out, int64_t cap,
                       int64_t* out_size);
int ffp_png_encode_batch_dev(int device, const void* d_base, int n, const int64_t* offsets, const int32_t* hs, const int32_t* ws, const int64_t* strides,
                             int channels, int bit_depth, int bgr, int level, uint8_t* out, int64_t cap, int64_t* out_offsets);

int ffp_op_conv1x1_up2(int device, int precision, const float* coarse, const float* fine, int n, int h, int w, int c_up, int c_fine,
                       const float* wt, const float* bias, int cout, int act, float* y);

int ffp_op_conv2d_shape(int force_shape);
int ffp_op_conv2d_shape_name(int shape, char* out, int cap);
int ffp_op_conv2d_last_variant(char* out, int cap);
int ffp_op_conv2d_act_post(int act);


int ffp_op_variant(int family, int variant);
int ffp_op_cls_tower_variant(int rows, int wg_cap);

int ffp_op_sppf_pool(int device, int precision, int n, const int32_t* hs, const int32_t* ws, int px_align, int c, const float* x, int x_cs,
                     int x_coff, float* y, int y_cs, int y1_coff, int y2_coff, int y3_coff);

int ffp_op_upsample2x(int device, int precision, int n, const int32_t* hs, const int32_t* ws, int px_align, int c, const float* x, int x_cs,
                      int x_coff, float* y, int y_cs, int y_coff);

int ffp_op_psa_attention(int device, int precision, int n, const int32_t* hs, const int32_t* ws, int px_align, int nh, const float* qkv, int q_cs,
                         int q_coff, float* out, int o_cs, int o_coff);

int ffp_op_dwconv3x3(int device, int precision, int n, const int32_t* hs, const int32_t* ws, int px_align, int c, const float* x, int x_cs,
                     int x_coff, int grp, int grp_stride, int grp_off, const float* wt, const float* bias, int act, const float* res, int r_cs,
                     int r_coff, float* y, int y_cs, int y_coff);

int ffp_op_cls_tower(int device, int n, const int32_t* hs, const int32_t* ws, int px_align, int cin, int nc, const float* x, const float* dw0_w,
                     const float* dw0_b, const float* pw0_w, const float* pw0_b, const float* dw1_w, const float* dw1_b, const float* pw1_w,
                     const float* pw1_b, const float* fin_w, const float* fin_b, float* e1, float* head, int head_cs, int head_coff, int64_t* stray);

int ffp_op_conv2d_views(int device, int precision, int n, const int32_t* hs, const int32_t* ws, int px_align, const float* x, int x_cs, int x_coff,
                        int cin, const float* wt, const float* bias, int cout, int k, int stride, int act, int act_post, int up, const float* res1,
                        int r1_cs, int r1_coff, float s1, const float* res2, int r2_cs, int r2_coff, float s2, float* y, int y_cs, int y_coff,
                        int per_image_amax, uint32_t* amax_out, const int32_t* gate, const int32_t* gate_prev, int64_t* stray);

int ffp_op_det_post(int device, int n, const int32_t* hs, const int32_t* ws, int px_align, int nc, int nkpt, const float* head8, const float* head16,
                    const float* head32, const float* gain_pad, const int32_t* rects, float conf, float iou, int max_det, int round_boxes,
                    int shift, int full_h, int full_w, float* out_raw, float* out_dets, int32_t* out_counts);

int ffp_op_rt_topk(int device, int n, int nt, int nc, const float* scores, int s_cs, int s_coff, int32_t* out_idx);


int ffp_op_rt_dwconv(int device, int n, int h, int w, int c, int k, int s, int act, const float* x, int x_cs, int x_coff, const float* wt,
                     const float* bias, float* y, int y_cs, int y_coff, uint32_t* amax);
int ffp_op_rt_maxpool2(int device, int n, int h, int w, int c, const float* x, int x_cs, int x_coff, float* y, int y_cs, int y_coff, uint32_t* amax);
int ffp_op_rt_add(int device, long long npx, int c, const float* a, int a_cs, int a_coff, const float* b, int b_cs, int b_coff, long long period,
                  float* y, int y_cs, int y_coff, uint32_t* amax);
int ffp_op_rt_layernorm(int device, long long npx, const float* x, int x_cs, int x_coff, const float* gamma, const float* beta, float* y, int y_cs,
                        int y_coff, uint32_t* amax);
int ffp_op_rt_gelu(int device, long long npx, int c, float* x, int cs, int coff, uint32_t* amax);
int ffp_op_rt_attention(int device, int n, int L, const float* qk, int qk_cs, int qk_coff, const float* v, int v_cs, int v_coff, float* y, int y_cs,
                        int y_coff, uint32_t* amax);
int ffp_op_rt_enc_prep(int device, int n, const int32_t* hs, const int32_t* ws, const float* src0, const float* src1, const float* src2,
                       const int32_t* src_cs, const int32_t* src_coff, const float* valid, long long rows, float* t, float* tm, uint32_t* amax_t,
                       uint32_t* amax_tm);
int ffp_op_rt_gather(int device, int n, int nt, const float* e, int e_cs, int e_coff, const int32_t* idx, const float* anchors, float* q, int q_cs,
                     int q_coff, float* anc_out, uint32_t* amax);
int ffp_op_rt_ref(int device, long long nq, const float* delta, int d_cs, int d_coff, const float* anc, float* ref, int r_cs, int r_coff,
                  uint32_t* amax);
int ffp_op_rt_deform(int device, int n, const int32_t* hs, const int32_t* ws, const float* val, int v_cs, int v_coff, const float* oa, int oa_cs,
                     int oa_coff, const float* ref, int r_cs, int r_coff, float* y, int y_cs, int y_coff, uint32_t* amax);
int ffp_op_rt_decode(int device, int n, int nc, const float* ref, int r_cs, int r_coff, const float* scores, int s_cs, int s_coff, float conf,
                     const float* orig_wh, float* out_raw, float* out_det, int32_t* out_counts);
int ffp_op_rt_post_tiles(int device, int n, int nc, const float* ref, int r_cs, int r_coff, const float* scores, int s_cs, int s_coff, float conf,
                         const int32_t* tiles_xyxy, int full_h, int full_w, int mode, float* out_dets, int32_t* out_counts);

int ffp_op_scrfd_pool(int device, int n, const int32_t* hs, const int32_t* ws, int px_align, int c, int maxpool, int k, const float* x, int x_cs,
                      int x_coff, float* y, int y_cs, int y_coff);
int ffp_op_scrfd_post(int device, int n, int net_h, int net_w, int A, const int32_t* strides, int px_align, const float* const* heads,
                      const int32_t* cs, const int32_t* coff, const float* det_scale, float thresh, float nms_thresh, int cap, float* out,
                      int32_t* out_counts, float* raw_scores);
int ffp_op_scrfd_sahi_rows(int device, int n_tiles, int cap, const int32_t* tiles_xyxy, int full_h, int full_w, float conf, float* dets,
                           int32_t* counts, int32_t* out_bad);

int ffp_op_image_input(int device, int kind, int precision, const uint8_t* frame, int H, int W, int chan_order, int n, const int32_t* boxes_xyxy,
                       int size_a, int size_b, float* out, int32_t* out_hs, int32_t* out_ws);
int ffp_op_stem(int device, int precision, int fused, const uint8_t* frame, int H, int W, int chan_order, int n, const int32_t* boxes_xyxy, int imgsz,
                const float* w, const float* bias, int cout, int stride, int act, float* out);
int ffp_op_stem_conv(int device, const uint8_t* frame, int H, int W, int chan_order, int n, const int32_t* boxes_xyxy, int imgsz, const float* stem_w,
                     const float* stem_b, int stem_cout, const float* conv_w, const float* conv_b, float* out);

int ffp_op_conv2d_time(int device, int precision, int n, int h, int w, int cin, int cout, int k, int stride, int up, int iters,
                       int dbg_mask, int force_shape, float* out_us);

int ffp_det_last_ms(ffp_det* d, int stage, float* out_ms);
int ffp_sr_last_ms(ffp_sr* s, float* out_ms);

int ffp_det_last_conv_stats(ffp_det* d, double* out_flops, float* out_ms, int32_t* out_launches);
int ffp_sr_last_conv_stats(ffp_sr* s, double* out_flops, float* out_ms, int32_t* out_launches);

int ffp_det_set_profile(ffp_det* d, int enable);
int ffp_det_profile_count(ffp_det* d, int32_t* out_n);
int ffp_det_profile_get(ffp_det* d, int i, char* name, int name_cap, double* out_flops, float* out_ms, int32_t* out_launches);
int ffp_sr_set_profile(ffp_sr* s, int enable);
int ffp_sr_profile_count(ffp_sr* s, int32_t* out_n);
int ffp_sr_profile_get(ffp_sr* s, int i, char* name, int name_cap, double* out_flops, float* out_ms, int32_t* out_launches);
int ffp_det_profile_bytes(ffp_det* d, int i, double* out_bytes);
int ffp_sr_profile_bytes(ffp_sr* s, int i, double* out_bytes);
int ffp_conv_totals_enable(int on);
int ffp_conv_totals_count(int32_t* out_n);
int ffp_conv_totals_get(int i, char* name, int name_cap, double* out_flops, double* out_bytes, int64_t* out_launches);
int ffp_det_profile_detail(ffp_det* d, int i, char* name, int name_cap, double* out_flops, float* out_ms);
int ffp_sr_profile_detail(ffp_sr* s, int i, char* name, int name_cap, double* out_flops, float* out_ms);

typedef struct ffp_scrfd ffp_scrfd;

int ffp_scrfd_create(const void* onnx_bytes, size_t nbytes, int n, int device, int precision, ffp_scrfd** out);
void ffp_scrfd_destroy(ffp_scrfd* s);

int ffp_scrfd_describe(const void* onnx_bytes, size_t nbytes, int n, int det_w, int det_h, char* out, size_t cap);

int ffp_scrfd_infer_tiles(ffp_scrfd* s, const uint8_t* frame_hwc, int H, int W, int chan_order, const int32_t* tiles_xyxy,
                          int n_tiles, int det_w, int det_h, float det_thresh, float nms_thresh, float* out_dets, int cap,
                          int32_t* out_counts);

#define FFP_SCRFD_TILES_LOCAL 0
#define FFP_SCRFD_TILES_SAHI 1
#define FFP_SCRFD_TILES_DEFAULT_BATCH 16
int ffp_scrfd_infer_tiles_ex(ffp_scrfd* s, const uint8_t* frame_hwc, int H, int W, int chan_order, const int32_t* tiles_xyxy, int n_tiles,
                             int det_w, int det_h, float det_thresh, float nms_thresh, float conf, int mode, int max_batch, float* out_dets,
                             int cap, int32_t* out_counts);
int ffp_scrfd_infer_tiles_dev(ffp_scrfd* s, const uint8_t* d_frame_hwc, int H, int W, int chan_order, const int32_t* tiles_xyxy, int n_tiles,
                              int det_w, int det_h, float det_thresh, float nms_thresh, float conf, int mode, int max_batch,
                              float* d_out_dets, int cap, int32_t* d_out_counts);
int ffp_scrfd_sliced_predict(ffp_scrfd* s, const uint8_t* frame_hwc, int H, int W, int chan_order, int slice_h, int slice_w,
                             float overlap_h_ratio, float overlap_w_ratio, int perform_standard_pred, int det_w, int det_h, float det_thresh,
                             float nms_thresh, float conf, int max_batch, int tile_cap, int pp_type, int pp_metric, double pp_thr,
                             int class_agnostic, float* out, int cap, int32_t* out_n);
int ffp_scrfd_sliced_predict_dev(ffp_scrfd* s, const uint8_t* d_frame_hwc, int H, int W, int chan_order, int slice_h, int slice_w,
                                 float overlap_h_ratio, float overlap_w_ratio, int perform_standard_pred, int det_w, int det_h,
                                 float det_thresh, float nms_thresh, float conf, int max_batch, int tile_cap, int pp_type, int pp_metric,
                                 double pp_thr, int class_agnostic, float* d_out, int cap, int32_t* d_out_n);
int ffp_scrfd_mem_bytes(ffp_scrfd* s, uint64_t* out_plan_bytes, int32_t* out_plans_resident);
int ffp_scrfd_drop_plans(ffp_scrfd* s);

int ffp_scrfd_forward_raw(ffp_scrfd* s, const uint8_t* frame_hwc, int H, int W, int chan_order, const int32_t* tiles_xyxy,
                          int n_tiles, int det_w, int det_h, float* out, size_t cap, int64_t* out_sizes);
int ffp_scrfd_geometry(int h, int w, int net_w, int net_h, int32_t* out2, float* det_scale);
int ffp_scrfd_info(ffp_scrfd* s, int32_t* out_n_outputs, double* out_last_conv_flops);

typedef struct ffp_rtdetr ffp_rtdetr;

int ffp_rtdetr_create(const void* weights, size_t nbytes, int device, int precision, ffp_rtdetr** out);
void ffp_rtdetr_destroy(ffp_rtdetr* r);
int ffp_rtdetr_predict(ffp_rtdetr* r, const uint8_t* const* frames, const int32_t* hw, int n, int imgsz, float conf, float* out_dets,
                       int32_t* out_counts);
int ffp_rtdetr_forward_raw(ffp_rtdetr* r, const uint8_t* const* frames, const int32_t* hw, int n, int imgsz, float* out, int32_t* out_topk);
int ffp_rtdetr_info(ffp_rtdetr* r, int32_t* out_nc, double* out_last_conv_flops, int32_t* out_graph_state);
int ffp_rtdetr_set_profile(ffp_rtdetr* r, int on);
int ffp_rtdetr_profile_count(ffp_rtdetr* r, int32_t* out_n);
int ffp_rtdetr_profile_get(ffp_rtdetr* r, int i, char* name, int name_cap, float* out_ms);

#define FFP_RT_TILES_LOCAL 0
#define FFP_RT_TILES_SAHI 1
#define FFP_RT_TILES_DEFAULT_BATCH 8
int ffp_rtdetr_infer_tiles(ffp_rtdetr* r, const uint8_t* frame_hwc, int H, int W, int chan_order, const int32_t* tiles_xyxy, int n_tiles,
                           int imgsz, float conf, int mode, int max_batch, float* out_dets, int32_t* out_counts);
int ffp_rtdetr_infer_tiles_dev(ffp_rtdetr* r, const uint8_t* d_frame_hwc, int H, int W, int chan_order, const int32_t* tiles_xyxy, int n_tiles,
// ... 26 lines not shown
```

Baseline: 147.8.

## Add light high-occupancy conv_k3d form chosen by the autotuner for small stride-1 convs

Adds a 'light' template variant of the 3x3 conv_k3d kernel for stride-1 shapes with at most 64 channels per workgroup. It forces three workgroups per CU, uses a single accumulator set and shallow prefetch, stages bias and output scale in LDS, and prefetches residual loads and the amax slot before the epilogue. The autotuner times the light form for eligible convs and keeps it only when it beats the chosen regular shape by a margin. The aim is better latency hiding through occupancy, paid for with tighter register budgets, possible spills, and extra tuning time.

```diff
diff --git a/face-detection-with-yolov11-sahi-and-real-esrgan_amd/_lib.py b/face-detection-with-yolov11-sahi-and-real-esrgan_amd/_lib.py
--- a/face-detection-with-yolov11-sahi-and-real-esrgan_amd/_lib.py
+++ b/face-detection-with-yolov11-sahi-and-real-esrgan_amd/_lib.py
@@ -128,6 +128,8 @@
     "ffp_jpeg_decode_dev": (C.c_int, [C.c_int, _p(C.c_uint8), C.c_int64, C.c_int, C.c_void_p, C.c_int64, C.c_int64]),
     "ffp_jpeg_decode_stats": (C.c_int, [_p(C.c_int64), _p(C.c_int64), _p(C.c_int64)]),
     "ffp_op_conv2d_shape": (C.c_int, [C.c_int]),
+    "ffp_op_conv2d_k3d_light": (C.c_int, [C.c_int]),
+    "ffp_op_k3d_light_launches": (C.c_longlong, []),
     "ffp_op_conv2d_shape_name": (C.c_int, [C.c_int, C.c_char_p, C.c_int]),
     "ffp_op_conv2d_last_variant": (C.c_int, [C.c_char_p, C.c_int]),
     "ffp_op_conv2d_act_post": (C.c_int, [C.c_int]),
@@ -1542,6 +1544,14 @@
     _check(lib().ffp_op_conv2d_shape(int(shape)))
 
 
+def op_conv2d_k3d_light(form: int = -1) -> None:
+    _check(lib().ffp_op_conv2d_k3d_light(int(form)))
+
+
+def op_k3d_light_launches() -> int:
+    return int(lib().ffp_op_k3d_light_launches())
+
+
 def op_conv2d_shape_name(shape: int) -> str:
     out = C.create_string_buffer(64)
     _check(lib().ffp_op_conv2d_shape_name(int(shape), out, len(out)))
diff --git a/face-detection-with-yolov11-sahi-and-real-esrgan_amd/csrc/api_ops.cpp b/face-detection-with-yolov11-sahi-and-real-esrgan_amd/csrc/api_ops.cpp
--- a/face-detection-with-yolov11-sahi-and-real-esrgan_amd/csrc/api_ops.cpp
+++ b/face-detection-with-yolov11-sahi-and-real-esrgan_amd/csrc/api_ops.cpp
@@ -2,6 +2,7 @@
 #include <cmath>
 
 #include "api_util.hpp"
+#include "conv_args.hpp"
 #include "conv_route.hpp"
 #include "rtdetr.hpp"
 #include "scrfd.hpp"
@@ -19,6 +20,16 @@
   g_op_conv_shape = force_shape;
   FFP_API_END
 }
+
+static int g_op_conv_k3d_light = -1;
+int ffp_op_conv2d_k3d_light(int form) {
+  FFP_API_BEGIN
+  FFP_CHECK(form >= -1 && form <= 1, FFP_ERR_ARG, "conv2d_k3d_light: form %d (-1 the route's rule, 0 regular, 1 light)", form);
+  g_op_conv_k3d_light = form;
+  FFP_API_END
+}
+
+long long ffp_op_k3d_light_launches(void) { return conv_k3d_light_launches(); }
 
 int ffp_op_conv2d_shape_name(int shape, char* out, int cap) {
   FFP_API_BEGIN
@@ -102,6 +113,7 @@
     o.pc = &pc; o.in = vin; o.out = vout; o.stride = stride; o.act = act; o.up = up;
     if (res) { o.has_res1 = true; o.res1 = vres; o.s1 = res_scale; }
     o.force_shape = g_op_conv_shape;
+    o.k3d_light = g_op_conv_k3d_light;
     o.act_post = g_op_conv_act_post;
     launch_conv(o, cx.st);
     tl_op_conv_variant = conv_variant(o);
@@ -496,6 +508,7 @@
   if (res2) { o.has_res2 = true; o.res2 = view(dr2.p, r2_cs, r2_coff, cout, &lout, -1); o.s2 = s2; }
   if (gate) o.gate = dgate.as<int>();
   o.force_shape = g_op_conv_shape;
+  o.k3d_light = g_op_conv_k3d_light;
   launch_conv(o, cx.st);
   tl_op_conv_variant = conv_variant(o);
   FFP_HIP(hipStreamSynchronize(cx.st));
@@ -1230,6 +1243,7 @@
   }
   ConvOp o;
   o.pc = &pc; o.stride = stride; o.act = precision == FFP_PREC_F16 ? ACT_LRELU : ACT_SILU; o.up = up; o.dbg = dbg_mask; o.force_shape = force_shape;
+  o.k3d_light = g_op_conv_k3d_light;
   o.in = TView{din.p, T, pc.cin, 0, pc.cin, &lin};
   o.out = TView{dout.p, T, cout, 0, cout, &lout};
   std::unique_ptr<TrunkPlan> tp;
diff --git a/face-detection-with-yolov11-sahi-and-real-esrgan_amd/csrc/conv_args.hpp b/face-detection-with-yolov11-sahi-and-real-esrgan_amd/csrc/conv_args.hpp
--- a/face-detection-with-yolov11-sahi-and-real-esrgan_amd/csrc/conv_args.hpp
+++ b/face-detection-with-yolov11-sahi-and-real-esrgan_amd/csrc/conv_args.hpp
@@ -170,7 +170,9 @@
 void conv_dwpw_init();
 
 unsigned conv_k3d_mask(const ConvOp& op, const ConvArgs& a);
-void launch_conv_k3d(ConvArgs& a, int shape, int stride, Level* out_lvl, hipStream_t st);
+void launch_conv_k3d(ConvArgs& a, int shape, int stride, Level* out_lvl, hipStream_t st, bool light = false);
 void conv_k3d_init();
+bool conv_k3d_light_ok(int shape, int stride);
+long long conv_k3d_light_launches();
 
 }
diff --git a/face-detection-with-yolov11-sahi-and-real-esrgan_amd/csrc/conv_k3d.hip b/face-detection-with-yolov11-sahi-and-real-esrgan_amd/csrc/conv_k3d.hip
--- a/face-detection-with-yolov11-sahi-and-real-esrgan_amd/csrc/conv_k3d.hip
+++ b/face-detection-with-yolov11-sahi-and-real-esrgan_amd/csrc/conv_k3d.hip
@@ -1,4 +1,5 @@
 #include <algorithm>
+#include <atomic>
 #include <cstdlib>
 #include <type_traits>
 
@@ -14,8 +15,9 @@
 
 typedef unsigned u32x4 __attribute__((ext_vector_type(4)));
 
-template <int S, int WM, int WN, int MI, int NIW> struct K3Geo {
+template <int S, int WM, int WN, int MI, int NIW, int LT = 0> struct K3Geo {
   static_assert(WM * WN == 4 && (S == 1 || S == 2), "geometry");
+  static_assert(LT == 0 || (S == 1 && MI * NIW * 16 <= 64 && LT >= 3 && LT <= 4), "light form: stride 1, at most 64 channels per workgroup");
   static constexpr int TH = 2 * WM * MI;
   static constexpr int HH = (TH - 1) * S + 3, HWD = 15 * S + 3;
   static constexpr int RP = HWD;
@@ -29,17 +31,20 @@
   static constexpr bool SCR_IN_STAGE = STAGE >= SCR;
   static constexpr int TCAP = 32;
   static constexpr int DESC = 2 * STAGE + (SCR_IN_STAGE ? 0 : SCR);
-  static constexpr int LDS = DESC + TCAP * 48;
+  static constexpr int BO = DESC + TCAP * 48;
+  static constexpr int LDS = BO + (LT ? 4 * NIW * 8 * 32 : 0);
   static constexpr int NTB = WN * NIW;
-  static constexpr int OCC = (MI * NIW * 16 > 64 || LDS > 80 * 1024) ? 1 : 2;
-  static constexpr int NSET = ((OCC == 2 && MI * NIW * 16 + 2 * NPW * 4 > 120) || NPW > 9) ? 1 : 2;
+  static constexpr int OCC = LT ? LT : (MI * NIW * 16 > 64 || LDS > 80 * 1024) ? 1 : 2;
+  static_assert(OCC * LDS <= 160 * 1024, "conv_k3d: the promised workgroups do not fit the CU's LDS");
+  static constexpr int NSET = (LT && MI * NIW > 1) ? 1 : ((OCC == 2 && MI * NIW * 16 + 2 * NPW * 4 > 120) || NPW > 9) ? 1 : 2;
   static constexpr int MPS = 3 * NIW * MI;
-  static constexpr int AD = MPS >= 12 ? 2 : MPS >= 6 ? 5 : 8;
+  static constexpr int AD = LT ? 2 : MPS >= 12 ? 2 : MPS >= 6 ? 5 : 8;
+  static constexpr int NPRE = LT ? 1 : 0;
 };
 
-template <int S, int WM, int WN, int MI, int NIW>
-__global__ void __launch_bounds__(256, (K3Geo<S, WM, WN, MI, NIW>::OCC)) conv_k3d_kernel(const ConvArgs a) {
-  using G = K3Geo<S, WM, WN, MI, NIW>;
+template <int S, int WM, int WN, int MI, int NIW, int LT = 0>
+__global__ void __launch_bounds__(256, (K3Geo<S, WM, WN, MI, NIW, LT>::OCC)) conv_k3d_kernel(const ConvArgs a) {
+  using G = K3Geo<S, WM, WN, MI, NIW, LT>;
   constexpr int NPW = G::NPW, RP = G::RP, HWD = G::HWD, NPX = G::NPX;
   extern __shared__ __attribute__((aligned(16))) unsigned char smem[];
 
@@ -66,6 +71,18 @@
     desc[tid * 3] = t;
     desc[tid * 3 + 1] = a.in_tab[t.x];
     desc[tid * 3 + 2] = a.out_tab[t.x];
+  }
+  if constexpr (LT != 0) {
+    if (lane < 8 * NIW) {
+      const int nt = nb0 * G::NTB + wn * NIW + (lane >> 3), chb = nt * 32 + (lane & 7) * 4;
+      float4 bv = make_float4(0.f, 0.f, 0.f, 0.f), sv = make_float4(1.f, 1.f, 1.f, 1.f);
+      if (nt < a.ntiles32) {
+        bv = *reinterpret_cast<const float4*>(a.bias + chb);
+        if (a.oscale) sv = *reinterpret_cast<const float4*>(a.oscale + chb);
+      }
+      float4* q = reinterpret_cast<float4*>(smem + G::BO) + (wave * NIW * 8 + lane) * 2;
+      q[0] = bv; q[1] = sv;
+    }
   }
   __syncthreads();
 
@@ -250,6 +267,30 @@
     advance_pf();
   };
 
+  constexpr int NPRE = G::NPRE;
+  uint4 rpre[NPRE ? NPRE : 1][4];
+  unsigned slot_pre = 0u;
+  auto pre_epilogue = [&](int j) __attribute__((always_inline)) {
+    const int4 t = desc[j * 3], ot = desc[j * 3 + 2];
+    const int oy0 = sgpr(t.y), ox0 = sgpr(t.z), Ho = sgpr(ot.y), Wo = sgpr(ot.z);
+    if (a.amax_img && a.amax_out) slot_pre = slot_peek(a.amax_out + sgpr(t.x));
+    if (!a.res1) return;
+    const unsigned char* r1b = reinterpret_cast<const unsigned char*>(a.res1) + ((long long)sgpr(ot.x) * a.r1_cs + a.r1_coff) * 4;
+    const auto rs_r1 = __builtin_amdgcn_make_buffer_rsrc(uniform_ptr(r1b), 0, 0x7FFFFFF0, 0x00020000);
+    const int ch0 = (lane & 7) * 4;
+#pragma unroll
+    for (int k = 0; k < NPRE; ++k) {
+      const int f = wm * MI + k / NIW, nt = nb0 * G::NTB + wn * NIW + k % NIW;
+#pragma unroll
+      for (int it = 0; it < 4; ++it) {
+        const int pp = it * 8 + (lane >> 3);
+        const int oy = oy0 + 2 * f + (pp >> 4), ox = ox0 + (pp & 15);
+        const bool ok = nt < a.ntiles32 && oy < Ho && ox < Wo && nt * 32 + ch0 < a.cout;
+        rpre[k][it] = bload(rs_r1, ok ? ((unsigned)(oy * Wo + ox) * a.r1_cs + nt * 32 + ch0) * 4 : OOB);
+      }
+    }
+  };
+
   auto epilogue = [&](int j, unsigned char* scr) __attribute__((always_inline)) {
     const int4 t = desc[j * 3], ot = desc[j * 3 + 2];
     const int oy0 = sgpr(t.y), ox0 = sgpr(t.z), Ho = sgpr(ot.y), Wo = sgpr(ot.z);
@@ -258,7 +299,7 @@
     item_scales(img, &ts_unused, &tinv);
     float am = 0.f;
     unsigned slot_now = 0u;
-    if (a.amax_img && a.amax_out) slot_now = slot_peek(a.amax_out + img);
+    if (a.amax_img && a.amax_out) slot_now = LT ? slot_pre : slot_peek(a.amax_out + img);
     const long long out_base = sgpr(ot.x);
     const unsigned char* r1b = a.res1 ? reinterpret_cast<const unsigned char*>(a.res1) + (out_base * a.r1_cs + a.r1_coff) * 4 : wb;
     const unsigned char* r2b = a.res2 ? reinterpret_cast<const unsigned char*>(a.res2) + (out_base * a.r2_cs + a.r2_coff) * 4 : wb;
@@ -276,8 +317,9 @@
         const int nt = nb0 * G::NTB + wn * NIW + ni;
         if (nt >= a.ntiles32) continue;
         const int chb = nt * 32 + ch0;
-        const float4 bv = *reinterpret_cast<const float4*>(a.bias + chb);
-        const float4 sv = a.oscale ? *reinterpret_cast<const float4*>(a.oscale + chb) : make_float4(1.f, 1.f, 1.f, 1.f);
+        const float4* bo = reinterpret_cast<const float4*>(smem + G::BO) + ((wave * NIW + ni) * 8 + (lane & 7)) * 2;
+        const float4 bv = LT ? bo[0] : *reinterpret_cast<const float4*>(a.bias + chb);
+        const float4 sv = LT ? bo[1] : a.oscale ? *reinterpret_cast<const float4*>(a.oscale + chb) : make_float4(1.f, 1.f, 1.f, 1.f);
         const float bias_t[4] = {bv.x, bv.y, bv.z, bv.w};
         const float osc_t[4] = {sv.x * tinv, sv.y * tinv, sv.z * tinv, sv.w * tinv};
         unsigned rel[4];
@@ -290,8 +332,9 @@
           oks[it] = oy < Ho && ox < Wo && nt * 32 + ch0 < a.cout;
           rel[it] = (unsigned)(oy * Wo + ox);
           r1v[it] = make_uint4(0u, 0u, 0u, 0u); r2v[it] = r1v[it];
-          if (a.res1) r1v[it] = bload(rs_r1, oks[it] ? (rel[it] * a.r1_cs + nt * 32 + ch0) * 4 : OOB);
-          if (a.res2) r2v[it] = bload(rs_r2, oks[it] ? (rel[it] * a.r2_cs + nt * 32 + ch0) * 4 : OOB);
+          if (mi * NIW + ni < NPRE) { if (a.res1) r1v[it] = rpre[mi * NIW + ni][it]; }
+          else if (a.res1) r1v[it] = bload(rs_r1, oks[it] ? (rel[it] * a.r1_cs + nt * 32 + ch0) * 4 : OOB);
+          if (a.res2 && !LT) r2v[it] = bload(rs_r2, oks[it] ? (rel[it] * a.r2_cs + nt * 32 + ch0) * 4 : OOB);
         }
         asm volatile("s_waitcnt lgkmcnt(0)" ::: "memory");
 #pragma unroll
@@ -312,6 +355,7 @@
             for (int q = 0; q < 4; ++q) v[q] = v[q] * a.s1 + r[q];
           }
           if (a.res2) {
+            if (LT) r2v[it] = bload(rs_r2, oks[it] ? (rel[it] * a.r2_cs + nt * 32 + ch0) * 4 : OOB);
             const float* r = reinterpret_cast<const float*>(&r2v[it]);
 #pragma unroll
             for (int q = 0; q < 4; ++q) v[q] = v[q] * a.s2 + r[q];
@@ -363,8 +407,14 @@
       zero_acc();
       cc = 0; ++cj;
     }
+    if constexpr (LT != 0) {
+      if (cc == NC - 1 && cj < J && !(DBG & 1)) pre_epilogue(cj);
+    }
     if (!(DBG & 64)) __syncthreads();
   };
+  if constexpr (LT != 0) {
+    if (NC == 1 && !(DBG & 1)) pre_epilogue(0);
+  }
   for (int q = 0; q < Q; q += 2) {
     step_chunk(std::integral_constant<int, 0>{}, smem, smem + G::STAGE);
     if (q + 1 >= Q) break;
@@ -373,11 +423,13 @@
   if (a.amax_out && !a.amax_img) raise_amax(a.amax_out, amax_run);
 }
 
-template <int S, int WM, int WN, int MI, int NIW> struct K3Cfg {
-  using G = K3Geo<S, WM, WN, MI, NIW>;
+std::atomic<long long> g_light_launches{0};
+
+template <int S, int WM, int WN, int MI, int NIW, int LT = 0> struct K3Cfg {
+  using G = K3Geo<S, WM, WN, MI, NIW, LT>;
   static_assert(G::LDS <= 160 * 1024, "conv_k3d: LDS");
   static void init() {
-    FFP_HIP(hipFuncSetAttribute(reinterpret_cast<const void*>(&conv_k3d_kernel<S, WM, WN, MI, NIW>), hipFuncAttributeMaxDynamicSharedMemorySize, G::LDS));
+    FFP_HIP(hipFuncSetAttribute(reinterpret_cast<const void*>(&conv_k3d_kernel<S, WM, WN, MI, NIW, LT>), hipFuncAttributeMaxDynamicSharedMemorySize, G::LDS));
   }
   static void launch(ConvArgs& a, Level* out_lvl, hipStream_t st) {
     int n_tiles = 0;
@@ -392,7 +444,8 @@
     long long ws = std::max<long long>(ws_env > 0 ? ws_env : 32 * G::OCC, (per_xcd + G::TCAP - 1) / G::TCAP);
     ws = (ws + a.n_nblk - 1) / a.n_nblk * a.n_nblk;
     FFP_CHECK(8 * ws < (1ll << 31) && (per_xcd + ws - 1) / ws <= G::TCAP, FFP_ERR_STATE, "conv_k3d: launch geometry");
-    hipLaunchKernelGGL((conv_k3d_kernel<S, WM, WN, MI, NIW>), dim3((unsigned)(8 * ws)), dim3(256), G::LDS, st, a);
+    hipLaunchKernelGGL((conv_k3d_kernel<S, WM, WN, MI, NIW, LT>), dim3((unsigned)(8 * ws)), dim3(256), G::LDS, st, a);
+    if (LT) g_light_launches.fetch_add(1, std::memory_order_relaxed);
   }
 };
 
@@ -415,9 +468,25 @@
   }
 };
 
+struct K3Light {
+  using V1 = K3Cfg<1, 2, 2, 2, 1, 3>;
+  using V2 = K3Cfg<1, 4, 1, 1, 1, 3>;
+  static void init() { V1::init(); V2::init(); }
+  static void launch(ConvArgs& a, int shape, Level* out_lvl, hipStream_t st) {
+    switch (shape) {
+      case SHAPE_K3D_64: V1::launch(a, out_lvl, st); break;
+      case SHAPE_K3D_32: V2::launch(a, out_lvl, st); break;
+      default: fail(FFP_ERR_ARG, "conv_k3d: shape %d has no light form", shape);
+    }
+  }
+};
+
 }
 
-void conv_k3d_init() { K3Family<1>::init(); K3Family<2>::init(); }
+void conv_k3d_init() { K3Family<1>::init(); K3Family<2>::init(); K3Light::init(); }
+
+bool conv_k3d_light_ok(int shape, int stride) { return stride == 1 && (shape == SHAPE_K3D_64 || shape == SHAPE_K3D_32); }
+long long conv_k3d_light_launches() { return g_light_launches.load(std::memory_order_relaxed); }
 
 static constexpr EpiCaps kEpiK3d{EPI_ALL_ACTS, true, true, false, true};
 unsigned conv_k3d_mask(const ConvOp& op, const ConvArgs& a) {
@@ -437,8 +506,11 @@
   return m;
 }
 
-void launch_conv_k3d(ConvArgs& a, int shape, int stride, Level* out_lvl, hipStream_t st) {
-  if (stride == 1) K3Family<1>::launch(a, shape, out_lvl, st);
+void launch_conv_k3d(ConvArgs& a, int shape, int stride, Level* out_lvl, hipStream_t st, bool light) {
+  if (light) {
+    FFP_CHECK(conv_k3d_light_ok(shape, stride), FFP_ERR_ARG, "conv_k3d: shape %d at stride %d has no light form", shape, stride);
+    K3Light::launch(a, shape, out_lvl, st);
+  } else if (stride == 1) K3Family<1>::launch(a, shape, out_lvl, st);
   else K3Family<2>::launch(a, shape, out_lvl, st);
 }
 
diff --git a/face-detection-with-yolov11-sahi-and-real-esrgan_amd/csrc/conv_route.cpp b/face-detection-with-yolov11-sahi-and-real-esrgan_amd/csrc/conv_route.cpp
--- a/face-detection-with-yolov11-sahi-and-real-esrgan_amd/csrc/conv_route.cpp
+++ b/face-detection-with-yolov11-sahi-and-real-esrgan_amd/csrc/conv_route.cpp
@@ -72,20 +72,27 @@
 ConvArgs conv_route_args(const ConvOp& op) { return op.dw || conv_direct_eligible(op) ? ConvArgs{} : make_conv_args(op); }
 
 ConvRoute conv_route(const ConvOp& op, const ConvArgs& a) {
+  FFP_CHECK(op.k3d_light >= -1 && op.k3d_light <= 1, FFP_ERR_ARG, "conv %s: k3d_light %d (-1, 0 or 1)", op.pc->name.c_str(), op.k3d_light);
+  const bool light = op.k3d_light == 1;
   if (op.dw) {
     FFP_CHECK((op.force_shape < 0 || op.force_shape == SHAPE_DWPW) && conv_dwpw_eligible(op), FFP_ERR_ARG, "conv %s: the depthwise-fused kernel cannot run this op", op.pc->name.c_str());
+    FFP_CHECK(!light, FFP_ERR_ARG, "conv %s: the depthwise-fused kernel has no light form", op.pc->name.c_str());
     return {F::DWPW, SHAPE_DWPW};
   }
   if (conv_direct_eligible(op)) {
     FFP_CHECK(!op.gate, FFP_ERR_ARG, "conv %s: the image-input kernel cannot honour a gate", op.pc->name.c_str());
+    FFP_CHECK(!light, FFP_ERR_ARG, "conv %s: the image-input kernel has no light form", op.pc->name.c_str());
     return {F::DIRECT, SHAPE_AUTO};
   }
   if (op.force_shape >= 0) {
     const ConvShapeInfo* s = conv_shape_info(op.force_shape);
     FFP_CHECK(s, FFP_ERR_ARG, "conv %s: %d is not a shape number", op.pc->name.c_str(), op.force_shape);
     FFP_CHECK(family_runs(s->family, s->shape, op, a), FFP_ERR_ARG, "conv %s: %s shape %d cannot run this op", op.pc->name.c_str(), s->family_name, s->shape);
-    return {s->family, s->shape};
-  }
+    FFP_CHECK(!light || (s->family == F::K3D && conv_k3d_light_ok(s->shape, op.stride)), FFP_ERR_ARG, "conv %s: %s shape %d at stride %d has no light form", op.pc->name.c_str(),
+              s->family_name, s->shape, op.stride);
+    return {s->family, s->shape, light};
+  }
+  FFP_CHECK(!light, FFP_ERR_ARG, "conv %s: the light form needs a forced conv_k3d shape", op.pc->name.c_str());
   const Switches& sw = switches();
   if (sw.rows16 && conv_rows16_eligible(op, a, SHAPE_ROWS16)) {
     if (sw.rows16_pc && a.dbg == 0) return {F::ROWS16PC, SHAPE_ROWS16PC};
@@ -100,6 +107,8 @@
   const Switches& sw = switches();
   return conv_generic_mask(op, a) | (sw.pw ? conv_pw_mask(op, a) : 0u) | (sw.k3d ? conv_k3d_mask(op, a) : 0u);
 }
+
+bool conv_k3d_light_offered() { return !env_is("FFP_K3D_LIGHT", '0'); }
 
 void launch_conv(const ConvOp& op, hipStream_t st) {
   ConvArgs a = conv_route_args(op);
@@ -111,7 +120,7 @@
     case F::ROWS16: launch_conv_rows16(a, r.shape, *op.pc, op.out.lvl, st); break;
     case F::ROWS16PC: launch_conv_rows16pc(a, *op.pc, op.out.lvl, st); break;
     case F::PW: launch_conv_pw(a, r.shape, st); break;
-    case F::K3D: launch_conv_k3d(a, r.shape, op.stride, op.out.lvl, st); break;
+    case F::K3D: launch_conv_k3d(a, r.shape, op.stride, op.out.lvl, st, r.light); break;
     case F::DWPW: launch_conv_dwpw(op, st); break;
     case F::TRUNK: {
       TrunkPlan tp(std::vector<ConvOp>{op});
@@ -128,11 +137,13 @@
   const ConvRoute r = conv_route(op, conv_route_args(op));
   if (r.family == F::DIRECT) return std::string(pc.dt == F32 ? "f32" : "f16") + "_k3_direct";
   char buf[64];
-  snprintf(buf, sizeof(buf), "%s_k%ds%d_%s", pc.dt == F16 ? "f16" : pc.split ? "f32x3" : "f32", pc.k, op.stride, conv_route_info(r.shape)->suffix);
+  snprintf(buf, sizeof(buf), "%s_k%ds%d_%s%s", pc.dt == F16 ? "f16" : pc.split ? "f32x3" : "f32", pc.k, op.stride, conv_route_info(r.shape)->suffix,
+           r.light ? "l" : "");
   return buf;
 }
 
-int conv_tune(const ConvOp& op, hipStream_t st) {
+int conv_tune(const ConvOp& op, hipStream_t st, int* k3d_light) {
+  if (k3d_light) *k3d_light = 0;
   const PackedConv& pc = *op.pc;
   const ConvArgs a = conv_route_args(op);
   const ConvRoute r = conv_route(op, a);
@@ -140,10 +151,13 @@
   const unsigned mask = conv_candidates(op, a);
   if (__builtin_popcount(mask) < 2) return -1;
   const int heur = r.shape;
+  const bool lights = k3d_light && op.k3d_light < 0 && !op.gate && pc.cin <= 64 && conv_k3d_light_offered();
+  auto light_offered = [&](int shape) { return lights && shape == SHAPE_K3D_64 && conv_k3d_light_ok(shape, op.stride); };
   ScopedEvent e0, e1;
-  auto time_shape = [&](int shape, int iters) {
+  auto time_shape = [&](int shape, int light, int iters) {
     ConvOp o = op;
     o.force_shape = shape;
+    o.k3d_light = light;
     o.gate = nullptr;
     FFP_HIP(hipEventRecord(e0, st));
     for (int i = 0; i < iters; ++i) launch_conv(o, st);
@@ -153,25 +167,40 @@
     FFP_HIP(hipEventElapsedTime(&ms, e0, e1));
     return ms * 1e3f / iters;
   };
-  float best_t = 0.f, heur_t = 0.f;
-  int best = -1;
-  for (int shape = 0; shape < SHAPE_COUNT; ++shape) {
-    if (!(mask & shape_bit(shape))) continue;
-    const float t1 = time_shape(shape, 2);
+  auto time_candidate = [&](int shape, int light) {
+    const float t1 = time_shape(shape, light, 2);
     const int iters = std::min(24, std::max(3, (int)(300.f / std::max(t1, 1.f))));
-    const float t = time_shape(shape, iters);
-    if (shape == heur) heur_t = t;
-    if (best < 0 || t < best_t) { best = shape; best_t = t; }
+    const float t = time_shape(shape, light, iters);
     static const bool log = [] { const char* e = getenv("FFP_TUNE_LOG"); return e && e[0] == '1'; }();
     if (log) {
       ConvOp o = op;
       o.force_shape = shape;
+      o.k3d_light = light;
       fprintf(stderr, "[tune] %-28s %4d->%4d k%d s%d px %9lld  shape %2d %-22s %9.1f us%s\n", pc.name.c_str(), pc.cin_real, pc.cout, pc.k, op.stride,
-              (long long)op.out.lvl->actual_px(), shape, conv_variant(o).c_str(), t, shape == heur ? "  (heuristic)" : "");
+              (long long)op.out.lvl->actual_px(), shape, conv_variant(o).c_str(), t, shape == heur && !light ? "  (heuristic)" : "");
     }
-  }
-  if (heur_t > 0.f && best_t > 0.97f * heur_t) return heur;
-  return best;
-}
-
-}
+    return t;
+  };
+  float best_t = 0.f, heur_t = 0.f, light_t = 0.f;
+  int best = -1, best_light = -1;
+  for (int shape = 0; shape < SHAPE_COUNT; ++shape) {
+    if (!(mask & shape_bit(shape))) continue;
+    const float t = time_candidate(shape, 0);
+    if (shape == heur) heur_t = t;
+    if (best < 0 || t < best_t) { best = shape; best_t = t; }
+    if (light_offered(shape)) {
+      const float tl = time_candidate(shape, 1);
+      if (best_light < 0 || tl < light_t) { best_light = shape; light_t = tl; }
+    }
+  }
+  int pick = best;
+  float pick_t = best_t;
+  if (heur_t > 0.f && best_t > 0.97f * heur_t) { pick = heur; pick_t = heur_t; }
+  if (best_light >= 0 && light_t < 0.97f * pick_t) {
+    *k3d_light = 1;
+    return best_light;
+  }
+  return pick;
+}
+
+}
diff --git a/face-detection-with-yolov11-sahi-and-real-esrgan_amd/csrc/conv_route.hpp b/face-detection-with-yolov11-sahi-and-real-esrgan_amd/csrc/conv_route.hpp
--- a/face-detection-with-yolov11-sahi-and-real-esrgan_amd/csrc/conv_route.hpp
+++ b/face-detection-with-yolov11-sahi-and-real-esrgan_amd/csrc/conv_route.hpp
@@ -28,9 +28,10 @@
 const ConvShapeInfo* conv_shape_info(int shape);
 const ConvShapeInfo* conv_route_info(int shape);
 
-struct ConvRoute { ConvFamily family; int shape; };
+struct ConvRoute { ConvFamily family; int shape; bool light = false; };
 ConvRoute conv_route(const ConvOp& op, const ConvArgs& a);
 ConvArgs conv_route_args(const ConvOp& op);
 unsigned conv_candidates(const ConvOp& op, const ConvArgs& a);
+bool conv_k3d_light_offered();
 
 }
diff --git a/face-detection-with-yolov11-sahi-and-real-esrgan_amd/csrc/engine.cpp b/face-detection-with-yolov11-sahi-and-real-esrgan_amd/csrc/engine.cpp
--- a/face-detection-with-yolov11-sahi-and-real-esrgan_amd/csrc/engine.cpp
+++ b/face-detection-with-yolov11-sahi-and-real-esrgan_amd/csrc/engine.cpp
@@ -351,9 +351,11 @@
   if (off) return;
   for (Step& s : steps) {
     if (!s.is_conv || s.trunk || s.conv->force_shape >= 0) continue;
-    const int best = conv_tune(*s.conv, st);
+    int light = 0;
+    const int best = conv_tune(*s.conv, st, &light);
     if (best >= 0) {
       s.conv->force_shape = best;
+      s.conv->k3d_light = light;
       s.variant = conv_variant(*s.conv);
     }
   }
diff --git a/face-detection-with-yolov11-sahi-and-real-esrgan_amd/csrc/ops.hpp b/face-detection-with-yolov11-sahi-and-real-esrgan_amd/csrc/ops.hpp
--- a/face-detection-with-yolov11-sahi-and-real-esrgan_amd/csrc/ops.hpp
+++ b/face-detection-with-yolov11-sahi-and-real-esrgan_amd/csrc/ops.hpp
@@ -30,13 +30,14 @@
   TView fin_out;
   std::string label;
   int dwpw_force = 0;
+  int k3d_light = -1;
   int force_shape = -1;
 };
 void launch_conv(const ConvOp& op, hipStream_t st);
 bool conv_direct_eligible(const ConvOp& op);
 void launch_conv_direct(const ConvOp& op, hipStream_t st);
 void conv_kernels_init();
-int conv_tune(const ConvOp& op, hipStream_t st);
+int conv_tune(const ConvOp& op, hipStream_t st, int* k3d_light);
 bool stem_conv_eligible(const ConvOp& stem, const ConvOp& conv);
 void stem_conv_pack(const ConvOp& stem, int flip, DevBuf& out, hipStream_t st);
 void launch_stem_conv(const uint8_t* d_frame, int H, int W, const DevBuf& d_imgs, const DevBuf& stem_w, const ConvOp& stem, const ConvOp& conv, hipStream_t st);
diff --git a/include/ffp.h b/include/ffp.h
--- a/include/ffp.h
+++ b/include/ffp.h
@@ -167,6 +167,8 @@
                        const float* wt, const float* bias, int cout, int act, float* y);
 
 int ffp_op_conv2d_shape(int force_shape);
+int ffp_op_conv2d_k3d_light(int form);
+long long ffp_op_k3d_light_launches(void);
 int ffp_op_conv2d_shape_name(int shape, char* out, int cap);
 int ffp_op_conv2d_last_variant(char* out, int cap);
 int ffp_op_conv2d_act_post(int act);
```

New measurement: 148.4 (median of 5 runs). About the same (+0.4%).
